# Linyou/Ced-NeRF

Measured on AMD Instinct MI355X. Metric: samples_per_sec (render_image_test, 800x800 D-NeRF lego-shaped synthetic), higher is better.
Workload: dtype f32 (MLP GEMMs: split-fp16 MFMA, 22-bit operands, fp32 accumulate)

## Files before the change

ced_nerf_amd/_lib.py:

```python
from __future__ import annotations

import ctypes as C
import os
import subprocess
from typing import List, Optional

_PKG = os.path.dirname(os.path.abspath(__file__))
_ROOT = os.path.dirname(_PKG)
LIB_PATH = os.environ.get("CED_NERF_LIB", os.path.join(_PKG, "libcednerf_hip.so"))
SOURCES = ["runtime.hip", "march.hip", "composite.hip", "field.hip", "field_half.hip", "field_mixed.hip", "frame.hip", "occgrid.hip",
           "raygen.hip", "wgrad.hip", "pixels.hip", "accel.hip", "linear.hip", "mlp.hip", "train_glue.hip", "losses.hip",
           "metrics.hip", "train_batch.hip", "importance.hip"]
MLP_F32, MLP_F16X2, MLP_F16, MLP_F32_HEAD16X2 = 0, 1, 2, 3
MLP_PRECISIONS = {"f32": MLP_F32, "f16x2": MLP_F16X2, "f16": MLP_F16, "f32+h16x2": MLP_F32_HEAD16X2}
HIPCC_FLAGS = ["--offload-arch=gfx950", "-O3", "-ffp-contract=off", "-fno-slp-vectorize", "-fPIC", "-shared", "-std=c++17"]
PER_SOURCE_FLAGS = {"field_half.hip": ["-mllvm", "-amdgpu-sched-strategy=max-memory-clause"]}
MAX_LEVELS = 16


class HashDesc(C.Structure):
    _fields_ = [
        ("n_levels", C.c_int32), ("table_dtype", C.c_int32), ("temporal", C.c_int32), ("reserved", C.c_int32),
        ("scale", C.c_float * MAX_LEVELS), ("res", C.c_uint32 * MAX_LEVELS), ("offset", C.c_uint32 * MAX_LEVELS),
        ("size", C.c_uint32 * MAX_LEVELS), ("hashed", C.c_uint32 * MAX_LEVELS),
# ... 20 lines not shown


EXCHANGE_FN = C.CFUNCTYPE(C.c_int, C.c_void_p, C.c_void_p, C.c_int32, C.c_int32, C.c_void_p)


class ShardExchange(C.Structure):
    _fields_ = [
        ("global_rays_per_frame", C.c_int64), ("local_rays", C.c_void_p), ("counts", C.c_void_p),
        ("reduce", EXCHANGE_FN), ("user", C.c_void_p),
    ]


_vp, _i64, _i32, _f = C.c_void_p, C.c_int64, C.c_int32, C.c_float

PROTOTYPES = {
    "ced_version": (C.c_int, []),
    "ced_last_error_string": (C.c_char_p, []),
    "ced_set_option": (C.c_int, [C.c_char_p, C.c_int]),
    "ced_packed_weight_floats": (_i64, [C.c_int, C.c_int]),
    "ced_pack_field_weights": (C.c_int, [C.c_int, C.c_int] + [_vp] * 10),
    "ced_packed_weight_words": (_i64, [C.c_int, C.c_int, C.c_int]),
    "ced_pack_field_weights_half": (C.c_int, [C.c_int, C.c_int, C.c_int] + [_vp] * 10),
    "ced_pack_field_weights_half_for": (C.c_int, [C.c_int] * 5 + [_vp] * 10),
    "ced_pack_field_weights_mixed": (C.c_int, [C.c_int, C.c_int] + [_vp] * 10),
    "ced_ray_aabb_intersect": (C.c_int, [_i64, _vp, _vp, _i32, _vp, _f, _f, _f, _vp, _vp, _vp, _vp]),
    "ced_sort_intersections": (C.c_int, [_i64, _i32, _vp, _vp, _vp, _vp, _vp]),
    "ced_traverse_grids": (C.c_int, [_i64, _vp, _vp, _vp, _i32, _i32, _vp, _vp, _vp, _f, _f, _i32, _vp, _vp, _vp, _vp,
                                     _i32, _vp, _vp, _vp, _vp, _vp, _vp, _vp, _vp]),
    "ced_host_skip_march": (_f, [_f, _f, _f, _f]),
    "ced_occupancy_accel_bytes": (_i64, [_i32, _i32]),
    "ced_build_occupancy_accel": (C.c_int, [_vp, _i32, _i32, _vp, _i64, _vp]),
    "ced_host_build_occupancy_accel": (C.c_int, [_vp, _i32, _i32, _vp]),
    "ced_host_count_steps": (_i32, [C.POINTER(C.c_float), _f, _f, _i32, C.POINTER(C.c_float)]),
    "ced_host_march_frame": (C.c_int, [_i64, _vp, _vp, _vp, _i32, _i32, _vp, _vp, _f, _f, _f, _i32, _vp, _vp, _vp, _vp, _i32, _i32,
                                       _i32, _vp, _vp, _vp, _vp]),
    "ced_hash_encode": (C.c_int, [C.POINTER(HashDesc), _i64, _vp, _vp, _vp, _vp]),
    "ced_hash_encode_backward": (C.c_int, [C.POINTER(HashDesc), _i64, _vp, _vp, _vp, _vp, _i32, _vp]),
    "ced_hash_encode_backward_temporal": (C.c_int, [C.POINTER(HashDesc), _i64, _vp, _vp, _vp, _vp, _vp]),
    "ced_field_forward": (C.c_int, [C.POINTER(FieldDesc), _i64, _vp, _vp, _vp, _vp, _vp, _vp, _vp]),
    "ced_field_forward_rays": (C.c_int, [C.POINTER(FieldDesc), _i64, _vp, _vp, _vp, _vp, _vp, _vp, _vp, _i32, _i32,
                                         _vp, _vp, _vp]),
    "ced_render_weights": (C.c_int, [_i64, _vp, _vp, _vp, _vp, _vp, _vp, _vp, _vp, _vp]),
    "ced_accumulate_along_rays": (C.c_int, [_i64, _vp, _vp, _vp, _i32, _vp, _vp]),
    "ced_reduce_along_rays": (C.c_int, [_i64, _vp, _vp, _i32, _vp, _i32, _i64, _i32, _vp, _vp, _vp]),
    "ced_visibility_mask": (C.c_int, [_i64, _vp, _vp, _vp, _vp, _f, _f, _vp, _vp]),
    "ced_composite_prefix": (C.c_int, [_i64, _vp, _vp, _vp, _vp, _vp, _vp, _vp, _vp, _vp]),
    "ced_composite_backward": (C.c_int, [_i64, _vp, _vp, _vp, _vp, _vp, _vp, _vp, _vp, _vp, _vp, _vp]),
    "ced_distortion_workspace_bytes": (_i64, [_i64, _i64, _i32]),
    "ced_distortion_loss": (C.c_int, [_i64, _i64] + [_vp] * 10),
    "ced_distortion_loss_density": (C.c_int, [_i64, _i64] + [_vp] * 10),
    "ced_ssim_workspace_bytes": (_i64, [_i64, _i64, _i64, _i64, _i32, _i32]),
    "ced_ssim": (C.c_int, [_i64, _i64, _i64, _i64, _vp, C.POINTER(_i64), _vp, C.POINTER(_i64), C.c_double, C.c_double,
                           C.c_double, _i32, C.POINTER(C.c_float), _i32, C.POINTER(C.c_float), _i32, _vp, _vp, _vp, _vp,
                           _vp, _vp]),
    "ced_frame_to_rgb8": (C.c_int, [_i32, _i32, _vp, _i32, _vp, _vp]),
    "ced_depth_to_u8": (C.c_int, [_i32, _i32, _vp, _i32, _vp, _vp, _vp]),
    "ced_scatter_pixels": (C.c_int, [_i64, _vp, _i32, _vp, _i32, _vp, _i32, _vp, _i64, _vp, _vp, _vp, _vp, _i32, _i32, _vp]),
    "ced_linear": (C.c_int, [_i64, _vp, _i32, _vp, _i32, _i32, _i32, _i32, _i32, _vp, _vp, _vp]),
    "ced_weight_grad_workspace_bytes": (_i64, [_i64, _i32, _i32]),
    "ced_weight_grad": (C.c_int, [_i64, _vp, _i32, _vp, _i32, _vp, _vp, _i64, _vp]),
    "ced_composite_step": (C.c_int, [_i64, _vp, _vp, _vp, _vp, _vp, _vp, _vp, _vp, _f, _i32, _vp, _vp, _vp]),
    "ced_composite_test": (C.c_int, [_i64, _vp, _vp, _vp, _vp, _vp, _vp, _f, _f, _vp, _vp, _vp, _vp]),
    "ced_finalize_pixels": (C.c_int, [_i64, _vp, _vp, _vp, _vp, _vp]),
    "ced_occ_cell_points": (C.c_int, [_i64, _vp, _vp, _i32, C.POINTER(C.c_float), _vp, _vp]),
    "ced_occ_ema_update": (C.c_int, [_i64, _vp, _vp, _f, _f, _vp, _vp]),
    "ced_generate_rays_pinhole": (C.c_int, [_i32, _i32, _f, _f, _f, _f, C.POINTER(C.c_float), _i32, _vp, _vp, _vp, _vp]),
    "ced_generate_rays_hypercam": (C.c_int, [_i32, _i32, C.POINTER(C.c_float), C.POINTER(C.c_float), _f, _f, _f, _f, _f,
                                             C.POINTER(C.c_float), C.POINTER(C.c_float), _vp, _vp, _vp]),
    "ced_sample_training_batch": (C.c_int, [_i32] * 5 + [_vp] * 3 + [_i64, C.c_uint64, _i64, _i32, _i32] + [_vp] * 7),
    "ced_importance_batch_workspace_bytes": (_i64, [_i64, _i64, _i64]),
    "ced_sample_importance_batch": (C.c_int, [_i32] * 5 + [_vp] * 4 + [_i32, _i64, _i64, C.c_uint64, _i64, _i32] + [_vp] * 8
                                    + [_i64, _vp]),
    "ced_temporal_median_u8": (C.c_int, [_i32] * 4 + [_vp] * 3),
    "ced_isg_weights": (C.c_int, [_i32] * 4 + [_vp, _vp, _f, _vp, _vp]),
    "ced_ist_weights": (C.c_int, [_i32] * 4 + [_vp, _f, _i32, _vp, _vp]),
    "ced_render_image_test_workspace_bytes": (_i64, [_i64, _i32, _i32, _f, _i32]),
    "ced_render_image_test": (C.c_int, [C.POINTER(FieldDesc), _i64, _vp, _vp, _vp, _i32, _i32, _vp, _vp, _f, _f, _f, _f, _f,
                                        _i32, _vp, _i32, _vp, _vp, _vp, _vp, _vp, _i64, _vp, C.POINTER(_i64),
                                        C.POINTER(FrameTrace), _vp, _vp]),
    "ced_render_frames_test_workspace_bytes": (_i64, [_i32, _i64, _i32, _i32, _f, _i32]),
    "ced_render_frames_test": (C.c_int, [C.POINTER(FieldDesc), _i32, _i64, _vp, _vp, _vp, _i32, _i32, _vp, _vp, _f, _f, _f, _f,
                                         _f, _i32, _vp, _vp, _vp, _vp, _vp, _vp, _i64, _vp, C.POINTER(_i64),
                                         C.POINTER(FrameTrace), _vp, _vp]),
    "ced_render_frames_test_sharded_workspace_bytes": (_i64, [_i32, _i64, _i64, _i32, _i32, _f, _i32]),
    "ced_render_frames_test_iterations": (_i32, [_f, _i32]),
    "ced_render_frames_test_host_bytes": (_i64, [_f, _i32]),
    "ced_render_frames_test_sharded": (C.c_int, [C.POINTER(FieldDesc), _i32, _i64, _vp, _vp, _vp, _i32, _i32, _vp, _vp, _f, _f, _f,
                                                 _f, _f, _i32, _vp, _vp, _vp, _vp, _vp, _vp, _i64, _vp, C.POINTER(_i64),
                                                 C.POINTER(FrameTrace), _vp, _vp, C.POINTER(ShardExchange)]),
    "ced_wall_clock_khz": (_i64, []),
    "ced_mlp_chain": (C.c_int, [_i64, _i32, _i32, _vp, C.POINTER(_i32), C.POINTER(_vp), C.POINTER(_vp), C.POINTER(_vp), _i32, _vp]),
    "ced_march_all": (C.c_int, [_i64, _vp, _vp, _vp, _i32, _i32, _vp, _vp, _vp, _f, _f, _f, _vp, _vp, _vp, _i32, _vp, _vp, _vp,
                                _vp, _i64, _vp, _vp]),
    "ced_render_image_workspace_bytes": (_i64, [_i64, _i64]),
    "ced_render_image": (C.c_int, [C.POINTER(FieldDesc), _i64, _vp, _vp, _i64, _vp, _vp, _vp, _f, _f, _vp, _i32, _vp, _vp, _vp,
                                   _vp, _vp, _vp, _i64, _vp, C.POINTER(_i64), _vp, _vp]),
    "ced_mlp_backward_dw_workspace_bytes": (_i64, [_i64, _i32, C.POINTER(_i32)]),
    "ced_mlp_backward_dw": (C.c_int, [_i64, _i32, _vp, C.POINTER(_i32), C.POINTER(_vp), C.POINTER(_vp), _vp, _vp, _vp, _i64, _vp]),
    "ced_train_inputs": (C.c_int, [_i64] + [_vp] * 13),
    "ced_train_warp": (C.c_int, [_i64, _vp, _vp, _i32, _i32, _f, C.POINTER(C.c_float), _vp, _vp, _vp, _vp]),
    "ced_train_warp_backward": (C.c_int, [_i64, _vp, _vp, _i32, _i32, _f, C.POINTER(C.c_float), _vp, _vp, _vp, _vp]),
    "ced_train_head_in": (C.c_int, [_i64] + [_vp] * 6),
    "ced_train_head_in_backward": (C.c_int, [_i64] + [_vp] * 6),
    "ced_render_image_gather": (C.c_int, [_i64, _i64, _i64, _vp, _i64, _vp, _i64, _vp, _vp, _vp, _vp, _vp, _vp, _vp, _vp, _vp]),
}


def _includes(path: str, seen=None) -> List[str]:
    import re
    seen = set() if seen is None else seen
    if path in seen or not os.path.exists(path):
        return []
    seen.add(path)
    out = [path]
    for inc in re.findall(r'^\s*#\s*include\s+"([^"]+)"', open(path).read(), flags=re.M):
        out += _includes(os.path.normpath(os.path.join(os.path.dirname(path), inc)), seen)
    return out


def build(force: bool = False, verbose: bool = False, extra_flags: Optional[List[str]] = None) -> str:
    from concurrent.futures import ThreadPoolExecutor
    srcs = [os.path.join(_PKG, "csrc", s) for s in SOURCES]
    hipcc = os.environ.get("HIPCC", "hipcc")
    flags = [f for f in HIPCC_FLAGS if f != "-shared"] + list(extra_flags or [])
    obj_dir = os.path.join(_ROOT, "build", "obj")
    os.makedirs(obj_dir, exist_ok=True)
    stamp = os.path.join(obj_dir, "flags.txt")
    flag_text = " ".join([hipcc] + flags + [f"{k}:{' '.join(v)}" for k, v in sorted(PER_SOURCE_FLAGS.items())])
    if not os.path.exists(stamp) or open(stamp).read() != flag_text:
        force = True
    jobs, objs = [], []
    for src in srcs:
        obj = os.path.join(obj_dir, os.path.basename(src) + ".o")
        objs.append(obj)
        deps = _includes(src)
        if force or not os.path.exists(obj) or any(os.path.getmtime(obj) < os.path.getmtime(d) for d in deps):
            jobs.append([hipcc] + flags + PER_SOURCE_FLAGS.get(os.path.basename(src), []) + ["-c", src, "-o", obj])
    if not jobs and os.path.exists(LIB_PATH) and all(os.path.getmtime(LIB_PATH) >= os.path.getmtime(o) for o in objs):
        return LIB_PATH

    def run(cmd):
        if verbose:
            print(" ".join(cmd), flush=True)
        subprocess.check_call(cmd)

    workers = max(1, min(len(jobs), int(os.environ.get("CED_BUILD_JOBS", str(min(os.cpu_count() or 1, 8))))))
    if jobs:
        with ThreadPoolExecutor(max_workers=workers) as pool:
            list(pool.map(run, jobs))
    run([hipcc, "--offload-arch=gfx950", "-shared", "-fPIC", "-o", LIB_PATH] + objs)
    from . import _k32_gate
    _, bad = _k32_gate.check(LIB_PATH)
    if bad:
        os.remove(LIB_PATH)
        raise RuntimeError("K = 32 residency gate failed (ced_nerf_amd/_k32_gate.py): "
                           + "; ".join(f"{k}: {v}" for k, v in sorted(bad.items())))
    with open(stamp, "w") as f:
        f.write(flag_text)
    return LIB_PATH


_lib: Optional[C.CDLL] = None


def lib() -> C.CDLL:
    global _lib
# ... 30 lines not shown
```

ced_nerf_amd/csrc/field_args.hpp:

```cpp
#pragma once
#include <hip/hip_runtime.h>
#include <atomic>
#include <cstdint>

#include "../../include/cednerf_hip.h"

namespace ced {

struct FieldArgs {
    int64_t n;
    const int64_t *n_dev;
    unsigned long long *stamp;
    const int64_t *base_dev;
    const float *pos, *t, *dir;
    const float *rays_o, *rays_d;
    const int64_t *ray_idx;
    const int32_t *ray_idx32;
    const float *t0, *t1, *timestamps;
    int rays_mode, t_per_ray, want_rgb;
    float *rgb, *sigma, *geo;
    float aabb[6];
    float moving_step;
    int use_div, time_mode;
    const void *weights;
    int table_dtype, temporal;
    int spread_tiles;
    int level_mode;
    int max_blocks;
    const void *table;
    float scale[CED_MAX_LEVELS];
    uint32_t res[CED_MAX_LEVELS], offset[CED_MAX_LEVELS], size[CED_MAX_LEVELS], hashed[CED_MAX_LEVELS];
};

extern std::atomic<int> g_march_two_pass;
extern std::atomic<int> g_field_spread_tiles;
constexpr int kFieldBlocksDefault = 256;

template <int NT, int THREADS, typename Kernel>
void launch_field_grid(Kernel kernel, const FieldArgs &A, void *stream)
{
    const int64_t n_tiles = (A.n + 16 * NT - 1) / (16 * NT);
    constexpr int waves = THREADS / 64;
    int64_t blocks = A.spread_tiles ? (n_tiles + 3) / 4 : (n_tiles + waves - 1) / waves;
    const int cap = A.max_blocks > 0 ? A.max_blocks : kFieldBlocksDefault;
    if (blocks > cap) blocks = cap;
    hipLaunchKernelGGL(kernel, dim3((unsigned)blocks), dim3(THREADS), 0, (hipStream_t)stream, A);
}

int launch_field(const ced_field_desc *d, FieldArgs &A, void *stream);
int launch_field_half(FieldArgs &A, int time_mode, int precision, void *stream);
int launch_field_mixed(FieldArgs &A, int time_mode, void *stream);

}
```

ced_nerf_amd/csrc/field_half.hip:

```cpp
#include <cstring>

#include "ced_common.hpp"
#include "field_args.hpp"
#include "field_device.hpp"
#include "field_half_device.hpp"

namespace ced {

template <bool TE> struct HalfBlob {
    static constexpr int KS_B0 = TE ? 2 : 1;
    static constexpr int M0 = 0;
    static constexpr int M1 = M0 + 4 * 1;
    static constexpr int M2 = M1 + 4 * 2;
    static constexpr int M3 = M2 + 4 * 2;
    static constexpr int B0 = M3 + 1 * 2;
    static constexpr int B1 = B0 + 4 * KS_B0;
    static constexpr int H0 = B1 + 1 * 2;
    static constexpr int H1 = H0 + 4 * 1;
    static constexpr int H2 = H1 + 4 * 2;
    static constexpr int FRAGS = H2 + 1 * 2;
};

constexpr bool half_kernel_k32(bool te, bool temporal, bool split, int threads)
{
// ... 10 lines not shown
    constexpr int WAVES = THREADS / kWave;
    constexpr bool K32 = half_kernel_k32(TE, TEMPORAL, SPLIT, THREADS);
    static_assert(!K32 || (WAVES & (WAVES - 1)) == 0, "field_tile_seq needs a power-of-two wave count");
    constexpr int TILE = 16 * NT;
    using BL = HalfBlob<TE>;
    constexpr int PLANE = BL::FRAGS * kFragHalves;
    constexpr int WHALVES = PLANE * (SPLIT ? 2 : 1);
    __shared__ __attribute__((aligned(16))) _Float16 lds[WHALVES + 16 * CED_MAX_LEVELS];
    __shared__ int next_elem;
    const int tid = threadIdx.x;
    const int lane = tid & 63;
    const int wave = __builtin_amdgcn_readfirstlane(tid >> 6);
    const int g = lane >> 4, c = lane & 15;

    int64_t n_eff = A.n;
    if (A.n_dev) {
        const int64_t nd = *A.n_dev;
        n_eff = nd < n_eff ? nd : n_eff;
    }
    const int64_t sbase = A.base_dev ? *A.base_dev : 0;
    const int64_t n_tiles = (n_eff + TILE - 1) / TILE;
    TileRange tiles;
    TileSeq seq;
    if constexpr (K32) {
        if (!field_tile_seq(A.spread_tiles, n_tiles, WAVES, seq)) return;
        tiles.first = field_tile_at(seq, wave);
        tiles.end = seq.end;
        tiles.stride = 0;
        if (tid == 0) next_elem = WAVES;
    } else {
        if (!field_tile_range(A.spread_tiles, n_tiles, WAVES, wave, tiles)) return;
    }
    if (A.stamp && tid == 0) atomicMin(A.stamp, (unsigned long long)wall_clock64());

    {
        const f4 *src = reinterpret_cast<const f4 *>(A.weights);
        f4 *dst = reinterpret_cast<f4 *>(lds);
        for (int i = tid; i < WHALVES / 8; i += THREADS) dst[i] = src[i];
        if (tid < CED_MAX_LEVELS) {
            uint32_t *lt = reinterpret_cast<uint32_t *>(lds + WHALVES);
            const LevelConst L = make_level(A.scale[tid], A.res[tid], A.offset[tid], A.size[tid], A.hashed[tid],
                                            EntryBytes<F16, TEMPORAL>::value);
            store_level(lt + tid * 8, L);
        }
    }
    __syncthreads();

    const float extent[3] = { A.aabb[3] - A.aabb[0], A.aabb[4] - A.aabb[1], A.aabb[5] - A.aabb[2] };

    auto next_tile = [&](int64_t tile) -> int64_t {
        if constexpr (K32) {
            int i = 0;
            if (lane == 0) i = atomicAdd(&next_elem, 1);
            return field_tile_at(seq, __builtin_amdgcn_readfirstlane(i));
        } else {
            return tile + tiles.stride;
        }
    };
    for (int64_t tile = tiles.first; tile < tiles.end; tile = next_tile(tile)) {
        int lds_off = 0;
        asm volatile("" : "+v"(lds_off));
        const _Float16 *const whi = lds + lds_off;
        const _Float16 *const wlo = whi + PLANE;
        const int64_t tile_base = tile * TILE;
        const int64_t left = n_eff - tile_base;
        const int in_tile = left < TILE ? (int)left : TILE;
        int sofs[NT];
        int64_t ridx[NT];
        float px[NT][3], tq[NT];
        bool any_used = !A.rays_mode;
#pragma unroll
        for (int j = 0; j < NT; ++j) {
            sofs[j] = 16 * j + c < in_tile ? 16 * j + c : in_tile - 1;
            const int64_t s = tile_base + sofs[j];
            if (A.rays_mode) {
                const int64_t r_in = A.ray_idx32 ? (int64_t)A.ray_idx32[sbase + s] : A.ray_idx[sbase + s];
                const bool used = r_in >= 0;
                const int64_t r = used ? r_in : 0;
                any_used = any_used || used;
                ridx[j] = r;
                const float tm2 = used ? A.t0[sbase + s] + A.t1[sbase + s] : 0.0f;
#pragma unroll
                for (int a = 0; a < 3; ++a) px[j][a] = A.rays_o[3 * r + a] + (A.rays_d[3 * r + a] * tm2) / 2.0f;
                tq[j] = A.t_per_ray ? A.timestamps[r] : A.timestamps[0];
            } else {
                ridx[j] = s;
#pragma unroll
                for (int a = 0; a < 3; ++a) px[j][a] = A.pos[3 * s + a];
                tq[j] = A.t[s];
            }
        }

        if (__ballot(any_used) == 0ull) continue;

        h8 Bh[NT][2], Bl[NT][2];
        f4 D[NT][4];

#pragma unroll
        for (int j = 0; j < NT; ++j) {
            float v = tq[j];
            v = (g == 0) ? px[j][0] : v;
            v = (g == 1) ? px[j][1] : v;
            v = (g == 2) ? px[j][2] : v;
            float f[8];
#pragma unroll
            for (int e = 0; e < 8; ++e) f[e] = det_sinpi_phase(v * (float)(1 << (e >> 1)), e & 1);
            to_half8<SPLIT>(f, Bh[j][0], Bl[j][0]);
        }
        mlp_layer_h<1, 4, NT, SPLIT>(whi + BL::M0 * kFragHalves, wlo + BL::M0 * kFragHalves, lane, Bh, Bl, D);
        to_operand_h<NT, SPLIT>(D, Bh, Bl);
        mlp_layer_h<2, 4, NT, SPLIT, K32>(whi + BL::M1 * kFragHalves, wlo + BL::M1 * kFragHalves, lane, Bh, Bl, D);
        to_operand_h<NT, SPLIT>(D, Bh, Bl);
        mlp_layer_h<2, 4, NT, SPLIT, K32>(whi + BL::M2 * kFragHalves, wlo + BL::M2 * kFragHalves, lane, Bh, Bl, D);
        to_operand_h<NT, SPLIT>(D, Bh, Bl);
        mlp_layer_h<2, 1, NT, SPLIT, K32>(whi + BL::M3 * kFragHalves, wlo + BL::M3 * kFragHalves, lane, Bh, Bl, D);

        float xn[NT][3], mnorm[NT];
        bool sel[NT];
#pragma unroll
        for (int j = 0; j < NT; ++j) {
            float mv[3];
            bool inside = true;
#pragma unroll
            for (int a = 0; a < 3; ++a) {
                const float off = __shfl(D[j][0][a], c, 64);
                float m = off * A.moving_step;
                if (A.use_div) {
                    constexpr int kFineReg[3] = { 3, 0, 1 };
                    const float fine = __shfl(D[j][0][kFineReg[a]], (a == 0) ? c : 16 + c, 64);
                    const float e = det_expf(2.0f * fine);
                    const float th = 1.0f - 2.0f / (e + 1.0f);
                    m = m + th * A.moving_step;
                }
                mv[a] = m;
                const float xm = px[j][a] + m;
                const float x = (xm - A.aabb[a]) / extent[a];
                inside = inside && (x > 0.0f && x < 1.0f);
                xn[j][a] = __builtin_fminf(__builtin_fmaxf(x, 0.0f), 1.0f);
            }
            sel[j] = inside;
            mnorm[j] = TE ? __builtin_sqrtf((mv[0] * mv[0] + mv[1] * mv[1]) + mv[2] * mv[2]) : 0.0f;
        }

        float R[NT][8];
        int k_lo[NT];
        float t_frac[NT];
#pragma unroll
        for (int j = 0; j < NT; ++j) {
            k_lo[j] = 0;
            t_frac[j] = 0.0f;
            if constexpr (TEMPORAL) temporal_keyframe(tq[j], k_lo[j], t_frac[j]);
        }
        const uint32_t *const ltab = reinterpret_cast<const uint32_t *>(whi + WHALVES);
#pragma unroll
        for (int i = 0; i < 4; ++i) {
            const LevelConst L = load_level(ltab + (4 * i + g) * 8);
            const int mode = (A.level_mode >> (2 * i)) & 3;
            if (mode == 1) {
#pragma unroll
                for (int j = 0; j < NT; ++j)
                    hash_level<F16, TEMPORAL, 1>(L, A.table, xn[j], k_lo[j], t_frac[j], R[j][2 * i], R[j][2 * i + 1]);
            } else if (mode == 2) {
#pragma unroll
                for (int j = 0; j < NT; ++j)
                    hash_level<F16, TEMPORAL, 2>(L, A.table, xn[j], k_lo[j], t_frac[j], R[j][2 * i], R[j][2 * i + 1]);
            } else if (mode == 3) {
#pragma unroll
                for (int j = 0; j < NT; ++j)
                    hash_level<F16, TEMPORAL, 3>(L, A.table, xn[j], k_lo[j], t_frac[j], R[j][2 * i], R[j][2 * i + 1]);
            } else {
#pragma unroll
                for (int j = 0; j < NT; ++j)
                    hash_level<F16, TEMPORAL, 0>(L, A.table, xn[j], k_lo[j], t_frac[j], R[j][2 * i], R[j][2 * i + 1]);
            }
        }
#pragma unroll
        for (int j = 0; j < NT; ++j) {
#pragma unroll
            for (int e = 0; e < 8; ++e) R[j][e] = __builtin_amdgcn_fmed3f(R[j][e], -kHalfMax, kHalfMax);
            to_half8<SPLIT>(R[j], Bh[j][0], Bl[j][0]);
            if constexpr (TE) {
                float tf[8];
#pragma unroll
                for (int e = 0; e < 8; ++e) tf[e] = (e < 3) ? time_feature(4 * e + g, A.time_mode, tq[j], mnorm[j]) : 0.0f;
                to_half8<SPLIT>(tf, Bh[j][1], Bl[j][1]);
            }
        }

        mlp_layer_h<BL::KS_B0, 4, NT, SPLIT>(whi + BL::B0 * kFragHalves, wlo + BL::B0 * kFragHalves, lane, Bh, Bl, D);
        to_operand_h<NT, SPLIT>(D, Bh, Bl);
        mlp_layer_h<2, 1, NT, SPLIT, K32>(whi + BL::B1 * kFragHalves, wlo + BL::B1 * kFragHalves, lane, Bh, Bl, D);

#pragma unroll
        for (int j = 0; j < NT; ++j) {
            const bool stored = 16 * j + c < in_tile;
            const int64_t s = tile_base + (16 * j + c);
            float sg = det_expf(D[j][0][3] - 1.0f);
            sg = sel[j] ? sg : 0.0f;
            if (g == 3 && stored) A.sigma[sbase + s] = sg;
            if (A.geo && stored) {
#pragma unroll
                for (int r = 0; r < 4; ++r)
                    if (4 * g + r < 15) A.geo[s * 15 + 4 * g + r] = D[j][0][r];
            }
        }

        if (A.want_rgb) {
#pragma unroll
            for (int j = 0; j < NT; ++j) {
                float dv[3];
#pragma unroll
                for (int a = 0; a < 3; ++a)
                    dv[a] = A.rays_mode ? A.rays_d[3 * ridx[j] + a] : A.dir[3 * (tile_base + sofs[j]) + a];
                const float nrm = __builtin_sqrtf((dv[0] * dv[0] + dv[1] * dv[1]) + dv[2] * dv[2]);
                const float comp = (g == 1) ? dv[1] : (g == 2) ? dv[2] : dv[0];
                const float u = (comp / nrm + 1.0f) / 2.0f;
                const float vv = u * 2.0f - 1.0f;
                const float coef = (g == 2) ? 0.48860251190291987f : -0.48860251190291987f;
                const float sh = (g == 0) ? 0.28209479177387814f : coef * vv;
                float hin[8];
                hin[0] = sh;
#pragma unroll
                for (int r = 0; r < 4; ++r) hin[1 + r] = __builtin_amdgcn_fmed3f(D[j][0][r], -kHalfMax, kHalfMax);
                hin[4] = (g == 3) ? 0.0f : hin[4];
                hin[5] = hin[6] = hin[7] = 0.0f;
                to_half8<SPLIT>(hin, Bh[j][0], Bl[j][0]);
            }
            mlp_layer_h<1, 4, NT, SPLIT>(whi + BL::H0 * kFragHalves, wlo + BL::H0 * kFragHalves, lane, Bh, Bl, D);
            to_operand_h<NT, SPLIT>(D, Bh, Bl);
            mlp_layer_h<2, 4, NT, SPLIT, K32>(whi + BL::H1 * kFragHalves, wlo + BL::H1 * kFragHalves, lane, Bh, Bl, D);
            to_operand_h<NT, SPLIT>(D, Bh, Bl);
            mlp_layer_h<2, 1, NT, SPLIT, K32>(whi + BL::H2 * kFragHalves, wlo + BL::H2 * kFragHalves, lane, Bh, Bl, D);
#pragma unroll
            for (int j = 0; j < NT; ++j) {
                const int64_t s = tile_base + (16 * j + c);
                const float o1 = 1.0f / (1.0f + det_expf(-D[j][0][0]));
                if (g < 3 && 16 * j + c < in_tile) A.rgb[3 * (sbase + s) + g] = o1;
            }
        }
    }
    if constexpr (K32) {
        __syncthreads();
        asm volatile("" ::: "v127");
    }
    if (A.stamp && lane == 0) atomicMax(A.stamp + 1, (unsigned long long)wall_clock64());
}

void pack_half_layer(const float *w, int n_out, int n_in, int nb, int ks, int frag, int row_map, int col_map,
                     _Float16 *hi, _Float16 *lo)
{
    for (int p = 0; p < nb * 16; ++p) {
        int neuron = p;
        if (row_map == HALF_ROW_HIDDEN) neuron = half_hidden_neuron(p);
        else if (row_map == HALF_ROW_HIDDEN_K32) neuron = half_hidden_neuron_k32(p);
        else if (row_map == HALF_ROW_BASE_OUT) neuron = half_base_out_neuron(p);
        else if (row_map == HALF_ROW_RGB) neuron = (p % 4 == 0) ? p / 4 : n_out;
        if (neuron >= n_out) continue;
        for (int k = 0; k < ks * 32; ++k) {
            const int g = (k % 32) / 8, e = k % 8;
            int in = k;
            if (col_map == HALF_COL_HASH) {
                if (k < 32) in = 2 * (4 * (e >> 1) + g) + (e & 1);
                else in = (e < 3 && 4 * e + g <= 8) ? 32 + 4 * e + g : -1;
            } else if (col_map == HALF_COL_K32) {
                in = half_hidden_neuron_k32(16 * (2 * (k / 32) + (e >> 2)) + 4 * g + (e & 3));
            } else if (col_map == HALF_COL_HEAD) {
                if (e == 0) in = g;
                else if (e <= 4 && 4 * g + e - 1 < 15) in = 4 + 4 * g + e - 1;
                else in = -1;
            }
            if (in < 0 || in >= n_in) continue;
            const float v = w[(int64_t)neuron * n_in + in];
            const _Float16 h = (_Float16)v;
            const int64_t idx = ((int64_t)(frag + (p / 16) * ks + k / 32) * 64 + 16 * g + (p % 16)) * 8 + e;
            hi[idx] = h;
            if (lo) lo[idx] = (_Float16)(v - (float)h);
        }
    }
}

int launch_field_half(FieldArgs &A, int time_mode, int precision, void *stream)
{
    const int sel = (time_mode ? 1 : 0) | (A.table_dtype ? 2 : 0) | (A.temporal ? 4 : 0);
    if (precision == CED_MLP_F16X2) {
        switch (sel) {
        case 0: launch_field_grid<2, 1024>(field_half_kernel<false, false, false, true, 2, 1024>, A, stream); break;
        case 1: launch_field_grid<2, 768>(field_half_kernel<true, false, false, true, 2, 768>, A, stream); break;
        case 2: launch_field_grid<2, 1024>(field_half_kernel<false, true, false, true, 2, 1024>, A, stream); break;
        case 3: launch_field_grid<2, 768>(field_half_kernel<true, true, false, true, 2, 768>, A, stream); break;
        case 4: launch_field_grid<2, 512>(field_half_kernel<false, false, true, true, 2, 512>, A, stream); break;
        case 5: launch_field_grid<2, 512>(field_half_kernel<true, false, true, true, 2, 512>, A, stream); break;
        case 6: launch_field_grid<2, 512>(field_half_kernel<false, true, true, true, 2, 512>, A, stream); break;
        default: launch_field_grid<2, 512>(field_half_kernel<true, true, true, true, 2, 512>, A, stream); break;
        }
    } else {
        switch (sel) {
        case 0: launch_field_grid<2, 768>(field_half_kernel<false, false, false, false, 2, 768>, A, stream); break;
        case 1: launch_field_grid<2, 768>(field_half_kernel<true, false, false, false, 2, 768>, A, stream); break;
        case 2: launch_field_grid<2, 768>(field_half_kernel<false, true, false, false, 2, 768>, A, stream); break;
        case 3: launch_field_grid<2, 768>(field_half_kernel<true, true, false, false, 2, 768>, A, stream); break;
// ... 78 lines not shown
```

ced_nerf_amd/csrc/field_kernel.hpp:

```cpp
#pragma once
#include "ced_common.hpp"
#include "field_args.hpp"
#include "field_device.hpp"
#include "field_half_device.hpp"

namespace ced {

struct LayerShape { int nb; int ks; };
__host__ __device__ constexpr int ks4_of(int ks) { return (ks + 3) / 4; }
__host__ __device__ constexpr int layer_floats(int nb, int ks) { return nb * ks4_of(ks) * 256; }

__host__ __device__ constexpr int base_out_neuron(int p)
{
    const int g = p >> 2, r = p & 3;
    return r > 0 ? (4 * r + g - 3) : (g < 3 ? 13 + g : 0);
}

template <bool TE> struct Blob {
    static constexpr int KS_B0 = TE ? 11 : 8;
    static constexpr int M0 = 0;
    static constexpr int M1 = M0 + layer_floats(4, 8);
    static constexpr int M2 = M1 + layer_floats(4, 16);
    static constexpr int M3 = M2 + layer_floats(4, 16);
    static constexpr int B0 = M3 + layer_floats(1, 16);
// ... 34 lines not shown
                    acc[j] = __builtin_amdgcn_mfma_f32_16x16x4f32(a[s], B[j][4 * q + s], acc[j], 0, 0, 0);
            }
        }
        if (q == KS4 - 1) {
#pragma unroll
            for (int j = 0; j < NT; ++j) D[j][nb] = acc[j];
        }
        a = a_next;
    }
}

template <int NB, bool RELU, int NT>
__device__ __forceinline__ void to_operand(const f4 (&D)[NT][4], float (&B)[NT][16])
{
#pragma unroll
    for (int j = 0; j < NT; ++j) {
#pragma unroll
        for (int nb = 0; nb < NB; ++nb) {
            float r[4];
#pragma unroll
            for (int q = 0; q < 4; ++q) {
                float v = D[j][nb][q];
                if constexpr (RELU) {
                    const int bits = __float_as_int(v);
                    v = __int_as_float(bits > 0 ? bits : 0);
                }
                r[q] = v;
            }
#pragma unroll
            for (int s = 0; s < 4; ++s) B[j][4 * nb + s] = r[s];
        }
    }
}

template <bool TE, bool F16, bool TEMPORAL, int NT, int THREADS, bool HEAD16 = false>
__global__ __launch_bounds__(THREADS) void field_kernel(FieldArgs A)
{
    constexpr int FIELD_THREADS = THREADS;
    constexpr int FIELD_WAVES = THREADS / kWave;
    constexpr int TILE = 16 * NT;
    using BL = Blob<TE>;
    __shared__ __attribute__((aligned(16))) float lds[BL::TOTAL + 8 * CED_MAX_LEVELS];
    const int tid = threadIdx.x;
    const int lane = tid & 63;
    const int g = lane >> 4, c = lane & 15;

    int64_t n_eff = A.n;
    if (A.n_dev) {
        const int64_t nd = *A.n_dev;
        n_eff = nd < n_eff ? nd : n_eff;
    }
    const int64_t sbase = A.base_dev ? *A.base_dev : 0;
    const int64_t n_tiles = (n_eff + TILE - 1) / TILE;
    TileRange tiles;
    if (!field_tile_range(A.spread_tiles, n_tiles, FIELD_WAVES, threadIdx.x >> 6, tiles)) return;
    if (A.stamp && tid == 0) atomicMin(A.stamp, (unsigned long long)wall_clock64());

    {
        const f4 *src = reinterpret_cast<const f4 *>(A.weights);
        f4 *dst = reinterpret_cast<f4 *>(lds);
        for (int i = tid; i < BL::TOTAL / 4; i += FIELD_THREADS) dst[i] = src[i];
        if (tid < CED_MAX_LEVELS) {
            uint32_t *lt = reinterpret_cast<uint32_t *>(lds + BL::TOTAL);
            const LevelConst L = make_level(A.scale[tid], A.res[tid], A.offset[tid], A.size[tid], A.hashed[tid],
                                            EntryBytes<F16, TEMPORAL>::value);
            store_level(lt + tid * 8, L);
        }
    }
    __syncthreads();

    const float extent[3] = { A.aabb[3] - A.aabb[0], A.aabb[4] - A.aabb[1], A.aabb[5] - A.aabb[2] };
    const bool shared_time = A.rays_mode && !A.t_per_ray;
    float t_feat[2] = { 0.0f, 0.0f };
    if (shared_time) {
        const float t_all = A.timestamps[0];
#pragma unroll
        for (int S = 6; S < 8; ++S) t_feat[S - 6] = det_sinpi_phase(t_all * (float)(1 << (2 * (S & 1) + (g >> 1))), g & 1);
    }

    for (int64_t tile = tiles.first; tile < tiles.end; tile += tiles.stride) {
        int lds_off = 0;
        asm volatile("" : "+v"(lds_off));
        const float *const lw = lds + lds_off;
        int64_t sidx[NT];
        int64_t ridx[NT];
        float px[NT][3], tq[NT];
        bool any_used = !A.rays_mode;
#pragma unroll
        for (int j = 0; j < NT; ++j) {
            int64_t s = tile * TILE + 16 * j + c;
            s = s < n_eff ? s : n_eff - 1;
            sidx[j] = s;
            if (A.rays_mode) {
                const int64_t r_in = A.ray_idx32 ? (int64_t)A.ray_idx32[sbase + s] : A.ray_idx[sbase + s];
                const bool used = r_in >= 0;
                const int64_t r = used ? r_in : 0;
                any_used = any_used || used;
                ridx[j] = r;
                const float tm2 = used ? A.t0[sbase + s] + A.t1[sbase + s] : 0.0f;
#pragma unroll
                for (int a = 0; a < 3; ++a) px[j][a] = A.rays_o[3 * r + a] + (A.rays_d[3 * r + a] * tm2) / 2.0f;
                tq[j] = A.t_per_ray ? A.timestamps[r] : A.timestamps[0];
            } else {
                ridx[j] = s;
#pragma unroll
                for (int a = 0; a < 3; ++a) px[j][a] = A.pos[3 * s + a];
                tq[j] = A.t[s];
            }
        }
        if (__ballot(any_used) == 0ull) continue;

        float B[NT][16];
        f4 D[NT][4];

#pragma unroll
        for (int j = 0; j < NT; ++j) {
            const bool odd = (g & 1) != 0;
            const float sc0 = (float)(1 << (g >> 1)), sc1 = 4.0f * sc0;
            const float vxy = odd ? px[j][1] : px[j][0];
            float p0, p1;
            det_sinpi_both(vxy * sc0, p0, p1);
            auto sw = __builtin_amdgcn_permlane16_swap(__float_as_uint(p0), __float_as_uint(p1), false, false);
            B[j][0] = __uint_as_float(sw[0]); B[j][2] = __uint_as_float(sw[1]);
            det_sinpi_both(vxy * sc1, p0, p1);
            sw = __builtin_amdgcn_permlane16_swap(__float_as_uint(p0), __float_as_uint(p1), false, false);
            B[j][1] = __uint_as_float(sw[0]); B[j][3] = __uint_as_float(sw[1]);
            const float scz = odd ? sc1 : sc0;
            det_sinpi_both(px[j][2] * scz, p0, p1);
            sw = __builtin_amdgcn_permlane16_swap(__float_as_uint(p0), __float_as_uint(p1), false, false);
            B[j][4] = __uint_as_float(sw[0]); B[j][5] = __uint_as_float(sw[1]);
            if (shared_time) {
                B[j][6] = t_feat[0];
                B[j][7] = t_feat[1];
            } else {
                det_sinpi_both(tq[j] * scz, p0, p1);
                sw = __builtin_amdgcn_permlane16_swap(__float_as_uint(p0), __float_as_uint(p1), false, false);
                B[j][6] = __uint_as_float(sw[0]); B[j][7] = __uint_as_float(sw[1]);
            }
        }
        mlp_layer<8, 4, NT>(lw + BL::M0, lane, B, D);
        to_operand<4, true, NT>(D, B);
        mlp_layer<16, 4, NT>(lw + BL::M1, lane, B, D);
        to_operand<4, true, NT>(D, B);
        mlp_layer<16, 4, NT>(lw + BL::M2, lane, B, D);
        to_operand<4, true, NT>(D, B);
        mlp_layer<16, 1, NT>(lw + BL::M3, lane, B, D);

        float xn[NT][3], mnorm[NT];
        bool sel[NT];
#pragma unroll
        for (int j = 0; j < NT; ++j) {
            float mv[3];
            bool inside = true;
#pragma unroll
            for (int a = 0; a < 3; ++a) {
                const float off = __shfl(D[j][0][a], c, 64);
                float m = off * A.moving_step;
                if (A.use_div) {
                    constexpr int kFineReg[3] = { 3, 0, 1 };
                    const float fine = __shfl(D[j][0][kFineReg[a]], (a == 0) ? c : 16 + c, 64);
                    const float e = det_expf(2.0f * fine);
                    const float th = 1.0f - 2.0f / (e + 1.0f);
                    m = m + th * A.moving_step;
                }
                mv[a] = m;
                const float xm = px[j][a] + m;
                const float x = (xm - A.aabb[a]) / extent[a];
                inside = inside && (x > 0.0f && x < 1.0f);
                xn[j][a] = __builtin_fminf(__builtin_fmaxf(x, 0.0f), 1.0f);
            }
            sel[j] = inside;
            mnorm[j] = TE ? __builtin_sqrtf((mv[0] * mv[0] + mv[1] * mv[1]) + mv[2] * mv[2]) : 0.0f;
        }

        float R[NT][8];
        int k_lo[NT];
        float t_frac[NT];
#pragma unroll
        for (int j = 0; j < NT; ++j) {
            k_lo[j] = 0;
            t_frac[j] = 0.0f;
            if constexpr (TEMPORAL) temporal_keyframe(tq[j], k_lo[j], t_frac[j]);
        }
        const uint32_t *const ltab = reinterpret_cast<const uint32_t *>(lw + BL::TOTAL);
#pragma unroll
        for (int i = 0; i < 4; ++i) {
            const LevelConst L = load_level(ltab + (4 * i + 2 * (g & 1) + (g >> 1)) * 8);
            const int mode = (A.level_mode >> (2 * i)) & 3;
            if (mode == 1) {
#pragma unroll
                for (int j = 0; j < NT; ++j)
                    hash_level<F16, TEMPORAL, 1>(L, A.table, xn[j], k_lo[j], t_frac[j], R[j][2 * i], R[j][2 * i + 1]);
            } else if (mode == 2) {
#pragma unroll
                for (int j = 0; j < NT; ++j)
                    hash_level<F16, TEMPORAL, 2>(L, A.table, xn[j], k_lo[j], t_frac[j], R[j][2 * i], R[j][2 * i + 1]);
            } else if (mode == 3) {
#pragma unroll
                for (int j = 0; j < NT; ++j)
                    hash_level<F16, TEMPORAL, 3>(L, A.table, xn[j], k_lo[j], t_frac[j], R[j][2 * i], R[j][2 * i + 1]);
            } else {
#pragma unroll
                for (int j = 0; j < NT; ++j)
                    hash_level<F16, TEMPORAL, 0>(L, A.table, xn[j], k_lo[j], t_frac[j], R[j][2 * i], R[j][2 * i + 1]);
            }
        }
#pragma unroll
        for (int j = 0; j < NT; ++j) {
#pragma unroll
            for (int i = 0; i < 4; ++i) {
                auto sw = __builtin_amdgcn_permlane16_swap(__float_as_uint(R[j][2 * i]), __float_as_uint(R[j][2 * i + 1]), false, false);
                B[j][2 * i] = __uint_as_float(sw[0]);
                B[j][2 * i + 1] = __uint_as_float(sw[1]);
            }
            if (TE) {
#pragma unroll
                for (int S = 8; S < 11; ++S) B[j][S] = time_feature(4 * (S - 8) + g, A.time_mode, tq[j], mnorm[j]);
            }
        }

        mlp_layer<BL::KS_B0, 4, NT>(lw + BL::B0, lane, B, D);
        to_operand<4, true, NT>(D, B);
        mlp_layer<16, 1, NT>(lw + BL::B1, lane, B, D);

#pragma unroll
        for (int j = 0; j < NT; ++j) {
            const int64_t s = tile * TILE + 16 * j + c;
            float sg = det_expf(D[j][0][HEAD16 ? 3 : 0] - 1.0f);
            sg = sel[j] ? sg : 0.0f;
            if (g == 3 && s < n_eff) A.sigma[sbase + s] = sg;
            if (A.geo && s < n_eff) {
#pragma unroll
                for (int r = 0; r < 4; ++r) {
                    const int nidx = HEAD16 ? half_base_out_neuron(4 * g + r) : base_out_neuron(4 * g + r);
                    if (nidx >= 1) A.geo[s * 15 + nidx - 1] = D[j][0][r];
                }
            }
        }

        if constexpr (HEAD16) {
            if (A.want_rgb) {
                const _Float16 *const hw = reinterpret_cast<const _Float16 *>(lw + BL::H0);
                const _Float16 *const hwl = hw + BL::HEAD_FRAGS * kFragHalves;
                h8 Bh[NT][2], Bl[NT][2];
#pragma unroll
                for (int j = 0; j < NT; ++j) {
                    float dv[3];
#pragma unroll
                    for (int a = 0; a < 3; ++a)
                        dv[a] = A.rays_mode ? A.rays_d[3 * ridx[j] + a] : A.dir[3 * sidx[j] + a];
                    const float nrm = __builtin_sqrtf((dv[0] * dv[0] + dv[1] * dv[1]) + dv[2] * dv[2]);
                    const float comp = (g == 1) ? dv[1] : (g == 2) ? dv[2] : dv[0];
                    const float u = (comp / nrm + 1.0f) / 2.0f;
                    const float vv = u * 2.0f - 1.0f;
                    const float coef = (g == 2) ? 0.48860251190291987f : -0.48860251190291987f;
                    float hin[8];
                    hin[0] = (g == 0) ? 0.28209479177387814f : coef * vv;
#pragma unroll
                    for (int r = 0; r < 4; ++r) hin[1 + r] = __builtin_amdgcn_fmed3f(D[j][0][r], -kHalfMax, kHalfMax);
                    hin[4] = (g == 3) ? 0.0f : hin[4];
                    hin[5] = hin[6] = hin[7] = 0.0f;
                    to_half8<true>(hin, Bh[j][0], Bl[j][0]);
                }
                mlp_layer_h<1, 4, NT, true>(hw + BL::HF_H0 * kFragHalves, hwl + BL::HF_H0 * kFragHalves, lane, Bh, Bl, D);
                to_operand_h<NT, true>(D, Bh, Bl);
                mlp_layer_h<2, 4, NT, true>(hw + BL::HF_H1 * kFragHalves, hwl + BL::HF_H1 * kFragHalves, lane, Bh, Bl, D);
                to_operand_h<NT, true>(D, Bh, Bl);
                mlp_layer_h<2, 1, NT, true>(hw + BL::HF_H2 * kFragHalves, hwl + BL::HF_H2 * kFragHalves, lane, Bh, Bl, D);
#pragma unroll
                for (int j = 0; j < NT; ++j) {
                    const float o1 = 1.0f / (1.0f + det_expf(-D[j][0][0]));
                    int lane_now = (int)threadIdx.x;
                    asm volatile("" : "+v"(lane_now));
                    const int g_now = (lane_now >> 4) & 3;
                    const int64_t s_now = tile * TILE + 16 * j + (lane_now & 15);
                    if (g_now < 3 && s_now < n_eff) A.rgb[3 * (sbase + s_now) + g_now] = o1;
                }
            }
            continue;
        }

        if (A.want_rgb) {
#pragma unroll
            for (int j = 0; j < NT; ++j) {
                const float geo_tail = (g == 3) ? 0.0f : D[j][0][0];
                float dv[3];
#pragma unroll
                for (int a = 0; a < 3; ++a)
                    dv[a] = A.rays_mode ? A.rays_d[3 * ridx[j] + a] : A.dir[3 * sidx[j] + a];
                const float nrm = __builtin_sqrtf((dv[0] * dv[0] + dv[1] * dv[1]) + dv[2] * dv[2]);
                const float comp = (g == 1) ? dv[1] : (g == 2) ? dv[2] : dv[0];
                const float u = (comp / nrm + 1.0f) / 2.0f;
                const float vv = u * 2.0f - 1.0f;
                const float coef = (g == 2) ? 0.48860251190291987f : -0.48860251190291987f;
                B[j][0] = (g == 0) ? 0.28209479177387814f : coef * vv;
                B[j][1] = D[j][0][1];
                B[j][2] = D[j][0][2];
                B[j][3] = D[j][0][3];
                B[j][4] = geo_tail;
            }
            mlp_layer<5, 4, NT>(lw + BL::H0, lane, B, D);
            to_operand<4, true, NT>(D, B);
            mlp_layer<16, 4, NT>(lw + BL::H1, lane, B, D);
            to_operand<4, true, NT>(D, B);
            mlp_layer<16, 1, NT>(lw + BL::H2, lane, B, D);
#pragma unroll
            for (int j = 0; j < NT; ++j) {
                const int64_t s = tile * TILE + 16 * j + c;
                const float o1 = 1.0f / (1.0f + det_expf(-D[j][0][0]));
                int lane_now = (int)threadIdx.x;
                asm volatile("" : "+v"(lane_now));
                const int g_now = (lane_now >> 4) & 3;
                const int64_t s_now = tile * TILE + 16 * j + (lane_now & 15);
                if (g_now < 3 && s_now < n_eff) A.rgb[3 * (sbase + s_now) + g_now] = o1;
            }
        }
    }
    if (A.stamp && lane == 0) atomicMax(A.stamp + 1, (unsigned long long)wall_clock64());
}

}
```

ced_nerf_amd/csrc/frame.hip:

```cpp
#include <atomic>
#include <cfloat>
#include <chrono>
#include <vector>

#include "ced_common.hpp"
#include "field_args.hpp"
#include "march_accel.hpp"

#ifdef CED_MARCH_DIAG
__device__ unsigned long long g_march_diag[8][3];
__device__ __forceinline__ unsigned long long (*ced_diag_acc())[8][3]
{
    __shared__ unsigned long long acc[16][8][3];
    return acc;
}
__device__ __forceinline__ unsigned long long *ced_diag_state()
{
    __shared__ unsigned long long st[16][2];
    return &st[0][0];
}
__device__ void ced_diag_tick(int phase)
{
    const unsigned long long m = __ballot(1);
    const int wave = threadIdx.x >> 6;
// ... 49 lines not shown
    int32_t gcount[kMaxFrames];
    int32_t limit[kMaxFrames];
    int32_t last[kMaxFrames];
    int32_t used[kMaxFrames];
    int32_t slot_base[kMaxFrames];
    int32_t samp_bound[kMaxFrames];
    int32_t total_slots;
    int32_t done;
    int32_t n_cand;
    int32_t cursor;
    int64_t sample_base;
    int64_t total_samples;
    unsigned long long next[kMaxFrames];
};

__device__ __forceinline__ int frame_of_slot(const IterPlan &P, int n_frames, int64_t s0)
{
    int lo = 0, hi = n_frames - 1;
    while (lo < hi) {
        const int mid = (lo + hi + 1) >> 1;
        if ((int64_t)P.slot_base[mid] <= s0) lo = mid; else hi = mid - 1;
    }
    return (P.count[lo] > 0 && s0 >= P.slot_base[lo] && s0 < (int64_t)P.slot_base[lo] + P.count[lo]) ? lo : -1;
}

template <int kWaves, class Reserve>
__device__ __forceinline__ int64_t workgroup_reserve(int n, Reserve reserve)
{
    __shared__ int wave_tot[kWaves];
    __shared__ long long block_base;
    const int lane = threadIdx.x & 63, wave = threadIdx.x >> 6;
    int incl = n;
#pragma unroll
    for (int off = 1; off < 64; off <<= 1) {
        const int v = __shfl_up(incl, off, 64);
        if (lane >= off) incl += v;
    }
    if (lane == 63) wave_tot[wave] = incl;
    __syncthreads();
    if (threadIdx.x == 0) {
        int run = 0;
        for (int w = 0; w < kWaves; ++w) { const int t = wave_tot[w]; wave_tot[w] = run; run += t; }
        block_base = run > 0 ? reserve(run) : 0;
    }
    __syncthreads();
    return (int64_t)block_base + wave_tot[wave] + (incl - n);
}

template <int kWaves, int kSums, class Reserve>
__device__ __forceinline__ int workgroup_append(bool take, const int *sums, Reserve reserve)
{
    __shared__ int wave_cnt[kWaves], wave_sum[kSums > 0 ? kSums : 1][kWaves];
    __shared__ int block_base;
    const int lane = threadIdx.x & 63, wave = threadIdx.x >> 6;
    const unsigned long long ballot = __ballot(take);
    int tot[kSums > 0 ? kSums : 1];
#pragma unroll
    for (int k = 0; k < kSums; ++k) tot[k] = sums[k];
#pragma unroll
    for (int off = 32; off >= 1; off >>= 1)
#pragma unroll
        for (int k = 0; k < kSums; ++k) tot[k] += __shfl_xor(tot[k], off, 64);
    if (lane == 0) {
        wave_cnt[wave] = __builtin_popcountll(ballot);
#pragma unroll
        for (int k = 0; k < kSums; ++k) wave_sum[k][wave] = tot[k];
    }
    __syncthreads();
    if (threadIdx.x == 0) {
        int run = 0;
#pragma unroll
        for (int k = 0; k < kSums; ++k) tot[k] = 0;
        for (int w = 0; w < kWaves; ++w) {
            const int t = wave_cnt[w]; wave_cnt[w] = run; run += t;
#pragma unroll
            for (int k = 0; k < kSums; ++k) tot[k] += wave_sum[k][w];
        }
        block_base = reserve(run, tot);
    }
    __syncthreads();
    return block_base + wave_cnt[wave] + __builtin_popcountll(ballot & ((1ull << lane) - 1ull));
}

__global__ __launch_bounds__(256) void frame_times_kernel(int64_t n_rays, int rays_per_frame,
                                                          const float *__restrict__ frame_times, float *__restrict__ ts_ray)
{
    const int64_t r = (int64_t)blockIdx.x * blockDim.x + threadIdx.x;
    if (r < n_rays) ts_ray[r] = frame_times[r / rays_per_frame];
}

__global__ __launch_bounds__(256) void frame_prep_kernel(int64_t n_rays, const float *__restrict__ rays_o,
                                                         const float *__restrict__ rays_d, int m,
                                                         const float *__restrict__ aabbs, float near_plane,
                                                         float *__restrict__ t_sorted, uint8_t *__restrict__ t_indices,
                                                         uint8_t *__restrict__ hits, float *__restrict__ near_planes,
                                                         float *__restrict__ rgb,
                                                         float *__restrict__ opacity, float *__restrict__ depth)
{
    int64_t r = (int64_t)blockIdx.x * blockDim.x + threadIdx.x;
    if (r >= n_rays) return;
    const float o[3] = { rays_o[3 * r], rays_o[3 * r + 1], rays_o[3 * r + 2] };
    const float inv_d[3] = { 1.0f / rays_d[3 * r], 1.0f / rays_d[3 * r + 1], 1.0f / rays_d[3 * r + 2] };
    float ev[2 * kMaxGrids];
    int id[2 * kMaxGrids];
    for (int a = 0; a < m; ++a) {
        float t0 = __builtin_inff(), t1 = __builtin_inff();
        bool hit = slab_test(o, inv_d, aabbs + 6 * a, t0, t1);
        if (!hit) { t0 = __builtin_inff(); t1 = __builtin_inff(); }
        hits[r * m + a] = hit ? 1 : 0;
        ev[a] = t0; id[a] = a;
        ev[m + a] = t1; id[m + a] = m + a;
    }
    if (m > 1) {
        for (int i = 1; i < 2 * m; ++i) {
            float v = ev[i];
            int k = id[i], j = i - 1;
            while (j >= 0 && ev[j] > v) { ev[j + 1] = ev[j]; id[j + 1] = id[j]; --j; }
            ev[j + 1] = v; id[j + 1] = k;
        }
    }
    for (int i = 0; i < 2 * m; ++i) {
        t_sorted[r * 2 * m + i] = ev[i];
        t_indices[r * 2 * m + i] = (uint8_t)id[i];
    }
    near_planes[r] = near_plane;
    rgb[3 * r] = 0.0f; rgb[3 * r + 1] = 0.0f; rgb[3 * r + 2] = 0.0f;
    opacity[r] = 0.0f;
    depth[r] = 0.0f;
}

__global__ __launch_bounds__(256) void frame_prep_single_kernel(int64_t n_rays, float near_plane, float *__restrict__ near_planes,
                                                                float *__restrict__ rgb, float *__restrict__ opacity,
                                                                float *__restrict__ depth)
{
    int64_t r = (int64_t)blockIdx.x * blockDim.x + threadIdx.x;
    if (r >= n_rays) return;
    near_planes[r] = near_plane;
    rgb[3 * r] = 0.0f; rgb[3 * r + 1] = 0.0f; rgb[3 * r + 2] = 0.0f;
    opacity[r] = 0.0f;
    depth[r] = 0.0f;
}

struct ScheduleArgs {
    IterPlan *plans;
    int it, n_frames, rays_per_frame, min_samples, max_samples;
    long long *host;
    long long seq;
    const int32_t *local_rays;
    const int64_t *xcounts;
    int64_t global_rays;
    long long *host_iter;
};

__device__ __forceinline__ void make_next_plan(const ScheduleArgs &S)
{
    const int f = threadIdx.x & 63;
    IterPlan &N = S.plans[S.it + 1];
    int local = 0, used = 0;
    long long global = 0;
    if (f < S.n_frames) {
        if (S.it < 0) {
            local = S.local_rays ? S.local_rays[f] : S.rays_per_frame;
            global = S.global_rays > 0 ? S.global_rays : local;
        } else {
            const IterPlan &P = S.plans[S.it];
            const unsigned long long nx = __hip_atomic_load(&P.next[f], __ATOMIC_RELAXED, __HIP_MEMORY_SCOPE_AGENT);
            const bool finished = P.last[f] || P.gcount[f] == 0;
            local = (finished || P.count[f] == 0) ? 0 : (int)(nx & 0xffffffffull);
            global = finished ? 0 : (S.xcounts ? S.xcounts[(int64_t)S.it * S.n_frames + f] : local);
            used = P.used[f];
        }
    }
    int count = 0, gcount = 0, limit = 0, last = 0;
    if (global > 0 && used < S.max_samples) {
        const long long n_total = S.global_rays > 0 ? S.global_rays : S.rays_per_frame;
        const long long q = n_total / global;
        limit = q < 64 ? (int)q : 64;
        if (limit < S.min_samples) limit = S.min_samples;
        used += limit;
        last = used >= S.max_samples ? 1 : 0;
        count = local;
        gcount = (int)(global < 0x7fffffffll ? global : 0x7fffffffll);
    }
    const int padded = (count + kSlotAlign - 1) & ~(kSlotAlign - 1);
    int incl = padded;
#pragma unroll
    for (int off = 1; off < 64; off <<= 1) {
        const int v = __shfl_up(incl, off, 64);
        if (f >= off) incl += v;
    }
    long long alive_here = count, alive_all = gcount;
#pragma unroll
    for (int off = 32; off >= 1; off >>= 1) {
        alive_here += __shfl_xor(alive_here, off, 64);
        alive_all += __shfl_xor(alive_all, off, 64);
    }
    const int total_slots = __shfl(incl, 63, 64);
    N.count[f] = count; N.gcount[f] = gcount; N.limit[f] = limit; N.last[f] = last; N.used[f] = used;
    N.slot_base[f] = incl - padded; N.samp_bound[f] = count * limit;
    N.next[f] = 0;
    if (f == 0) {
        N.total_slots = total_slots;
        N.sample_base = S.it < 0 ? 0 : S.plans[S.it].sample_base + S.plans[S.it].total_samples;
        N.total_samples = 0;
        N.n_cand = 0;
        N.cursor = 0;
        N.done = alive_all == 0 ? 1 : 0;
        S.host[0] = alive_here;
        S.host[1] = N.done;
        if (S.host_iter) {
            S.host_iter[3 * (S.it + 1)] = alive_here;
            S.host_iter[3 * (S.it + 1) + 1] = N.done;
        }
        __threadfence_system();
        __hip_atomic_store(&S.host[2], S.seq, __ATOMIC_RELEASE, __HIP_MEMORY_SCOPE_SYSTEM);
        if (S.host_iter) __hip_atomic_store(&S.host_iter[3 * (S.it + 1) + 2], S.seq, __ATOMIC_RELEASE, __HIP_MEMORY_SCOPE_SYSTEM);
    }
}

__global__ void frame_init_kernel(ScheduleArgs S, float *__restrict__ lattice_dev, unsigned long long *stamps = nullptr,
                                  int n_stamps = 0)
{
    for (int i = threadIdx.x; i < n_stamps; i += blockDim.x) {
// ... 140 lines not shown
            f = frame_of_slot(P, A.n_frames, s0);
            if (f < 0) continue;
            const int64_t idx = s0 + threadIdx.x - P.slot_base[f];
            active = idx < P.count[f];
            const int64_t first = (int64_t)f * A.rays_per_frame;
            r = active ? (A.alive ? (int64_t)A.alive[first + idx] : first + idx) : 0;
        }
        const int limit = P.limit[f];
        GridSpec grid = A.grid;
        grid.limit = limit;
        const int m = grid.n_grids;
        float o[3] = { 0.0f, 0.0f, 0.0f }, d[3] = { 0.0f, 0.0f, 1.0f };
        float near = 0.0f, t_term = 0.0f;
        const auto walk = [&](auto &&emit, float &t_out) {
            return traverse_ray_frame<kFrameLook, SINGLE, FIRST>(
                grid, A.accel, FIRST, o, d, near, A.far_plane,
                SINGLE ? nullptr : A.t_sorted + r * 2 * m, SINGLE ? (const uint8_t *)nullptr : A.t_indices + r * 2 * m,
                SINGLE ? nullptr : A.hits + r * m, emit, t_out);
        };
        SampleRuns runs;
        int n = 0;
        CED_DIAG_TICK(0);
        if (active) {
#pragma unroll
            for (int a = 0; a < 3; ++a) { o[a] = A.rays_o[3 * r + a]; d[a] = A.rays_d[3 * r + a]; }
            near = A.near_planes[r];
            n = walk([&](int i, float t0, float t1) { runs.record(i, t0, t1); }, t_term);
            A.near_planes[r] = t_term;
        }
        CED_DIAG_TICK(6);
        const int64_t start = workgroup_reserve<kWaves>(n, [&](int run) {
            return (long long)atomicAdd(reinterpret_cast<unsigned long long *>(&plan->total_samples), (unsigned long long)run);
        });
        if (active) {
            A.packed[2 * r] = (int32_t)start;
            A.packed[2 * r + 1] = n;
            float *const p0 = A.t_starts + start, *const p1 = A.t_ends + start;
            int32_t *const pr = A.ray_idx + start;
            const auto store = [&](int i, float t0, float t1) { p0[i] = t0; p1[i] = t1; pr[i] = (int32_t)r; };
            if (n > 0 && !runs.replayable(grid)) {
                float unused;
                (void)walk(store, unused);
            } else {
                runs.replay(grid, store);
            }
        }
        CED_DIAG_TICK(7);
        __syncthreads();
    }
#ifdef CED_MARCH_DIAG
    ced_diag_flush();
#endif
}

#ifdef CED_MARCH_DIAG
}
extern "C" int ced_diag_march_read(unsigned long long *out, int reset)
{
    if (hipDeviceSynchronize() != hipSuccess) return -1;
    if (out && hipMemcpyFromSymbol(out, HIP_SYMBOL(g_march_diag), sizeof(unsigned long long) * 24) != hipSuccess) return -1;
    if (reset) {
        unsigned long long z[24] = { 0 };
        if (hipMemcpyToSymbol(HIP_SYMBOL(g_march_diag), z, sizeof(z)) != hipSuccess) return -1;
    }
    return 0;
}
extern "C" int ced_diag_march_waves(unsigned int *out, int max_rows, int reset)
{
    if (hipDeviceSynchronize() != hipSuccess) return -1;
    unsigned int n = 0;
    if (hipMemcpyFromSymbol(&n, HIP_SYMBOL(g_march_wave_n), 4) != hipSuccess) return -1;
    if (n > (unsigned)kDiagWaves) n = kDiagWaves;
    if ((int)n > max_rows) n = max_rows;
    if (out && n && hipMemcpyFromSymbol(out, HIP_SYMBOL(g_march_wave_log), (size_t)n * 96) != hipSuccess) return -1;
    if (reset) {
        unsigned int z = 0;
        if (hipMemcpyToSymbol(HIP_SYMBOL(g_march_wave_n), &z, 4) != hipSuccess) return -1;
    }
    return (int)n;
}
namespace ced {
#endif

__global__ __launch_bounds__(kCompositeThreads) void frame_composite_kernel(
    IterPlan *plan, int n_frames, int rays_per_frame, const int32_t *__restrict__ alive_list,
    int32_t *__restrict__ next_list, const int32_t *__restrict__ packed, const float *__restrict__ t0,
    const float *__restrict__ t1, const float *__restrict__ sig, const float *__restrict__ rgbs, float *__restrict__ rgb,
    float *__restrict__ opacity, float *__restrict__ depth, float opc_thres)
{
    const IterPlan &P = *plan;
    const int64_t total = P.total_slots;
    for (int64_t s0 = (int64_t)blockIdx.x * kCompositeThreads; s0 < total; s0 += (int64_t)gridDim.x * kCompositeThreads) {
        const int f = frame_of_slot(P, n_frames, s0);
        if (f < 0) continue;
        const int limit = P.limit[f];
        const int64_t idx = s0 + threadIdx.x - P.slot_base[f];
        const bool active = idx < P.count[f];
        const int64_t first = (int64_t)f * rays_per_frame;
        const int64_t r = active ? (alive_list ? (int64_t)alive_list[first + idx] : first + idx) : 0;
        int cnt = 0;
        bool alive = false;
        if (active) {
            const int64_t sb = packed[2 * r];
            cnt = packed[2 * r + 1];
            float op = opacity[r];
            if (cnt > 0) {
                const float prefix = 1.0f - op;
                float c0 = rgb[3 * r], c1 = rgb[3 * r + 1], c2 = rgb[3 * r + 2], dp = depth[r];
                float acc = 0.0f;
                constexpr int kU = 4;
                int64_t i = sb;
                const int64_t end = sb + cnt;
                for (; i + kU <= end; i += kU) {
                    float ts[kU], te[kU], sg[kU], cr[kU], cg[kU], cb[kU];
#pragma unroll
                    for (int u = 0; u < kU; ++u) {
                        ts[u] = t0[i + u]; te[u] = t1[i + u]; sg[u] = sig[i + u];
                        cr[u] = rgbs[3 * (i + u)]; cg[u] = rgbs[3 * (i + u) + 1]; cb[u] = rgbs[3 * (i + u) + 2];
                    }
#pragma unroll
                    for (int u = 0; u < kU; ++u) {
                        float sd = sg[u] * (te[u] - ts[u]);
                        float a = 1.0f - det_expf(-sd);
                        float t = det_expf(-acc) * prefix;
                        float w = t * a;
                        c0 = c0 + w * cr[u];
                        c1 = c1 + w * cg[u];
                        c2 = c2 + w * cb[u];
                        op = op + w;
                        dp = dp + w * ((ts[u] + te[u]) / 2.0f);
                        acc = acc + sd;
                    }
                }
                for (; i < end; ++i) {
                    float ts = t0[i], te = t1[i];
                    float sd = sig[i] * (te - ts);
                    float a = 1.0f - det_expf(-sd);
                    float t = det_expf(-acc) * prefix;
                    float w = t * a;
                    c0 = c0 + w * rgbs[3 * i];
                    c1 = c1 + w * rgbs[3 * i + 1];
                    c2 = c2 + w * rgbs[3 * i + 2];
                    op = op + w;
                    dp = dp + w * ((ts + te) / 2.0f);
                    acc = acc + sd;
                }
                rgb[3 * r] = c0; rgb[3 * r + 1] = c1; rgb[3 * r + 2] = c2;
                opacity[r] = op;
                depth[r] = dp;
            }
            alive = !P.last[f] && (op <= opc_thres) && (cnt == limit);
        }
        const int slot = workgroup_append<kCompositeThreads / 64, 1>(alive, &cnt, [&](int run, const int *samples) {
            const unsigned long long add = (unsigned long long)run + ((unsigned long long)samples[0] << 32);
            return add != 0 ? (int)(atomicAdd(&plan->next[f], add) & 0xffffffffull) : 0;
        });
        if (alive) next_list[first + slot] = (int32_t)r;
        __syncthreads();
    }
}

__global__ __launch_bounds__(64) void frame_schedule_kernel(ScheduleArgs S)
{
    make_next_plan(S);
}

__global__ __launch_bounds__(64) void frame_pack_counts_kernel(const IterPlan *__restrict__ plan, int n_frames,
                                                               int64_t *__restrict__ row)
{
    const int f = threadIdx.x;
    if (f >= n_frames) return;
    const unsigned long long nx = __hip_atomic_load(&plan->next[f], __ATOMIC_RELAXED, __HIP_MEMORY_SCOPE_AGENT);
    const bool finished = plan->last[f] || plan->gcount[f] == 0 || plan->count[f] == 0;
    row[f] = finished ? 0 : (int64_t)(nx & 0xffffffffull);
}

__global__ __launch_bounds__(256) void frame_finalize_kernel(int64_t n_rays, const float *__restrict__ bkgd,
                                                             float *__restrict__ rgb, const float *__restrict__ opacity,
                                                             float *__restrict__ depth)
{
    int64_t r = (int64_t)blockIdx.x * blockDim.x + threadIdx.x;
    if (r >= n_rays) return;
    float op = opacity[r];
    if (bkgd) {
        float rem = 1.0f - op;
        rgb[3 * r] = rgb[3 * r] + bkgd[0] * rem;
        rgb[3 * r + 1] = rgb[3 * r + 1] + bkgd[1] * rem;
        rgb[3 * r + 2] = rgb[3 * r + 2] + bkgd[2] * rem;
    }
    depth[r] = depth[r] / __builtin_fmaxf(op, FLT_EPSILON);
}

struct ImageState {
    int32_t *cursor;
    float *acc_all;
    float *acc_kept;
    int32_t *kept;
};

__global__ __launch_bounds__(256) void image_prep_kernel(int64_t n_rays, ImageState st, float *__restrict__ rgb,
                                                         float *__restrict__ opacity, float *__restrict__ depth)
{
    int64_t r = (int64_t)blockIdx.x * blockDim.x + threadIdx.x;
    if (r >= n_rays) return;
    st.cursor[r] = 0; st.acc_all[r] = 0.0f; st.acc_kept[r] = 0.0f; st.kept[r] = 0;
    if (rgb) {
        rgb[3 * r] = 0.0f; rgb[3 * r + 1] = 0.0f; rgb[3 * r + 2] = 0.0f;
        opacity[r] = 0.0f;
        depth[r] = 0.0f;
    }
}

__device__ __forceinline__ int64_t ray_count(const int64_t *__restrict__ packed_all, int64_t r, int64_t n_all)
{
    const int64_t start = packed_all[2 * r], cnt = packed_all[2 * r + 1];
    return (start < 0 || cnt < 0 || start + cnt > n_all) ? 0 : cnt;
}

__global__ __launch_bounds__(kMarchThreads) void image_chunk_kernel(
    IterPlan *__restrict__ plan, int64_t n_all, const int32_t *__restrict__ alive, const int64_t *__restrict__ packed_all,
    const float *__restrict__ t0_all, const float *__restrict__ t1_all, const int32_t *__restrict__ cursor,
    float *__restrict__ t0s, float *__restrict__ t1s, int32_t *__restrict__ ridx, int32_t *__restrict__ packed)
{
    const IterPlan &P = *plan;
    const int64_t total = P.count[0];
    const int limit = P.limit[0];
    const int64_t base = P.sample_base;
    for (int64_t s0 = (int64_t)blockIdx.x * kMarchThreads; s0 < total; s0 += (int64_t)gridDim.x * kMarchThreads) {
        const int64_t idx = s0 + threadIdx.x;
        const bool active = idx < total;
        const int64_t r = active ? (alive ? (int64_t)alive[idx] : idx) : 0;
        int n = 0;
        int64_t src = 0;
        if (active) {
            const int cur = cursor[r];
            const int64_t left = ray_count(packed_all, r, n_all) - cur;
            n = (int)(left < limit ? left : limit);
            src = packed_all[2 * r] + cur;
        }
        const int64_t slot = workgroup_reserve<kMarchThreads / 64>(n, [&](int run) {
            return (long long)atomicAdd(reinterpret_cast<unsigned long long *>(&plan->total_samples), (unsigned long long)run);
        });
        if (active) {
            const int64_t start = base + slot;
            packed[2 * r] = (int32_t)start;
            packed[2 * r + 1] = n;
            for (int i = 0; i < n; ++i) {
                t0s[start + i] = t0_all[src + i];
                t1s[start + i] = t1_all[src + i];
                ridx[start + i] = (int32_t)r;
            }
        }
        __syncthreads();
    }
}

template <bool FULL>
__global__ __launch_bounds__(kCompositeThreads) void image_composite_kernel(
    IterPlan *plan, const int32_t *__restrict__ alive_list, int32_t *__restrict__ next_list,
    const int32_t *__restrict__ packed, const int64_t *__restrict__ packed_all, const float *__restrict__ t0,
    const float *__restrict__ t1, const float *__restrict__ sig, const float *__restrict__ rgbs, ImageState st,
    float *__restrict__ w_out, float *__restrict__ tr_out, float *__restrict__ al_out, int32_t *__restrict__ rank_out,
    float *__restrict__ rgb, float *__restrict__ opacity, float *__restrict__ depth, float eps, float alpha_thre,
    int64_t n_all)
{
    const IterPlan &P = *plan;
    const int64_t total = P.count[0];
    for (int64_t s0 = (int64_t)blockIdx.x * kCompositeThreads; s0 < total; s0 += (int64_t)gridDim.x * kCompositeThreads) {
        const int64_t idx = s0 + threadIdx.x;
        const bool active = idx < total;
        const int64_t r = active ? (alive_list ? (int64_t)alive_list[idx] : idx) : 0;
        int cnt = 0, kept_new = 0;
        bool alive = false;
        if (active) {
            const int64_t sb = packed[2 * r];
            cnt = packed[2 * r + 1];
            if (cnt > 0) {
                float c0 = 0.0f, c1 = 0.0f, c2 = 0.0f, op = 0.0f, dp = 0.0f;
                if constexpr (FULL) { c0 = rgb[3 * r]; c1 = rgb[3 * r + 1]; c2 = rgb[3 * r + 2]; op = opacity[r]; dp = depth[r]; }
                float acc = st.acc_all[r], acck = st.acc_kept[r];
                int kept = st.kept[r];
                const int kept_before = kept;
                bool open = true;
                constexpr int kU = 4;
                const int64_t end = sb + cnt;
                for (int64_t i = sb; i < end; i += kU) {
                    float ts[kU], te[kU], sg[kU], cr[kU], cg[kU], cb[kU];
#pragma unroll
// ... 105 lines not shown
#pragma unroll
    for (int a = 0; a < 3; ++a) { o[a] = A.rays_o[3 * r + a]; d[a] = A.rays_d[3 * r + a]; }
    const int m = A.grid.n_grids;
    const float *const ts_row = SINGLE ? nullptr : A.t_sorted + r * 2 * m;
    const int64_t *const ti_row = SINGLE ? nullptr : A.t_indices + r * 2 * m;
    const uint8_t *const hit_row = SINGLE ? nullptr : A.hits + r * m;
    float t_term;
    if constexpr (!FILL) {
        const int n = traverse_ray_frame<kFrameLook, SINGLE, false>(A.grid, A.accel, true, o, d, A.near_planes[r], A.far_plane, ts_row,
                                                             ti_row, hit_row, [](int, float, float) {}, t_term);
        A.packed[2 * r + 1] = n;
    } else {
        const int64_t start = A.packed[2 * r];
        if (A.packed[2 * r + 1] == 0) return;
        float *const p0 = A.t_starts + start, *const p1 = A.t_ends + start;
        int64_t *const pr = A.ray_indices ? A.ray_indices + start : nullptr;
        (void)traverse_ray_frame<kFrameLook, SINGLE, false>(A.grid, A.accel, true, o, d, A.near_planes[r], A.far_plane, ts_row, ti_row,
                                                     hit_row,
                                                     [&](int i, float t0, float t1) {
                                                         p0[i] = t0; p1[i] = t1;
                                                         if (pr) pr[i] = r;
                                                     },
                                                     t_term);
    }
}

template <bool SINGLE>
__global__ __launch_bounds__(kMarchThreads, SINGLE ? 4 : 3) void march_all_onepass_kernel(MarchAllArgs A, int64_t capacity,
                                                                                         unsigned long long *total)
{
    const int64_t r = (int64_t)blockIdx.x * kMarchThreads + threadIdx.x;
    const bool active = r < A.n_rays;
    const int m = A.grid.n_grids;
    float o[3] = { 0.0f, 0.0f, 0.0f }, d[3] = { 0.0f, 0.0f, 1.0f };
    float near = 0.0f, t_term = 0.0f;
    const float *const ts_row = (SINGLE || !active) ? nullptr : A.t_sorted + r * 2 * m;
    const int64_t *const ti_row = (SINGLE || !active) ? nullptr : A.t_indices + r * 2 * m;
    const uint8_t *const hit_row = (SINGLE || !active) ? nullptr : A.hits + r * m;
    const auto walk = [&](auto &&emit, float &t_out) {
        return traverse_ray_frame<kFrameLook, SINGLE, false>(A.grid, A.accel, true, o, d, near, A.far_plane, ts_row, ti_row,
                                                             hit_row, emit, t_out);
    };
    SampleRuns runs;
    int n = 0;
    if (active) {
#pragma unroll
        for (int a = 0; a < 3; ++a) { o[a] = A.rays_o[3 * r + a]; d[a] = A.rays_d[3 * r + a]; }
        near = A.near_planes[r];
        n = walk([&](int i, float t0, float t1) { runs.record(i, t0, t1); }, t_term);
    }
    const int64_t start = workgroup_reserve<kMarchThreads / 64>(n, [&](int run) {
        return (long long)atomicAdd(total, (unsigned long long)run);
    });
    if (!active) return;
    A.packed[2 * r] = start;
    A.packed[2 * r + 1] = n;
    if (n == 0 || start + n > capacity) return;
    float *const p0 = A.t_starts + start, *const p1 = A.t_ends + start;
    const auto store = [&](int i, float t0, float t1) { p0[i] = t0; p1[i] = t1; };
    if (!runs.replayable(A.grid)) {
        float unused;
        (void)walk(store, unused);
    } else {
        runs.replay(A.grid, store);
    }
}

struct Carver {
    char *base;
    size_t off = 0;
    template <class T> T *take(size_t count)
    {
        T *p = (T *)(base + off);
        off = (off + count * sizeof(T) + 255) & ~(size_t)255;
        return p;
    }
};

struct FrameWorkspace {
    float *t_sorted; uint8_t *t_indices; uint8_t *hits; float *near; int32_t *packed;
    int32_t *alive_a, *alive_b;
    IterPlan *plans;
    float *lattice;
    float *ts_ray;
    float *t0, *t1; int32_t *ridx; float *sigma, *rgbs;
    uint8_t *accel;
    size_t bytes;
};

static inline int min_samples_of(float cone_angle) { return cone_angle == 0.0f ? 1 : 4; }
static inline int max_iterations(int max_samples, int min_samples) { return (max_samples + min_samples - 1) / min_samples; }

static inline int64_t sample_capacity(int n_frames, int64_t rays_per_frame, int min_samples, int64_t global_rays)
{
    int64_t per = rays_per_frame * min_samples;
    if (global_rays > rays_per_frame) {
        const int64_t worst = rays_per_frame * 64 < global_rays ? rays_per_frame * 64 : global_rays;
        if (worst > per) per = worst;
    }
    return per * n_frames;
}

static FrameWorkspace carve(void *base, int64_t n, int m, int64_t cap, int max_iters, int res, bool per_ray_times = false)
{
    FrameWorkspace w{};
    Carver c{ (char *)base };
    w.t_sorted = c.take<float>((size_t)n * 2 * m);
    w.t_indices = c.take<uint8_t>((size_t)n * 2 * m);
    w.hits = c.take<uint8_t>((size_t)n * m);
    w.near = c.take<float>((size_t)n);
    w.packed = c.take<int32_t>((size_t)n * 2);
    w.alive_a = c.take<int32_t>((size_t)n);
    w.alive_b = c.take<int32_t>((size_t)n);
    w.plans = c.take<IterPlan>((size_t)max_iters + 2);
    w.lattice = c.take<float>(256);
    w.ts_ray = c.take<float>(per_ray_times ? (size_t)n : 0);
    w.t0 = c.take<float>((size_t)cap);
    w.t1 = c.take<float>((size_t)cap);
    w.ridx = c.take<int32_t>((size_t)cap);
    w.sigma = c.take<float>((size_t)cap);
    w.rgbs = c.take<float>((size_t)cap * 3);
    const int64_t nbk = (res + kBrick - 1) / kBrick;
    w.accel = c.take<uint8_t>((size_t)(2 * m * nbk * nbk * nbk));
    w.bytes = c.off;
    return w;
}

static std::atomic<long long> g_publish_seq{ 0 };

#if defined(__HIP_DEVICE_COMPILE__)
#define CED_CPU_PAUSE()
#else
#define CED_CPU_PAUSE() __builtin_ia32_pause()
#endif

static int wait_published(volatile long long *flag, long long seq, hipStream_t stream, const char *who)
{
    const auto t_start = std::chrono::steady_clock::now();
    long spins = 0;
    while (__atomic_load_n(flag, __ATOMIC_ACQUIRE) < seq) {
        if ((++spins & 0x3ff) == 0) {
            if (std::chrono::steady_clock::now() - t_start > std::chrono::milliseconds(200)) {
                if (hipStreamSynchronize(stream) != hipSuccess) return check_launch("render_image_test (sync)");
                if (__atomic_load_n(flag, __ATOMIC_ACQUIRE) < seq) {
                    set_error("%s: iteration %lld was not published although the stream has drained", who, seq);
                    return CED_E_LAUNCH;
                }
                break;
            }
        } else {
            CED_CPU_PAUSE();
        }
    }
    return CED_OK;
}

static int run_ahead(volatile long long *pub, volatile long long *host_iter, const std::vector<long long> &plan_seq, int it,
                     hipStream_t stream, const char *who, bool &stop, long long &alive_bound)
{
    const int need = it - kRunAhead;
    if (need < 0 && host_iter) return CED_OK;
    volatile long long *const rec = host_iter ? host_iter + 3 * need : pub;
    if (need >= 0) {
        const int rc = wait_published(rec + 2, plan_seq[need], stream, who);
        if (rc) return rc;
    }
    if (host_iter || __atomic_load_n(pub + 2, __ATOMIC_ACQUIRE) >= plan_seq[0]) {
        if (rec[1]) {
            stop = true;
            return CED_OK;
        }
        const long long a = rec[0];
        if (a >= 0 && a < alive_bound) alive_bound = a;
    }
    return CED_OK;
}

static int read_back_plans(const IterPlan *dev_plans, int enqueued, hipStream_t stream, const char *what, const char *who,
                           std::vector<IterPlan> &plans, int &n_iters)
{
    plans.resize((size_t)enqueued + 1);
    if (hipMemcpyAsync(plans.data(), dev_plans, plans.size() * sizeof(IterPlan), hipMemcpyDeviceToHost, stream) != hipSuccess ||
        hipStreamSynchronize(stream) != hipSuccess)
        return check_launch(what);
    n_iters = 0;
    while (n_iters < enqueued && !plans[n_iters].done && plans[n_iters].total_slots != 0) ++n_iters;
    if (n_iters == enqueued && !plans[enqueued].done) {
        set_error("%s: the loop stopped after %d iterations with rays still alive", who, enqueued);
        return CED_E_LAUNCH;
    }
    return CED_OK;
}

static int render_frames_impl(const ced_field_desc *field, int n_frames, int64_t rays_per_frame, const float *rays_o,
                              const float *rays_d, const uint8_t *binaries, int32_t n_grids, int32_t res,
                              const float *aabbs, const void *accel, float near_plane, float far_plane, float step_size,
                              float cone_angle, float early_stop_eps, int32_t max_samples, const float *timestamps,
                              int32_t t_per_ray, const float *frame_times, const float *bkgd, float *rgb, float *opacity,
                              float *depth, void *workspace, int64_t workspace_bytes, int64_t *host_stats,
                              int64_t *total_samples_out, ced_frame_trace *trace, void *field_stream_, void *stream_,
                              const char *who, const ced_shard_exchange *xch = nullptr)
{
    hipStream_t stream = (hipStream_t)stream_;
    hipStream_t fstream = field_stream_ ? (hipStream_t)field_stream_ : stream;
    const bool split = fstream != stream;
    constexpr int kMaxDevices = 64;
    static thread_local hipEvent_t ev_to_field[kMaxDevices] = {}, ev_from_field[kMaxDevices] = {};
    int dev = 0;
    if (split) {
        if (hipGetDevice(&dev) != hipSuccess || dev < 0 || dev >= kMaxDevices) return check_launch("render_image_test (device)");
        if (!ev_to_field[dev] &&
            (hipEventCreateWithFlags(&ev_to_field[dev], hipEventDisableTiming) != hipSuccess ||
             hipEventCreateWithFlags(&ev_from_field[dev], hipEventDisableTiming) != hipSuccess))
            return check_launch("render_image_test (event create)");
    }
    const int64_t n_rays = (int64_t)n_frames * rays_per_frame;
    CED_REQUIRE(field != nullptr, "%s: null field descriptor", who);
    CED_REQUIRE(n_frames >= 1 && n_frames <= kMaxFrames, "%s: n_frames must be 1..%d", who, kMaxFrames);
    CED_REQUIRE(rays_per_frame >= 0 && n_grids >= 1 && n_grids <= kMaxGrids && res >= 1 && res <= 1024, "%s: bad sizes", who);
    CED_REQUIRE(n_rays < (1ll << 31) / 4, "%s: too many rays for 32-bit sample indices", who);
    CED_REQUIRE(max_samples >= 0, "%s: max_samples < 0", who);
    if (total_samples_out)
        for (int f = 0; f < n_frames; ++f) total_samples_out[f] = 0;
    if (trace) trace->n_iters = 0;
    if (n_rays == 0) return CED_OK;
    CED_REQUIRE(rays_o && rays_d && binaries && aabbs && (timestamps || frame_times) && rgb && opacity && depth &&
                    workspace && host_stats,
                "%s: null pointer", who);
    const int min_samples = min_samples_of(cone_angle);
    const int64_t cap = sample_capacity(n_frames, rays_per_frame, min_samples, xch ? xch->global_rays_per_frame : 0);
    CED_REQUIRE(cap < (1ll << 31) - 64, "%s: too many samples per iteration for 32-bit sample indices", who);
    const int max_iters = max_iterations(max_samples, min_samples);
    FrameWorkspace W = carve(workspace, n_rays, n_grids, cap, max_iters, res, frame_times != nullptr);
    CED_REQUIRE((int64_t)W.bytes <= workspace_bytes, "%s: workspace too small (%lld < %lld bytes)", who,
                (long long)workspace_bytes, (long long)W.bytes);
    if (xch) {
        CED_REQUIRE(xch->reduce && xch->counts && xch->global_rays_per_frame >= rays_per_frame &&
                        xch->global_rays_per_frame < (1ll << 31),
                    "%s: bad ced_shard_exchange (reduce / counts NULL, or global_rays_per_frame < rays_per_frame)", who);
        CED_REQUIRE(!field_stream_ || field_stream_ == stream_, "%s: a sharded call takes no separate field stream", who);
    }
    long long *const host_iter = xch ? (long long *)host_stats + kHostIterWord : nullptr;
    const dim3 blk(256), grd((unsigned)((n_rays + 255) / 256));

    if (n_grids == 1)
        hipLaunchKernelGGL(frame_prep_single_kernel, grd, blk, 0, stream, n_rays, near_plane, W.near, rgb, opacity, depth);
    else
        hipLaunchKernelGGL(frame_prep_kernel, grd, blk, 0, stream, n_rays, rays_o, rays_d, (int)n_grids, aabbs, near_plane,
                           W.t_sorted, W.t_indices, W.hits, W.near, rgb, opacity, depth);
    if (frame_times)
        hipLaunchKernelGGL(frame_times_kernel, grd, blk, 0, stream, n_rays, (int)rays_per_frame, frame_times, W.ts_ray);
    const int nb = (res + kBrick - 1) / kBrick;
    AccelSpec acc;
    if (accel) {
        acc = accel_view(accel, n_grids, res, true);
    } else {
        int rc = build_brick_accel(binaries, n_grids, res, W.accel, W.accel + (size_t)n_grids * nb * nb * nb, stream);
        if (rc) return rc;
        acc = AccelSpec{ W.accel, nb, nullptr };
    }
    volatile long long *pub = (volatile long long *)host_stats;
    std::vector<long long> plan_seq((size_t)max_iters + 1);
    plan_seq[0] = ++g_publish_seq;
    const bool use_lattice = cone_angle == 0.0f && step_size > 0.0f && near_plane >= 0.0f;
    if (use_lattice) build_lattice(near_plane, step_size, reinterpret_cast<float *>(host_stats + kHostLatticeWord));
    hipLaunchKernelGGL(frame_init_kernel, dim3(1), dim3(64), 0, stream,
                       ScheduleArgs{ W.plans, -1, n_frames, (int)rays_per_frame, min_samples, (int)max_samples,
                                     (long long *)host_stats, plan_seq[0], xch ? xch->local_rays : nullptr, nullptr,
                                     xch ? xch->global_rays_per_frame : 0, host_iter },
                       use_lattice ? W.lattice : (float *)nullptr,
                       (unsigned long long *)(trace ? trace->field_stamps : nullptr),
                       (trace && trace->field_stamps) ? (int)trace->capacity : 0);
    int rc = check_launch("render_image_test (prep)");
    if (rc) return rc;

    const float opc_thres = (float)(1.0 - (double)early_stop_eps);
    long long alive_bound = n_rays;
    int it = 0;
    for (; it < max_iters; ++it) {
        bool stop = false;
        rc = run_ahead(pub, host_iter, plan_seq, it, stream, who, stop, alive_bound);
        if (rc) return rc;
        if (stop) break;
        IterPlan *plan = W.plans + it;
        const int32_t *cur_list = it == 0 ? nullptr : ((it & 1) ? W.alive_a : W.alive_b);
        int32_t *next_list = (it & 1) ? W.alive_b : W.alive_a;

        const int64_t slot_bound = alive_bound + (int64_t)n_frames * kSlotAlign;
        MarchArgs M{ rays_o, rays_d, GridSpec{ binaries, aabbs, n_grids, res, step_size, cone_angle, 0, use_lattice ? W.lattice : nullptr },
                     acc, W.near, far_plane, cur_list, n_frames,
                     (int)rays_per_frame, W.t_sorted, W.t_indices, W.hits, W.t0, W.t1, W.ridx, W.packed, W.alive_b };
        int64_t mgrid = (slot_bound + kMarchThreads - 1) / kMarchThreads;
        if (mgrid > 8192) mgrid = 8192;
        const dim3 mblk(kMarchThreads);
        const int two_pass_opt = g_march_two_pass;
        const bool two_pass = two_pass_opt < 0 ? n_grids > 1 : two_pass_opt != 0;
        if (it == 0 && acc.bdist && two_pass) {
            int64_t kgrid = (slot_bound + kCullThreads - 1) / kCullThreads;
            if (kgrid > 8192) kgrid = 8192;
            if (mgrid > 4096) mgrid = 4096;
            if (n_grids == 1) {
                hipLaunchKernelGGL(march_cull_kernel<true>, dim3((unsigned)kgrid), dim3(kCullThreads), 0, stream, M, plan);
                hipLaunchKernelGGL((march_frame_kernel<true, true, true>), dim3((unsigned)mgrid), mblk, 0, stream, M, plan);
            } else {
                hipLaunchKernelGGL(march_cull_kernel<false>, dim3((unsigned)kgrid), dim3(kCullThreads), 0, stream, M, plan);
                hipLaunchKernelGGL((march_frame_kernel<false, true, true>), dim3((unsigned)mgrid), mblk, 0, stream, M, plan);
            }
        } else if (it == 0) {
            if (n_grids == 1) hipLaunchKernelGGL((march_frame_kernel<true, false, true>), dim3((unsigned)mgrid), mblk, 0, stream, M, plan);
            else hipLaunchKernelGGL((march_frame_kernel<false, false, true>), dim3((unsigned)mgrid), mblk, 0, stream, M, plan);
        } else {
            if (n_grids == 1) hipLaunchKernelGGL((march_frame_kernel<true, false, false>), dim3((unsigned)mgrid), mblk, 0, stream, M, plan);
            else hipLaunchKernelGGL((march_frame_kernel<false, false, false>), dim3((unsigned)mgrid), mblk, 0, stream, M, plan);
        }
        rc = check_launch("render_image_test (march)");
        if (rc) return rc;

        FieldArgs F{};
        F.n = cap;
        F.n_dev = &plan->total_samples;
        F.rays_o = rays_o; F.rays_d = rays_d; F.ray_idx32 = W.ridx;
        F.t0 = W.t0; F.t1 = W.t1;
        F.timestamps = frame_times ? W.ts_ray : timestamps;
        F.rays_mode = 1; F.t_per_ray = (frame_times || t_per_ray) ? 1 : 0; F.want_rgb = 1;
        F.rgb = W.rgbs; F.sigma = W.sigma; F.geo = nullptr;
        if (trace && trace->field_stamps && it < trace->capacity)
            F.stamp = reinterpret_cast<unsigned long long *>(trace->field_stamps) + 2 * it;
        if (split) {
            (void)hipEventRecord(ev_to_field[dev], stream);
            (void)hipStreamWaitEvent(fstream, ev_to_field[dev], 0);
        }
        if (trace && it < trace->capacity && trace->field_begin)
            (void)hipEventRecord((hipEvent_t)trace->field_begin[it], fstream);
        rc = launch_field(field, F, (void *)fstream);
        if (rc) return rc;
        if (trace && it < trace->capacity && trace->field_end)
            (void)hipEventRecord((hipEvent_t)trace->field_end[it], fstream);
        if (split) {
            (void)hipEventRecord(ev_from_field[dev], fstream);
            (void)hipStreamWaitEvent(stream, ev_from_field[dev], 0);
        }

        int64_t cgrid = (slot_bound + kCompositeThreads - 1) / kCompositeThreads;
        if (cgrid > 4096) cgrid = 4096;
        plan_seq[it + 1] = ++g_publish_seq;
        hipLaunchKernelGGL(frame_composite_kernel, dim3((unsigned)cgrid), dim3(kCompositeThreads), 0, stream,
                           plan, n_frames, (int)rays_per_frame, cur_list, next_list, W.packed, W.t0, W.t1, W.sigma, W.rgbs,
                           rgb, opacity, depth, opc_thres);
        int64_t *xrow = nullptr;
        if (xch) {
            xrow = xch->counts + (int64_t)it * n_frames;
            hipLaunchKernelGGL(frame_pack_counts_kernel, dim3(1), dim3(64), 0, stream, plan, n_frames, xrow);
            rc = check_launch("render_image_test (pack counts)");
            if (rc) return rc;
            const int xrc = xch->reduce(xch->user, xrow, n_frames, it, (void *)stream);
            if (xrc != 0) {
                set_error("%s: the exchange step of iteration %d failed (code %d)", who, it, xrc);
                (void)hipStreamSynchronize(stream);
                return CED_E_LAUNCH;
            }
        }
        hipLaunchKernelGGL(frame_schedule_kernel, dim3(1), dim3(64), 0, stream,
                           ScheduleArgs{ W.plans, it, n_frames, (int)rays_per_frame, min_samples, (int)max_samples,
                                         (long long *)host_stats, plan_seq[it + 1], xch ? xch->local_rays : nullptr,
                                         xch ? xch->counts : nullptr, xch ? xch->global_rays_per_frame : 0, host_iter });
        rc = check_launch("render_image_test (composite / schedule)");
        if (rc) return rc;
    }
    const int enqueued = it;
    hipLaunchKernelGGL(frame_finalize_kernel, grd, blk, 0, stream, n_rays, bkgd, rgb, opacity, depth);
    rc = check_launch("render_image_test (finalize)");
    if (rc) return rc;
    std::vector<IterPlan> plans;
    int n_iters = 0;
    rc = read_back_plans(W.plans, enqueued, stream, "render_image_test (read-back)", who, plans, n_iters);
    if (rc) return rc;
    int64_t total[kMaxFrames] = { 0 };
    for (int k = 0; k < n_iters; ++k) {
        const IterPlan &P = plans[k];
        int64_t alive_total = 0, samples_it = 0;
        int max_limit = 0;
        for (int f = 0; f < n_frames; ++f) {
            alive_total += P.count[f];
            samples_it += (int64_t)(P.next[f] >> 32);
            total[f] += (int64_t)(P.next[f] >> 32);
            if (P.count[f] > 0 && P.limit[f] > max_limit) max_limit = P.limit[f];
        }
        if (trace && k < trace->capacity) {
            if (trace->iter_alive) trace->iter_alive[k] = alive_total;
            if (trace->iter_n_samples) trace->iter_n_samples[k] = max_limit;
            if (trace->iter_samples) trace->iter_samples[k] = samples_it;
        }
    }
    if (trace) trace->n_iters = n_iters;
    if (total_samples_out)
        for (int f = 0; f < n_frames; ++f) total_samples_out[f] = total[f];
    return CED_OK;
}

struct ImageWorkspace {
    ImageState st;
    int32_t *packed, *alive_a, *alive_b;
    IterPlan *plans;
    float *t0, *t1; int32_t *ridx; float *sigma, *rgbs, *w, *tr, *al; int32_t *rank;
    size_t bytes;
};

constexpr int kImageMaxIters = 1024;

static ImageWorkspace carve_image(void *base, int64_t n, int64_t cap)
{
    ImageWorkspace w{};
    Carver c{ (char *)base };
    w.st.cursor = c.take<int32_t>((size_t)n);
    w.st.acc_all = c.take<float>((size_t)n);
    w.st.acc_kept = c.take<float>((size_t)n);
    w.packed = c.take<int32_t>((size_t)n * 2);
    w.alive_a = c.take<int32_t>((size_t)n);
    w.alive_b = c.take<int32_t>((size_t)n);
    w.plans = c.take<IterPlan>((size_t)kImageMaxIters + 2);
    w.t0 = c.take<float>((size_t)cap);
    w.t1 = c.take<float>((size_t)cap);
    w.ridx = c.take<int32_t>((size_t)cap);
    w.sigma = c.take<float>((size_t)cap);
    w.rgbs = c.take<float>((size_t)cap * 3);
    w.w = c.take<float>((size_t)cap);
    w.tr = c.take<float>((size_t)cap);
    w.al = c.take<float>((size_t)cap);
    w.rank = c.take<int32_t>((size_t)cap);
    w.bytes = c.off;
    return w;
}

static inline int64_t image_capacity(int64_t n_rays, int64_t n_all) { return n_all + 64; }

static int render_image_impl(const ced_field_desc *field, int64_t n_rays, const float *rays_o, const float *rays_d,
                             int64_t n_all, const int64_t *packed_all, const float *t0_all, const float *t1_all,
                             float early_stop_eps, float alpha_thre, const float *timestamps, int32_t t_per_ray,
                             const float *bkgd, float *rgb, float *opacity, float *depth, int32_t *kept, void *workspace,
                             int64_t workspace_bytes, int64_t *host_stats, int64_t *stats_out, void *field_stream_,
                             void *stream_)
{
    const char *who = "render_image";
    hipStream_t stream = (hipStream_t)stream_;
    hipStream_t fstream = field_stream_ ? (hipStream_t)field_stream_ : stream;
    CED_REQUIRE(fstream == stream, "%s: a separate field stream is not supported", who);
    CED_REQUIRE(field != nullptr, "%s: null field descriptor", who);
    CED_REQUIRE(n_rays >= 0 && n_all >= 0, "%s: bad sizes", who);
    CED_REQUIRE(n_rays < (1ll << 31) / 4 && n_all < (1ll << 31) - 128, "%s: too many rays / samples for 32-bit indices", who);
    if (stats_out) { stats_out[0] = 0; stats_out[1] = 0; stats_out[2] = 0; }
    if (n_rays == 0) return CED_OK;
    const bool full = rgb != nullptr;
    CED_REQUIRE(rays_o && rays_d && packed_all && (n_all == 0 || (t0_all && t1_all)) && timestamps && kept && workspace &&
                    host_stats && (!full || (opacity && depth)),
                "%s: null pointer", who);
    const int64_t cap = image_capacity(n_rays, n_all);
    ImageWorkspace W = carve_image(workspace, n_rays, cap);
    W.st.kept = kept;
    CED_REQUIRE((int64_t)W.bytes <= workspace_bytes, "%s: workspace too small (%lld < %lld bytes)", who,
                (long long)workspace_bytes, (long long)W.bytes);
    const dim3 blk(256), grd((unsigned)((n_rays + 255) / 256));
    hipLaunchKernelGGL(image_prep_kernel, grd, blk, 0, stream, n_rays, W.st, rgb, opacity, depth);
    volatile long long *pub = (volatile long long *)host_stats;
    std::vector<long long> plan_seq((size_t)kImageMaxIters + 1);
    plan_seq[0] = ++g_publish_seq;
    const int big = 1 << 30;
    const int min_chunk = full ? 4 : 8;
    hipLaunchKernelGGL(frame_init_kernel, dim3(1), dim3(64), 0, stream,
                       ScheduleArgs{ W.plans, -1, 1, (int)n_rays, min_chunk, big, (long long *)host_stats, plan_seq[0] }, (float *)nullptr,
                       (unsigned long long *)nullptr, 0);
    int rc = check_launch("render_image (prep)");
    if (rc) return rc;
    long long alive_bound = n_rays;
    int it = 0;
    for (; it < kImageMaxIters; ++it) {
        bool stop = false;
        rc = run_ahead(pub, nullptr, plan_seq, it, stream, who, stop, alive_bound);
        if (rc) return rc;
        if (stop) break;
        IterPlan *plan = W.plans + it;
        const int32_t *cur_list = it == 0 ? nullptr : ((it & 1) ? W.alive_a : W.alive_b);
        int32_t *next_list = (it & 1) ? W.alive_b : W.alive_a;
        int64_t mgrid = (alive_bound + kMarchThreads - 1) / kMarchThreads;
        if (mgrid > 8192) mgrid = 8192;
        if (mgrid < 1) mgrid = 1;
        hipLaunchKernelGGL(image_chunk_kernel, dim3((unsigned)mgrid), dim3(kMarchThreads), 0, stream, plan, n_all, cur_list,
                           packed_all, t0_all, t1_all, W.st.cursor, W.t0, W.t1, W.ridx, W.packed);
        FieldArgs F{};
        F.n = n_rays * (int64_t)min_chunk;
        F.n_dev = &plan->total_samples;
        F.base_dev = &plan->sample_base;
        F.rays_o = rays_o; F.rays_d = rays_d; F.ray_idx32 = W.ridx;
        F.t0 = W.t0; F.t1 = W.t1;
        F.timestamps = timestamps;
        F.rays_mode = 1; F.t_per_ray = t_per_ray ? 1 : 0; F.want_rgb = full ? 1 : 0;
        F.rgb = full ? W.rgbs : nullptr; F.sigma = W.sigma; F.geo = nullptr;
        rc = launch_field(field, F, (void *)stream);
        if (rc) return rc;
        int64_t cgrid = (alive_bound + kCompositeThreads - 1) / kCompositeThreads;
        if (cgrid > 4096) cgrid = 4096;
        if (cgrid < 1) cgrid = 1;
        plan_seq[it + 1] = ++g_publish_seq;
        if (full)
            hipLaunchKernelGGL(image_composite_kernel<true>, dim3((unsigned)cgrid), dim3(kCompositeThreads), 0, stream, plan,
                               cur_list, next_list, W.packed, packed_all, W.t0, W.t1, W.sigma, W.rgbs, W.st, W.w, W.tr, W.al,
                               W.rank, rgb, opacity, depth, early_stop_eps, alpha_thre, n_all);
        else
            hipLaunchKernelGGL(image_composite_kernel<false>, dim3((unsigned)cgrid), dim3(kCompositeThreads), 0, stream, plan,
                               cur_list, next_list, W.packed, packed_all, W.t0, W.t1, W.sigma, (const float *)nullptr, W.st,
                               (float *)nullptr, (float *)nullptr, (float *)nullptr, W.rank, (float *)nullptr,
                               (float *)nullptr, (float *)nullptr, early_stop_eps, alpha_thre, n_all);
        hipLaunchKernelGGL(frame_schedule_kernel, dim3(1), dim3(64), 0, stream,
                           ScheduleArgs{ W.plans, it, 1, (int)n_rays, min_chunk, big, (long long *)host_stats, plan_seq[it + 1] });
        rc = check_launch("render_image (iteration)");
        if (rc) return rc;
    }
    const int enqueued = it;
    if (full) hipLaunchKernelGGL(frame_finalize_kernel, grd, blk, 0, stream, n_rays, bkgd, rgb, opacity, depth);
    rc = check_launch("render_image (finalize)");
    if (rc) return rc;
    std::vector<IterPlan> plans;
    int n_iters = 0;
    rc = read_back_plans(W.plans, enqueued, stream, "render_image (read-back)", who, plans, n_iters);
    if (rc) return rc;
    int64_t processed = 0, kept_total = 0;
    for (int k = 0; k < n_iters; ++k) {
        processed = plans[k].sample_base + plans[k].total_samples;
        kept_total += (int64_t)plans[k].next[1];
    }
    CED_REQUIRE(processed <= cap, "%s: internal: %lld samples processed, capacity %lld", who, (long long)processed, (long long)cap);
    if (stats_out) { stats_out[0] = processed; stats_out[1] = n_iters; stats_out[2] = kept_total; }
    return CED_OK;
}

}

extern "C" int64_t ced_render_image_test_workspace_bytes(int64_t n_rays, int32_t n_grids, int32_t res,
                                                         float cone_angle, int32_t max_samples)
{
    if (n_rays < 0 || n_grids < 1 || n_grids > ced::kMaxGrids || res < 1 || res > 1024 || max_samples < 0) return -1;
    const int ms = ced::min_samples_of(cone_angle);
    return (int64_t)ced::carve(nullptr, n_rays, n_grids, n_rays * ms, ced::max_iterations(max_samples, ms), res).bytes;
}

extern "C" int ced_render_image_test(const ced_field_desc *field, int64_t n_rays, const float *rays_o,
                                     const float *rays_d, const uint8_t *binaries, int32_t n_grids, int32_t res,
                                     const float *aabbs, const void *accel, float near_plane, float far_plane,
                                     float step_size, float cone_angle, float early_stop_eps, int32_t max_samples,
                                     const float *timestamps, int32_t t_per_ray, const float *bkgd, float *rgb,
                                     float *opacity, float *depth, void *workspace, int64_t workspace_bytes,
                                     int64_t *host_stats, int64_t *total_samples_out, ced_frame_trace *trace,
                                     void *field_stream_, void *stream_)
{
    return ced::render_frames_impl(field, 1, n_rays, rays_o, rays_d, binaries, n_grids, res, aabbs, accel, near_plane,
                                   far_plane, step_size, cone_angle, early_stop_eps, max_samples, timestamps, t_per_ray,
                                   nullptr, bkgd, rgb, opacity, depth, workspace, workspace_bytes, host_stats,
                                   total_samples_out, trace, field_stream_, stream_, "render_image_test");
}

extern "C" int64_t ced_render_frames_test_workspace_bytes(int32_t n_frames, int64_t rays_per_frame, int32_t n_grids,
                                                          int32_t res, float cone_angle, int32_t max_samples)
{
    if (n_frames < 1 || n_frames > ced::kMaxFrames || rays_per_frame < 0 || n_grids < 1 || n_grids > ced::kMaxGrids ||
        res < 1 || res > 1024 || max_samples < 0)
        return -1;
    const int64_t n_rays = (int64_t)n_frames * rays_per_frame;
    const int ms = ced::min_samples_of(cone_angle);
    return (int64_t)ced::carve(nullptr, n_rays, n_grids, n_rays * ms, ced::max_iterations(max_samples, ms), res, true).bytes;
}

extern "C" int ced_render_frames_test(const ced_field_desc *field, int32_t n_frames, int64_t rays_per_frame,
                                      const float *rays_o, const float *rays_d, const uint8_t *binaries, int32_t n_grids,
                                      int32_t res, const float *aabbs, const void *accel, float near_plane,
                                      float far_plane, float step_size, float cone_angle, float early_stop_eps,
                                      int32_t max_samples, const float *frame_times, const float *bkgd, float *rgb,
                                      float *opacity, float *depth, void *workspace, int64_t workspace_bytes,
                                      int64_t *host_stats, int64_t *total_samples_out, ced_frame_trace *trace,
                                      void *field_stream_, void *stream_)
{
    CED_REQUIRE(frame_times != nullptr, "render_frames_test: null frame_times");
    return ced::render_frames_impl(field, n_frames, rays_per_frame, rays_o, rays_d, binaries, n_grids, res, aabbs, accel,
                                   near_plane, far_plane, step_size, cone_angle, early_stop_eps, max_samples, nullptr, 0,
                                   frame_times, bkgd, rgb, opacity, depth, workspace, workspace_bytes, host_stats,
                                   total_samples_out, trace, field_stream_, stream_, "render_frames_test");
}


extern "C" int64_t ced_render_frames_test_sharded_workspace_bytes(int32_t n_frames, int64_t rays_per_frame,
                                                                  int64_t global_rays_per_frame, int32_t n_grids,
                                                                  int32_t res, float cone_angle, int32_t max_samples)
{
    if (n_frames < 1 || n_frames > ced::kMaxFrames || rays_per_frame < 0 || global_rays_per_frame < rays_per_frame ||
        n_grids < 1 || n_grids > ced::kMaxGrids || res < 1 || res > 1024 || max_samples < 0)
        return -1;
    const int64_t n_rays = (int64_t)n_frames * rays_per_frame;
    const int ms = ced::min_samples_of(cone_angle);
    return (int64_t)ced::carve(nullptr, n_rays, n_grids, ced::sample_capacity(n_frames, rays_per_frame, ms, global_rays_per_frame),
                               ced::max_iterations(max_samples, ms), res, true).bytes;
}

extern "C" int32_t ced_render_frames_test_iterations(float cone_angle, int32_t max_samples)
{
    if (max_samples < 0) return -1;
    return ced::max_iterations(max_samples, ced::min_samples_of(cone_angle));
}

extern "C" int64_t ced_render_frames_test_host_bytes(float cone_angle, int32_t max_samples)
{
    if (max_samples < 0) return -1;
    const int64_t iters = ced::max_iterations(max_samples, ced::min_samples_of(cone_angle));
    return (ced::kHostIterWord + 3 * (iters + 2)) * (int64_t)sizeof(int64_t);
}

extern "C" int ced_render_frames_test_sharded(const ced_field_desc *field, int32_t n_frames, int64_t rays_per_frame,
                                              const float *rays_o, const float *rays_d, const uint8_t *binaries,
                                              int32_t n_grids, int32_t res, const float *aabbs, const void *accel,
                                              float near_plane, float far_plane, float step_size, float cone_angle,
                                              float early_stop_eps, int32_t max_samples, const float *frame_times,
                                              const float *bkgd, float *rgb, float *opacity, float *depth, void *workspace,
                                              int64_t workspace_bytes, int64_t *host_stats, int64_t *total_samples_out,
                                              ced_frame_trace *trace, void *field_stream_, void *stream_,
                                              const ced_shard_exchange *exchange)
{
    CED_REQUIRE(frame_times != nullptr, "render_frames_test_sharded: null frame_times");
    return ced::render_frames_impl(field, n_frames, rays_per_frame, rays_o, rays_d, binaries, n_grids, res, aabbs, accel,
                                   near_plane, far_plane, step_size, cone_angle, early_stop_eps, max_samples, nullptr, 0,
                                   frame_times, bkgd, rgb, opacity, depth, workspace, workspace_bytes, host_stats,
                                   total_samples_out, trace, field_stream_, stream_, "render_frames_test_sharded", exchange);
}

extern "C" int64_t ced_render_image_workspace_bytes(int64_t n_rays, int64_t n_all)
{
    if (n_rays < 0 || n_all < 0) return -1;
    return (int64_t)ced::carve_image(nullptr, n_rays, ced::image_capacity(n_rays, n_all)).bytes;
}

extern "C" int ced_render_image(const ced_field_desc *field, int64_t n_rays, const float *rays_o, const float *rays_d,
                                int64_t n_all, const int64_t *packed_info, const float *t_starts, const float *t_ends,
                                float early_stop_eps, float alpha_thre, const float *timestamps, int32_t t_per_ray,
                                const float *bkgd, float *rgb, float *opacity, float *depth, int32_t *kept,
                                void *workspace, int64_t workspace_bytes, int64_t *host_stats, int64_t *stats_out,
                                void *field_stream, void *stream)
{
    return ced::render_image_impl(field, n_rays, rays_o, rays_d, n_all, packed_info, t_starts, t_ends, early_stop_eps,
                                  alpha_thre, timestamps, t_per_ray, bkgd, rgb, opacity, depth, kept, workspace,
                                  workspace_bytes, host_stats, stats_out, field_stream, stream);
}

extern "C" int ced_render_image_gather(int64_t n_rays, int64_t n_all, int64_t processed, const void *workspace,
                                       int64_t workspace_bytes, const int64_t *ray_offsets, int64_t chunk_rays,
                                       int64_t *ray_indices, float *t_starts, float *t_ends, float *sigmas, float *rgbs,
                                       float *weights, float *trans, float *alphas, void *stream)
{
    CED_REQUIRE(n_rays >= 0 && n_all >= 0 && processed >= 0, "render_image_gather: bad sizes");
    if (processed == 0) return CED_OK;
    CED_REQUIRE(workspace && ray_offsets && ray_indices && t_starts && t_ends, "render_image_gather: null pointer");
    CED_REQUIRE((rgbs && weights && trans && alphas) || (!rgbs && !weights && !trans && !alphas),
                "render_image_gather: rgbs / weights / trans / alphas go together");
    const ced::ImageWorkspace W = ced::carve_image(const_cast<void *>(workspace), n_rays, ced::image_capacity(n_rays, n_all));
    CED_REQUIRE((int64_t)W.bytes <= workspace_bytes && processed <= ced::image_capacity(n_rays, n_all),
                "render_image_gather: workspace does not match");
    int64_t grid = (processed + 255) / 256;
    if (grid > 16384) grid = 16384;
    hipLaunchKernelGGL(ced::image_gather_kernel, dim3((unsigned)grid), dim3(256), 0, (hipStream_t)stream, processed, W.rank,
                       W.ridx, W.t0, W.t1, W.sigma, W.rgbs, W.w, W.tr, W.al, ray_offsets, chunk_rays,
                       ced::ImageOut{ ray_indices, t_starts, t_ends, sigmas, rgbs, weights, trans, alphas });
    return ced::check_launch("render_image_gather");
}


extern "C" int ced_march_all(int64_t n_rays, const float *rays_o, const float *rays_d, const uint8_t *binaries,
                             int32_t n_grids, int32_t res, const float *aabbs, const void *accel, const float *near_planes,
                             float far_plane, float step_size, float cone_angle, const float *t_sorted,
                             const int64_t *t_indices, const uint8_t *hits, int32_t fill, int64_t *packed_info,
                             float *t_starts, float *t_ends, int64_t *ray_indices, int64_t capacity, int64_t *total,
                             void *stream)
{
    CED_REQUIRE(n_rays >= 0 && res >= 1 && res <= 1024 && n_grids >= 1 && n_grids <= ced::kMaxGrids, "march_all: bad sizes");
    if (n_rays == 0) return CED_OK;
    CED_REQUIRE(rays_o && rays_d && binaries && aabbs && accel && near_planes && packed_info, "march_all: null pointer");
    CED_REQUIRE(n_grids == 1 || (t_sorted && t_indices && hits), "march_all: %d grid levels need the sorted intersections", n_grids);
// ... 27 lines not shown
```

ced_nerf_amd/dist.py:

```python
from __future__ import annotations

from typing import Callable, Dict, Optional

import numpy as np
import torch
import torch.distributed as dist

TILE = 8


_assignment_cache: Dict = {}


def tile_cyclic_assignment(n_frames: int, height: int, width: int, world: int, tile: int = TILE):
    key = (n_frames, height, width, world, tile)
    if key not in _assignment_cache:
        if len(_assignment_cache) > 16:
            _assignment_cache.clear()
        _assignment_cache[key] = _tile_cyclic_assignment(n_frames, height, width, world, tile)
    return _assignment_cache[key]


def _tile_cyclic_assignment(n_frames: int, height: int, width: int, world: int, tile: int):
    ty = (np.arange(height) // tile)[:, None]
    tx = (np.arange(width) // tile)[None, :]
    tiles_x = (width + tile - 1) // tile
    tiles_y = (height + tile - 1) // tile
    tile_id = ty * tiles_x + tx
    ids = (np.arange(n_frames)[:, None, None] * (tiles_x * tiles_y) + tile_id[None]).reshape(-1)
    owner = (ids % world).astype(np.int32)
    order = np.argsort(ids, kind="stable")
    shards = [order[owner[order] == r] for r in range(world)]
    return owner, shards


class ShardedRenderer:

    def __init__(self, field, estimator, world: int, rank: int, device, max_samples: int = 1024,
                 render_kwargs: Optional[Dict] = None, render_fn: Optional[Callable] = None,
                 force_collective: bool = False, tile_order: bool = False, units: int = 1, schedule_group=None):
        self.field, self.estimator = field, estimator
        self.world, self.rank, self.device = world, rank, device
        self.max_samples = max_samples
        self.render_kwargs = dict(render_kwargs or {})
        self.render_fn = render_fn or self._hip_render
        self.shape = None
        self.tracer = None
        self.field_max_workgroups = 0
        self.field_stream = None
        self.force_collective = force_collective
        self.tile_order = tile_order
        self.unpermute = None
        self.units = int(units)
        assert 1 <= self.units <= 64, "units must be 1..64"
        self.schedule_group = schedule_group
        self.exchange = None
        self.exchange_issuer = None
        self.sharded = False

    def _hip_render(self, rays_o, rays_d, timestamps):
        from .utils import Rays, render_frames_test, render_image_test
        if self.sharded:
            F = self.shape[0]
            ts = timestamps.reshape(-1).float()
            ts = ts.expand(F).contiguous() if ts.numel() == 1 else ts
            if self.exchange is None:
                from . import ops
                H, W = self.shape[1], self.shape[2]
                self.exchange = ops.ScheduleExchange(F, H * W, self.local_real, rays_o.device, self.max_samples,
                                                     float(self.render_kwargs.get("cone_angle", 0.0)),
                                                     group=self.schedule_group)
            self.exchange.issuer = self.exchange_issuer
            rgb, op, dp, totals = render_frames_test(
                self.max_samples, self.field, self.estimator, Rays(rays_o.view(F, -1, 3), rays_d.view(F, -1, 3)), timestamps=ts,
                tracer=self.tracer, field_max_workgroups=self.field_max_workgroups, exchange=self.exchange,
                **self.render_kwargs)
            return rgb.view(-1, 3), op.view(-1, 1), dp.view(-1, 1), sum(totals)
        if self.units == 1:
            return render_image_test(self.max_samples, self.field, self.estimator, Rays(rays_o, rays_d),
                                     timestamps=timestamps, tracer=self.tracer, field_stream=self.field_stream,
                                     field_max_workgroups=self.field_max_workgroups, **self.render_kwargs)
        u = self.units
        ts = timestamps.reshape(-1).float()
        ts = ts.expand(u).contiguous() if ts.numel() == 1 else ts
        rgb, op, dp, totals = render_frames_test(
            self.max_samples, self.field, self.estimator, Rays(rays_o.view(u, -1, 3), rays_d.view(u, -1, 3)), timestamps=ts,
            tracer=self.tracer, field_stream=self.field_stream, field_max_workgroups=self.field_max_workgroups,
            **self.render_kwargs)
        return rgb.view(-1, 3), op.view(-1, 1), dp.view(-1, 1), sum(totals)

    def set_rays(self, origins: torch.Tensor, viewdirs: torch.Tensor) -> None:
        assert origins.ndim == 4 and origins.shape == viewdirs.shape, "rays must be [F,H,W,3]"
        F, H, W, _ = origins.shape
        o = origins.reshape(-1, 3); d = viewdirs.reshape(-1, 3)
        if self.shape == (F, H, W) and getattr(self, "_ray_index", None) is not None and self._ray_index.device == o.device:
            self.local_o, self.local_d = o[self._ray_index].contiguous(), d[self._ray_index].contiguous()
            return
        self.shape = (F, H, W)
        self._ray_index = None
        self.exchange = None
        self.sharded = self.world > 1 or self.force_collective
        if not self.sharded:
            if self.units > 1 and F % self.units:
                raise ValueError(f"{F} frames do not split into {self.units} equal groups")
            self.n_local = self.n_pad = o.shape[0]
            self.gather_index = None
            if self.tile_order:
                _, shards = tile_cyclic_assignment(F, H, W, 1)
                order = torch.from_numpy(shards[0].astype(np.int64)).to(o.device)
                self.local_o, self.local_d = o[order].contiguous(), d[order].contiguous()
                inv = torch.empty_like(order)
                inv[order] = torch.arange(order.numel(), device=o.device)
                self.unpermute = inv
                self._ray_index = order
            else:
                self.local_o, self.local_d = o.contiguous(), d.contiguous()
                self.unpermute = None
            return
        if F > 64:
            raise ValueError("at most 64 frames per sharded call")
        _, shards = tile_cyclic_assignment(F, H, W, self.world)
        n_img = H * W
        per = [[s[(s >= f * n_img) & (s < (f + 1) * n_img)] for f in range(F)] for s in shards]
        self.n_unit = max(1, max(len(x) for row in per for x in row))
        mine = per[self.rank]
        self.local_real = [len(x) for x in mine]
        self.n_local = int(sum(self.local_real))
        self.n_pad = F * self.n_unit
        self.global_rays = n_img

        def padded(x):
            fill = x[-1:] if len(x) else np.zeros((1,), np.int64)
            return np.concatenate([x, np.repeat(fill, self.n_unit - len(x))])
        idx = np.concatenate([padded(x) for x in mine])
        idx_t = torch.from_numpy(idx.astype(np.int64)).to(o.device)
        self._ray_index = idx_t
        self.local_o = o[idx_t].contiguous()
        self.local_d = d[idx_t].contiguous()
        n_rays = F * n_img
        dest = np.full((self.world, F, self.n_unit), n_rays, np.int64)
        for r in range(self.world):
            for f in range(F):
                dest[r, f, :len(per[r][f])] = per[r][f]
        dest = np.concatenate([dest.reshape(self.world, -1), np.full((self.world, 1), n_rays, np.int64)], axis=1)
        self.gather_index = torch.from_numpy(dest.reshape(-1)).to(o.device)

    @torch.no_grad()
    def render_local(self, timestamps: torch.Tensor):
        rgb, op, dp, n_samples = self.render_fn(self.local_o, self.local_d, timestamps)
        return rgb, op, dp, int(n_samples)

    @torch.no_grad()
    def gather(self, local, sync_total: bool = True) -> Dict:
        F, H, W = self.shape
        rgb, op, dp, n_samples = local
        if self.gather_index is None:
            if self.unpermute is not None:
                if rgb.is_cuda:
                    from . import ops
                    rgb, op, dp, _ = ops.scatter_pixels(self._ray_index, F * H * W, rgb.reshape(-1, 3), op.reshape(-1, 1),
                                                        dp.reshape(-1, 1))
                else:
                    rgb, op, dp = rgb[self.unpermute], op[self.unpermute], dp[self.unpermute]
            return dict(rgb=rgb.view(F, H, W, 3), opacity=op.view(F, H, W, 1), depth=dp.view(F, H, W, 1),
                        local_samples=n_samples, total_samples=n_samples)
        payload = torch.empty((self.n_pad + 1, 5), device=rgb.device, dtype=torch.float32)
        payload[:-1, 0:3] = rgb.reshape(-1, 3)
        payload[:-1, 3:4] = op.reshape(-1, 1)
        payload[:-1, 4:5] = dp.reshape(-1, 1)
        payload[-1].zero_()
        payload[-1, 0] = float(n_samples >> 16)
        payload[-1, 1] = float(n_samples & 0xFFFF)
        gathered = torch.empty((self.world, self.n_pad + 1, 5), device=rgb.device, dtype=torch.float32)
        if payload.is_cuda and dist.get_backend(self.schedule_group) == "gloo":
            parts = [torch.empty((self.n_pad + 1, 5), dtype=torch.float32) for _ in range(self.world)]
            dist.all_gather(parts, payload.cpu(), group=self.schedule_group)
            gathered.copy_(torch.stack(parts))
        else:
            dist.all_gather_into_tensor(gathered.view(-1, 5), payload, group=self.schedule_group)
        tail = gathered[:, -1, :2].to(torch.float64)
        total_t = (tail[:, 0] * 65536.0 + tail[:, 1]).sum()
        total = int(total_t.item()) if sync_total else None
        n_rays = F * H * W
        rows = gathered.view(-1, 5)
        if rows.is_cuda:
            from . import ops
            o_rgb, o_op, o_dp, _ = ops.scatter_pixels(self.gather_index, n_rays, rows[:, 0:3], rows[:, 3:4], rows[:, 4:5])
        else:
            image = torch.empty((n_rays + 1, 5), dtype=torch.float32)
            image[self.gather_index] = rows
            o_rgb, o_op, o_dp = image[:n_rays, 0:3], image[:n_rays, 3:4], image[:n_rays, 4:5]
        return dict(rgb=o_rgb.reshape(F, H, W, 3), opacity=o_op.reshape(F, H, W, 1), depth=o_dp.reshape(F, H, W, 1),
                    local_samples=n_samples, total_samples=total, total_samples_tensor=total_t)

    @torch.no_grad()
    def render(self, timestamps: torch.Tensor) -> Dict:
        return self.gather(self.render_local(timestamps))


def _all_reduce_on(row: torch.Tensor, stream: int, group) -> None:
    if not row.is_cuda:
        dist.all_reduce(row, op=dist.ReduceOp.SUM, group=group)
        return
    ext = torch.cuda.ExternalStream(stream, device=row.device) if stream else torch.cuda.current_stream(row.device)
    with torch.cuda.stream(ext):
        dist.all_reduce(row, op=dist.ReduceOp.SUM, group=group)


class ExchangeTimeout(RuntimeError):
    """A lane or the collecting thread of a PipelinedRenderer waited longer than `comm_timeout_s` for its counterpart."""


class PipelinedRenderer:

    def __init__(self, lanes, share_field_stream: bool = False, async_gather: bool = False,
                 field_max_blocks: Optional[int] = 128, comm_timeout_s: Optional[float] = None):
        import os
        from concurrent.futures import ThreadPoolExecutor
        self.lanes = list(lanes)
        self.field_max_blocks = field_max_blocks if len(self.lanes) > 1 else None
        if self.field_max_blocks is not None:
            for lane in self.lanes:
                lane.field_max_workgroups = int(self.field_max_blocks)
        self.async_gather = bool(async_gather)
        self.comm_timeout_s = float(comm_timeout_s if comm_timeout_s is not None else os.environ.get("CED_COMM_TIMEOUT_S", "120"))
        self.comm_stream = None
        self.streams = [torch.cuda.Stream(device=l.device) if torch.cuda.is_available() and str(l.device) != "cpu"
                        else None for l in self.lanes]
        self.pool = ThreadPoolExecutor(max_workers=len(self.lanes)) if len(self.lanes) > 1 else None
        collective = [l for l in self.lanes if getattr(l, "world", 1) > 1 or getattr(l, "force_collective", False)]
        if self.pool is not None and collective:
            groups = {id(getattr(l, "schedule_group", None)) for l in self.lanes}
            if len(groups) != 1:
                raise ValueError("PipelinedRenderer: the lanes use different process groups; every lane's collectives are "
                                 "issued by ONE thread on ONE communicator (pass the same schedule_group, or None, to all)")
            for i, lane in enumerate(self.lanes):
                lane.exchange_issuer = self._issuer_of_lane(i)
                if getattr(lane, "exchange", None) is not None:
                    lane.exchange.issuer = lane.exchange_issuer
        self._msgq = None
        self._abort = None
        self._where = None
        if share_field_stream and self.pool is not None and self.streams[0] is not None:
            self.field_stream = torch.cuda.Stream(device=self.lanes[0].device)
            for lane in self.lanes:
                lane.field_stream = self.field_stream

    def _issuer_of_lane(self, i):
        import threading

        def issue(exchange, row, stream, iteration):
            if self._abort is not None:
                raise self._abort
            q = self._msgq
            if q is None:
                _all_reduce_on(row, stream, exchange.group)
                return
            ack, box = threading.Event(), {}
            q[i].put(("reduce", iteration, row, stream, exchange.group, ack, box))
            waited = 0.0
            while not ack.wait(0.05):
                waited += 0.05
                if self._abort is not None:
                    raise self._abort
                if waited >= self.comm_timeout_s:
                    raise ExchangeTimeout(f"lane {i}: the survivor-count all-reduce of iteration {iteration} was not issued within "
                                          f"{self.comm_timeout_s:.0f} s; the collecting thread is waiting for (lane, step) {self._where}")
            if "error" in box:
                raise box["error"]
        return issue

    def _lane(self, i, timestamps):
        lane, stream = self.lanes[i], self.streams[i]
        if stream is None:
            return lane.render_local(timestamps)
        with torch.cuda.stream(stream):
            return lane.render_local(timestamps)

    @torch.no_grad()
    def render(self, timestamps: torch.Tensor):
# ... 113 lines not shown
```

ced_nerf_amd/ops.py:

```python
from __future__ import annotations

import ctypes as C
from typing import Dict, Optional, Tuple

import numpy as np
import torch

from . import _lib, profiling
from .hashgrid import level_tables


def _stream() -> C.c_void_p:
    return C.c_void_p(torch.cuda.current_stream().cuda_stream)


def _chk(t: Optional[torch.Tensor], dtype: torch.dtype, name: str, allow_none: bool = False):
    if t is None:
        if allow_none:
            return None
        raise ValueError(f"{name} is required")
    if not t.is_cuda:
        raise NotImplementedError(f"Only support cuda inputs ({name} is on {t.device}).")
    _check_current_device(t.device.index, name)
    if t.dtype != dtype:
# ... 790 lines not shown
                            _p(timestamps), int(bool(t_per_ray)), _p(bkgd), *(map(_p, pixels) if full else (None,) * 3),
                            _p(kept), _p(ws[0]), ws[0].numel(), C.c_void_p(ws[1].data_ptr()), stats, None, _stream())
    mode = "" if full else " (sampling)"
    _lib.check(rc, "render_image" + mode)
    processed = int(stats[0])
    offsets = torch.zeros((n + 1,), device=dev, dtype=torch.int64)
    torch.cumsum(kept, 0, out=offsets[1:])
    total = int(stats[2])
    extras = {"ray_indices": torch.empty((total,), device=dev, dtype=torch.int64), "t_starts": f(total), "t_ends": f(total)}
    if full:
        extras.update(sigmas=f(total), rgbs=f(total, 3), weights=f(total), trans=f(total), alphas=f(total))
    if total > 0:
        names = ("ray_indices", "t_starts", "t_ends", "sigmas", "rgbs", "weights", "trans", "alphas")
        rc = L.ced_render_image_gather(n, n_all, processed, _p(ws[0]), ws[0].numel(), _p(offsets), int(chunk_rays),
                                       *(_p(extras.get(k)) for k in names), _stream())
        _lib.check(rc, "render_image_gather" + mode)
    return pixels, extras, offsets, (processed, int(stats[1]))


def render_image_eval_native(desc: _lib.FieldDesc, rays_o, rays_d, packed_info, t_starts, t_ends, early_stop_eps,
                             alpha_thre, timestamps, t_per_ray, bkgd, chunk_rays: int = 0, max_workgroups: int = 0):
    _chk(bkgd, torch.float32, "render_bkgd", allow_none=True)
    assert rays_o.ndim == 2 and rays_o.shape[1] == 3 and rays_o.shape == rays_d.shape
    (rgb, opacity, depth), extras, offsets, stats = _render_image(
        desc, rays_o, rays_d, packed_info, t_starts, t_ends, early_stop_eps, alpha_thre, timestamps, t_per_ray, bkgd,
        True, chunk_rays, max_workgroups)
    return rgb, opacity, depth, extras, offsets, stats


def sampling_native(desc: _lib.FieldDesc, rays_o, rays_d, packed_info, t_starts, t_ends, early_stop_eps, alpha_thre,
                    timestamps, t_per_ray, max_workgroups: int = 0):
    _, extras, _, _ = _render_image(desc, rays_o, rays_d, packed_info, t_starts, t_ends, early_stop_eps, alpha_thre,
                                    timestamps, t_per_ray, None, False, 0, max_workgroups)
    return extras["ray_indices"], extras["t_starts"], extras["t_ends"]


class ScheduleExchange:

    def __init__(self, n_frames: int, global_rays: int, local_rays, device, max_samples: int, cone_angle: float,
                 group=None, reduce_fn=None):
        import torch.distributed as dist
        L = _lib.lib()
        self.n_frames = int(n_frames)
        self.iterations = int(L.ced_render_frames_test_iterations(float(cone_angle), int(max_samples)))
        self.host_words = (int(L.ced_render_frames_test_host_bytes(float(cone_angle), int(max_samples))) + 7) // 8
        self.counts = torch.zeros((self.iterations + 1, self.n_frames), device=device, dtype=torch.int64)
        self.local_rays = torch.as_tensor(local_rays, dtype=torch.int32).reshape(-1).to(device).contiguous()
        assert self.local_rays.numel() == self.n_frames
        self.group, self.error, self.calls = group, None, 0
        self._reduce_fn = reduce_fn
        self.issuer = None

        def _cb(user, counts_ptr, n_counts, iteration, stream):
            try:
                row = self.counts[iteration]
                assert row.data_ptr() == counts_ptr and n_counts == self.n_frames
                if self.issuer is not None and self._reduce_fn is None:
                    self.issuer(self, row, stream or 0, iteration)
                    self.calls += 1
                    return 0
                cur = torch.cuda.current_stream(row.device)
                if cur.cuda_stream != (stream or 0):
                    cur = torch.cuda.ExternalStream(stream, device=row.device)
                with torch.cuda.stream(cur):
                    if self._reduce_fn is not None:
                        self._reduce_fn(row)
                    else:
                        dist.all_reduce(row, op=dist.ReduceOp.SUM, group=self.group)
                self.calls += 1
                return 0
            except BaseException as e:
                self.error = e
                return 1

        self._cb = _lib.EXCHANGE_FN(_cb)
        self.struct = _lib.ShardExchange(int(global_rays), C.c_void_p(self.local_rays.data_ptr()),
                                         C.c_void_p(self.counts.data_ptr()), self._cb, None)


def render_frames_test_native(desc: _lib.FieldDesc, n_frames: int, rays_o, rays_d, binaries, aabbs, near_plane, far_plane,
                              render_step_size, cone_angle, early_stop_eps, max_samples, frame_times, bkgd,
                              tracer: Optional[FrameTracer] = None, field_stream: Optional[torch.cuda.Stream] = None,
                              accel: Optional[torch.Tensor] = None, max_workgroups: int = 0,
                              exchange: Optional[ScheduleExchange] = None):
    _chk(rays_o, torch.float32, "rays_o"); _chk(rays_d, torch.float32, "rays_d")
    _chk(aabbs, torch.float32, "aabbs"); _chk(frame_times, torch.float32, "frame_times")
    _chk(bkgd, torch.float32, "render_bkgd", allow_none=True)
    assert rays_o.ndim == 2 and rays_o.shape[1] == 3 and rays_o.shape == rays_d.shape
    assert binaries.is_cuda and binaries.is_contiguous() and binaries.ndim == 4
    n = rays_o.shape[0]
    assert n_frames >= 1 and n % n_frames == 0, "rays must hold n_frames equal frames"
    assert frame_times.numel() == n_frames, "one time per frame"
    m, res = binaries.shape[0], binaries.shape[1]
    assert aabbs.shape == (m, 6)
    dev = rays_o.device
    L = _lib.lib()
    if exchange is None:
        need = int(L.ced_render_frames_test_workspace_bytes(n_frames, n // n_frames, m, res, float(cone_angle), int(max_samples)))
    else:
        need = int(L.ced_render_frames_test_sharded_workspace_bytes(n_frames, n // n_frames, int(exchange.struct.global_rays_per_frame),
                                                                    m, res, float(cone_angle), int(max_samples)))
    if need < 0:
        raise ValueError("render_frames_test: unsupported sizes (1..64 frames)")
    host_words = 512 if exchange is None else max(512, exchange.host_words)
    ws = _cached_workspace(_frame_ws, dev, torch.cuda.current_stream().cuda_stream, need, host_words)
    rgb = torch.empty((n, 3), device=dev, dtype=torch.float32)
    opacity = torch.empty((n, 1), device=dev, dtype=torch.float32)
    depth = torch.empty((n, 1), device=dev, dtype=torch.float32)
    totals = (C.c_int64 * n_frames)()
    args = (C.byref(_with_workgroups(desc, max_workgroups)), n_frames, n // n_frames, _p(rays_o),
            _p(rays_d), _p(_as_u8(binaries)), m, res, _p(aabbs), _p(accel), float(near_plane), float(far_plane), float(render_step_size),
            float(cone_angle), float(early_stop_eps), int(max_samples), _p(frame_times), _p(bkgd),
            _p(rgb), _p(opacity), _p(depth), _p(ws[0]), ws[0].numel(), C.c_void_p(ws[1].data_ptr()),
            totals, C.byref(tracer.struct) if tracer is not None else None,
            C.c_void_p(field_stream.cuda_stream) if field_stream is not None else None, _stream())
    if exchange is None:
        rc = L.ced_render_frames_test(*args)
    else:
        assert exchange.n_frames == n_frames and exchange.counts.device == dev
        exchange.error = None
        rc = L.ced_render_frames_test_sharded(*args, C.byref(exchange.struct))
        if exchange.error is not None:
            raise exchange.error
    _lib.check(rc, "render_frames_test")
    return rgb, opacity, depth, [int(v) for v in totals]


def occ_cell_points(cell_indices: torch.Tensor, noise: torch.Tensor, res: int, aabb) -> torch.Tensor:
    _chk(cell_indices, torch.int64, "cell_indices"); _chk(noise, torch.float32, "noise")
    n = cell_indices.shape[0]
    assert noise.shape == (n, 3)
    pos = torch.empty((n, 3), device=cell_indices.device, dtype=torch.float32)
    ab = (C.c_float * 6)(*[float(v) for v in aabb])
    rc = _lib.lib().ced_occ_cell_points(n, _p(cell_indices), _p(noise), int(res), ab, _p(pos), _stream())
    _lib.check(rc, "occ_cell_points")
    return pos


def occ_ema_update_(occs: torch.Tensor, cell_ids: torch.Tensor, density: torch.Tensor, step_size: float,
                    ema_decay: float) -> None:
    _chk(occs, torch.float32, "occs"); _chk(cell_ids, torch.int64, "cell_ids"); _chk(density, torch.float32, "density")
    assert density.shape == cell_ids.shape
    rc = _lib.lib().ced_occ_ema_update(cell_ids.shape[0], _p(cell_ids), _p(density), float(step_size), float(ema_decay),
                                       _p(occs), _stream())
    _lib.check(rc, "occ_ema_update")
```

ced_nerf_amd/utils.py:

```python
from __future__ import annotations

import collections
import random
from typing import Optional

import numpy as np
import torch

from . import ops
from .nerfacc_api import OccGridEstimator, march_packed, ray_aabb_intersect, sort_intersections
from .render import rendering

Rays = collections.namedtuple("Rays", ("origins", "viewdirs"))


def namedtuple_map(fn, tup):
    return type(tup)(*(None if x is None else fn(x) for x in tup))


def set_random_seed(seed):
    random.seed(seed)
    np.random.seed(seed)
    torch.manual_seed(seed)

# ... 109 lines not shown

        def rgb_sigma_fn(t_starts, t_ends, ray_indices):
            return radiance_field.query_rays(chunk_rays.origins, chunk_rays.viewdirs, ray_indices, t_starts, t_ends,
                                             ts, want_rgb=True)

        ray_indices, t_starts, t_ends = estimator.sampling(
            chunk_rays.origins, chunk_rays.viewdirs, sigma_fn=sigma_fn, near_plane=near_plane, far_plane=far_plane,
            render_step_size=render_step_size, stratified=training, cone_angle=cone_angle, alpha_thre=alpha_thre,
            sigma_field=(radiance_field, ts, training) if two_pass else None)
        rgb, opacity, depth, extras = rendering(t_starts, t_ends, ray_indices, n_rays=n_pass,
                                                rgb_sigma_fn=rgb_sigma_fn, render_bkgd=render_bkgd)
        extras["ray_indices"] = ray_indices
        extras["t_starts"] = t_starts
        extras["t_ends"] = t_ends
        if training or n_pass <= test_chunk_size:
            results.append([rgb, opacity, depth, len(t_starts)])
            extra_info.append(extras)
            continue
        starts = list(range(0, n_pass, test_chunk_size)) + [n_pass]
        bounds = torch.searchsorted(ray_indices, torch.tensor(starts, device=rgb.device)).tolist()
        sizes = [bounds[c + 1] - bounds[c] for c in range(len(starts) - 1)]
        extras["ray_indices"] = ray_indices % test_chunk_size
        cut = {k: v.split(sizes) for k, v in extras.items()}
        results.append([rgb, opacity, depth, len(t_starts)])
        extra_info.extend([{k: cut[k][c] for k in cut} for c in range(len(sizes))])
    colors, opacities, depths, n_rendering_samples = [
        torch.cat(r, dim=0) if isinstance(r[0], torch.Tensor) else r for r in zip(*results)
    ]
    return (colors.view((*rays_shape[:-1], -1)), opacities.view((*rays_shape[:-1], -1)),
            depths.view((*rays_shape[:-1], -1)), sum(n_rendering_samples), extra_info)


@torch.no_grad()
def render_image_test(
    max_samples: int,
    radiance_field: torch.nn.Module,
    estimator: OccGridEstimator,
    rays: Rays,
    near_plane: float = 0.0,
    far_plane: float = 1e10,
    render_step_size: float = 1e-3,
    render_bkgd: Optional[torch.Tensor] = None,
    cone_angle: float = 0.0,
    alpha_thre: float = 0.0,
    early_stop_eps: float = 1e-4,
    timestamps: Optional[torch.Tensor] = None,
    tracer=None,
    field_stream=None,
    field_max_workgroups: int = 0,
):
    if timestamps is None:
        raise NotImplementedError("DNGPradianceField needs timestamps (dnerf path of cednerf/utils.py:186-194)")
    rays, rays_shape, N_rays = _flatten_rays(rays)
    rays_o = rays.origins.contiguous().float()
    rays_d = rays.viewdirs.contiguous().float()
    bk = None if render_bkgd is None else render_bkgd.to(rays_o.device, torch.float32).reshape(-1).contiguous()
    ts = timestamps.reshape(-1).float().contiguous()
    rgb, opacity, depth, total = ops.render_image_test_native(
        radiance_field._descriptor(), rays_o, rays_d, estimator.binaries, estimator.aabbs.contiguous(), near_plane,
        far_plane, render_step_size, cone_angle, early_stop_eps, max_samples, ts, bool(radiance_field.training), bk,
        tracer=tracer, field_stream=field_stream, accel=estimator.occupancy_accel(), max_workgroups=field_max_workgroups)
    return (rgb.view((*rays_shape[:-1], -1)), opacity.view((*rays_shape[:-1], -1)),
            depth.view((*rays_shape[:-1], -1)), total)


@torch.no_grad()
def render_frames_test(
    max_samples: int,
    radiance_field: torch.nn.Module,
    estimator: OccGridEstimator,
    rays: Rays,
    near_plane: float = 0.0,
    far_plane: float = 1e10,
    render_step_size: float = 1e-3,
    render_bkgd: Optional[torch.Tensor] = None,
    cone_angle: float = 0.0,
    alpha_thre: float = 0.0,
    early_stop_eps: float = 1e-4,
    timestamps: Optional[torch.Tensor] = None,
    tracer=None,
    field_stream=None,
    field_max_workgroups: int = 0,
    exchange=None,
):
    if timestamps is None:
        raise NotImplementedError("DNGPradianceField needs timestamps (dnerf path of cednerf/utils.py:186-194)")
    if radiance_field.training:
        raise NotImplementedError("render_frames_test renders eval frames (one time per frame)")
    shape = tuple(rays.origins.shape)
    assert len(shape) >= 3 and shape[-1] == 3 and tuple(rays.viewdirs.shape) == shape, "rays must be [F, ..., 3]"
    n_frames = shape[0]
    rays_o = rays.origins.reshape(-1, 3).contiguous().float()
    rays_d = rays.viewdirs.reshape(-1, 3).contiguous().float()
    bk = None if render_bkgd is None else render_bkgd.to(rays_o.device, torch.float32).reshape(-1).contiguous()
    ts = timestamps.reshape(-1).float().contiguous()
    assert ts.numel() == n_frames, "one timestamp per frame"
    rgb, opacity, depth, totals = ops.render_frames_test_native(
        radiance_field._descriptor(), n_frames, rays_o, rays_d, estimator.binaries, estimator.aabbs.contiguous(),
        near_plane, far_plane, render_step_size, cone_angle, early_stop_eps, max_samples, ts, bk,
        tracer=tracer, field_stream=field_stream, accel=estimator.occupancy_accel(), max_workgroups=field_max_workgroups,
        exchange=exchange)
    return rgb.view((*shape[:-1], 3)), opacity.view((*shape[:-1], 1)), depth.view((*shape[:-1], 1)), totals


@torch.no_grad()
def render_image_test_staged(
    max_samples: int,
    radiance_field: torch.nn.Module,
    estimator: OccGridEstimator,
    rays: Rays,
    near_plane: float = 0.0,
    far_plane: float = 1e10,
    render_step_size: float = 1e-3,
    render_bkgd: Optional[torch.Tensor] = None,
    cone_angle: float = 0.0,
    alpha_thre: float = 0.0,
    early_stop_eps: float = 1e-4,
    timestamps: Optional[torch.Tensor] = None,
):
    if timestamps is None:
        raise NotImplementedError("DNGPradianceField needs timestamps (dnerf path of cednerf/utils.py:186-194)")
    rays, rays_shape, N_rays = _flatten_rays(rays)
    rays_o = rays.origins.contiguous().float()
    rays_d = rays.viewdirs.contiguous().float()
    device = rays_o.device
    opacity = torch.zeros(N_rays, 1, device=device)
    depth = torch.zeros(N_rays, 1, device=device)
    rgb = torch.zeros(N_rays, 3, device=device)
    ray_mask = torch.ones(N_rays, device=device).bool()
    min_samples = 1 if cone_angle == 0 else 4
    iter_samples = total_samples = 0
    near_planes = torch.full_like(rays_o[..., 0], fill_value=near_plane)
    far_planes = torch.full_like(rays_o[..., 0], fill_value=far_plane)
    aabbs = estimator.aabbs.contiguous()
    t_mins, t_maxs, hits = ray_aabb_intersect(rays_o, rays_d, aabbs)
    t_sorted, t_indices = sort_intersections(t_mins, t_maxs)
    opc_thres = 1 - early_stop_eps
    op_flat, dp_flat = opacity.view(-1), depth.view(-1)
    binaries = estimator.binaries
    stats = torch.zeros((max(int(max_samples), 1) + 1, 2), device=device, dtype=torch.int64)
    host_stats = torch.zeros((2,), dtype=torch.int64).pin_memory()
    stream = torch.cuda.current_stream()
    N_alive = N_rays
    it = 0
    while iter_samples < max_samples:
        if N_alive == 0:
            break
        N_samples = max(min(N_rays // N_alive, 64), min_samples)
        iter_samples += N_samples
        bound = N_alive * N_samples
        counts = torch.empty((N_rays,), device=device, dtype=torch.int64)
        march = (rays_o, rays_d, binaries, aabbs, near_planes, far_planes, render_step_size, cone_angle, N_samples,
                 ray_mask, t_sorted, t_indices, hits)
        ops.traverse_grids_raw(*march, 0, counts=counts)
        incl = torch.cumsum(counts, 0)
        t_starts = torch.empty((bound,), device=device, dtype=torch.float32)
        t_ends = torch.empty((bound,), device=device, dtype=torch.float32)
        ray_indices = torch.empty((bound,), device=device, dtype=torch.int64)
        packed_info = torch.empty((N_rays, 2), device=device, dtype=torch.int64)
        ops.traverse_grids_raw(*march, 3, base=incl, counts=counts, t_starts=t_starts, t_ends=t_ends,
                               ray_indices=ray_indices, termination_planes=near_planes, packed_info_out=packed_info)
        rgbs, sigmas = radiance_field.query_rays(rays_o, rays_d, ray_indices, t_starts, t_ends, timestamps,
                                                 want_rgb=True, n_dev=incl[-1:])
        ops.composite_step_(packed_info, t_starts, t_ends, sigmas, rgbs, rgb, op_flat, dp_flat, opc_thres, N_samples,
                            ray_mask, stats[it])
        host_stats.copy_(stats[it], non_blocking=True)
        stream.synchronize()
        N_alive = int(host_stats[0])
        total_samples += int(host_stats[1])
        it += 1

    bk = None if render_bkgd is None else render_bkgd.to(device, torch.float32).reshape(-1).contiguous()
    ops.finalize_pixels_(bk, rgb, op_flat, dp_flat)
    return (rgb.view((*rays_shape[:-1], -1)), opacity.view((*rays_shape[:-1], -1)),
            depth.view((*rays_shape[:-1], -1)), total_samples)


render_image_with_occgrid = render_image
```

include/cednerf_hip.h:

```cpp
#ifndef CEDNERF_HIP_H
#define CEDNERF_HIP_H

#include <stddef.h>
#include <stdint.h>

#ifdef __cplusplus
extern "C" {
#endif

#define CED_MAX_LEVELS 16

#define CED_OK 0
#define CED_E_INVALID (-1)
#define CED_E_LAUNCH (-2)
#define CED_E_UNSUPPORTED (-3)

typedef struct ced_hash_desc {
    int32_t n_levels;
    int32_t table_dtype;
    int32_t temporal;
    int32_t reserved;
    float scale[CED_MAX_LEVELS];
    uint32_t res[CED_MAX_LEVELS];
    uint32_t offset[CED_MAX_LEVELS];
// ... 169 lines not shown
                        float *depth, void *stream);


int ced_occ_cell_points(int64_t n, const int64_t *cell_indices, const float *noise, int32_t res,
                        const float *aabb_host, float *positions, void *stream);

int ced_occ_ema_update(int64_t n, const int64_t *cell_ids, const float *density, float step_size,
                       float ema_decay, float *occs, void *stream);


int ced_generate_rays_pinhole(int32_t width, int32_t height, float fx, float fy, float cx, float cy,
                              const float *c2w_host, int32_t opengl, float *origins, float *viewdirs,
                              float *directions, void *stream);

int ced_generate_rays_hypercam(int32_t width, int32_t height, const float *orientation_host,
                               const float *position_host, float focal_length, float principal_x, float principal_y,
                               float skew, float pixel_aspect_ratio, const float *radial3_host,
                               const float *tangential2_host, float *origins, float *viewdirs, void *stream);

#define CED_CAMERA_PINHOLE 0
#define CED_CAMERA_HYPERCAM 1
#define CED_PINHOLE_FLOATS 17
#define CED_HYPERCAM_FLOATS 22
#define CED_VIEW_PER_RAY 0
#define CED_VIEW_PER_STEP 1
#define CED_BKGD_WHITE 0
#define CED_BKGD_BLACK 1
#define CED_BKGD_RANDOM 2
int ced_sample_training_batch(int32_t camera_model, int32_t n_views, int32_t width, int32_t height, int32_t channels,
                              const uint8_t *images, const float *cameras, const float *view_timestamps,
                              int64_t num_rays, uint64_t seed, int64_t step, int32_t view_mode, int32_t bkgd_mode,
                              float *origins, float *viewdirs, float *pixels, float *timestamps, float *color_bkgd,
                              int32_t *indices, void *stream);

int64_t ced_importance_batch_workspace_bytes(int64_t n_cells, int64_t pool_size, int64_t num_cells);
int ced_sample_importance_batch(int32_t camera_model, int32_t n_views, int32_t width, int32_t height, int32_t channels,
                                const uint8_t *images, const float *cameras, const float *view_timestamps,
                                const float *weights, int32_t weights_subsampled, int64_t pool_size, int64_t num_cells,
                                uint64_t seed, int64_t step, int32_t bkgd_mode, float *origins, float *viewdirs,
                                float *pixels, float *timestamps, float *color_bkgd, int32_t *indices, uint32_t *min_key,
                                void *workspace, int64_t workspace_bytes, void *stream);

int ced_temporal_median_u8(int32_t n_cameras, int32_t n_frames, int32_t height, int32_t width, const uint8_t *images,
                           uint8_t *median, void *stream);
int ced_isg_weights(int32_t n_cameras, int32_t n_frames, int32_t height, int32_t width, const uint8_t *images,
                    const uint8_t *median, float gamma, float *weights, void *stream);
int ced_ist_weights(int32_t n_cameras, int32_t n_frames, int32_t height, int32_t width, const uint8_t *images,
                    float alpha, int32_t frame_shift, float *weights, void *stream);

typedef struct ced_frame_trace {
    int32_t capacity;
    int32_t n_iters;
    void **field_begin;
    void **field_end;
    int64_t *iter_alive;
    int64_t *iter_n_samples;
    int64_t *iter_samples;
    uint64_t *field_stamps;
} ced_frame_trace;

int64_t ced_wall_clock_khz(void);

int64_t ced_render_image_test_workspace_bytes(int64_t n_rays, int32_t n_grids, int32_t res, float cone_angle,
                                              int32_t max_samples);

int ced_render_image_test(const ced_field_desc *field, int64_t n_rays, const float *rays_o, const float *rays_d,
                          const uint8_t *binaries, int32_t n_grids, int32_t res, const float *aabbs, const void *accel,
                          float near_plane, float far_plane, float render_step_size, float cone_angle,
                          float early_stop_eps, int32_t max_samples,
                          const float *timestamps, int32_t t_per_ray, const float *bkgd,
                          float *rgb, float *opacity, float *depth,
                          void *workspace, int64_t workspace_bytes, int64_t *host_stats,
                          int64_t *total_samples_out, ced_frame_trace *trace, void *field_stream, void *stream);

int64_t ced_render_frames_test_workspace_bytes(int32_t n_frames, int64_t rays_per_frame, int32_t n_grids, int32_t res,
                                               float cone_angle, int32_t max_samples);
int ced_render_frames_test(const ced_field_desc *field, int32_t n_frames, int64_t rays_per_frame,
                           const float *rays_o, const float *rays_d, const uint8_t *binaries, int32_t n_grids,
                           int32_t res, const float *aabbs, const void *accel, float near_plane, float far_plane,
                           float render_step_size, float cone_angle, float early_stop_eps, int32_t max_samples,
                           const float *frame_times, const float *bkgd, float *rgb, float *opacity, float *depth,
                           void *workspace, int64_t workspace_bytes, int64_t *host_stats,
                           int64_t *total_samples_out, ced_frame_trace *trace, void *field_stream, void *stream);

typedef int (*ced_exchange_fn)(void *user, int64_t *counts, int32_t n_counts, int32_t iteration, void *stream);
typedef struct ced_shard_exchange {
    int64_t global_rays_per_frame;
    const int32_t *local_rays;
    int64_t *counts;
    ced_exchange_fn reduce;
    void *user;
} ced_shard_exchange;
int64_t ced_render_frames_test_sharded_workspace_bytes(int32_t n_frames, int64_t rays_per_frame,
                                                       int64_t global_rays_per_frame, int32_t n_grids, int32_t res,
                                                       float cone_angle, int32_t max_samples);
int32_t ced_render_frames_test_iterations(float cone_angle, int32_t max_samples);
int64_t ced_render_frames_test_host_bytes(float cone_angle, int32_t max_samples);
int ced_render_frames_test_sharded(const ced_field_desc *field, int32_t n_frames, int64_t rays_per_frame,
                                   const float *rays_o, const float *rays_d, const uint8_t *binaries, int32_t n_grids,
                                   int32_t res, const float *aabbs, const void *accel, float near_plane, float far_plane,
                                   float render_step_size, float cone_angle, float early_stop_eps, int32_t max_samples,
                                   const float *frame_times, const float *bkgd, float *rgb, float *opacity, float *depth,
                                   void *workspace, int64_t workspace_bytes, int64_t *host_stats,
                                   int64_t *total_samples_out, ced_frame_trace *trace, void *field_stream, void *stream,
                                   const ced_shard_exchange *exchange);

int64_t ced_render_image_workspace_bytes(int64_t n_rays, int64_t n_all);
int ced_render_image(const ced_field_desc *field, int64_t n_rays, const float *rays_o, const float *rays_d,
                     int64_t n_all, const int64_t *packed_info, const float *t_starts, const float *t_ends,
                     float early_stop_eps, float alpha_thre, const float *timestamps, int32_t t_per_ray,
                     const float *bkgd, float *rgb, float *opacity, float *depth, int32_t *kept, void *workspace,
                     int64_t workspace_bytes, int64_t *host_stats, int64_t *stats_out, void *field_stream, void *stream);
int ced_render_image_gather(int64_t n_rays, int64_t n_all, int64_t processed, const void *workspace,
                            int64_t workspace_bytes, const int64_t *ray_offsets, int64_t chunk_rays,
                            int64_t *ray_indices, float *t_starts, float *t_ends, float *sigmas, float *rgbs,
                            float *weights, float *trans, float *alphas, void *stream);

int ced_march_all(int64_t n_rays, const float *rays_o, const float *rays_d, const uint8_t *binaries, int32_t n_grids,
                  int32_t res, const float *aabbs, const void *accel, const float *near_planes, float far_plane,
                  float render_step_size, float cone_angle, const float *t_sorted, const int64_t *t_indices,
                  const uint8_t *hits, int32_t fill, int64_t *packed_info, float *t_starts, float *t_ends,
                  int64_t *ray_indices, int64_t capacity, int64_t *total, void *stream);

int ced_mlp_chain(int64_t n, int32_t n_layers, int32_t backward, const float *x, const int32_t *widths,
                  const float *const *weights, float *const *outs, const float *const *masks, int32_t relu_last,
                  void *stream);

int64_t ced_mlp_backward_dw_workspace_bytes(int64_t n, int32_t n_layers, const int32_t *widths);
int ced_mlp_backward_dw(int64_t n, int32_t n_layers, const float *dy, const int32_t *widths,
                        const float *const *weights, const float *const *acts, float *g0, float *dws, void *workspace,
                        int64_t workspace_bytes, void *stream);

int ced_train_inputs(int64_t n, const float *rays_o, const float *rays_d, const int64_t *ray_indices,
                     const float *t_starts, const float *t_ends, const float *timestamps, const float *positions,
                     const float *directions, float *pos_out, float *enc_out, float *sh_out, float *t_out, void *stream);
int ced_train_warp(int64_t n, const float *pos, const float *mo, int32_t mo_width, int32_t use_div_offsets,
                   float moving_step, const float *aabb_host, float *xn, float *move, float *selector, void *stream);
int ced_train_warp_backward(int64_t n, const float *pos, const float *mo, int32_t mo_width, int32_t use_div_offsets,
                            float moving_step, const float *aabb_host, const float *d_xn, const float *d_move,
                            float *d_mo, void *stream);
int ced_train_head_in(int64_t n, const float *bout, const float *sh, const float *selector, float *head_in,
                      float *sigma, void *stream);
int ced_train_head_in_backward(int64_t n, const float *bout, const float *selector, const float *d_head_in,
                               const float *d_sigma, float *d_bout, void *stream);

#ifdef __cplusplus
}
#endif
#endif
```

Before: 4.517 billion.

## Precompute per-ray SH direction, fuse unpermute into finalize, derive frame index by magic division

The frame prep kernels now compute the normalized SH direction components once per ray and store them, so field kernels load them instead of recomputing the norm and division per sample. Per-ray timestamps are replaced by a frame index computed with multiply-high division, which removes the frame_times kernel and buffer. The finalize kernel scatters results straight to raster positions through a pixel index, skipping a separate unpermute pass. The first composite iteration skips reading zeroed accumulators, at the cost of an extra per-ray SH buffer and more code paths.

After: 4.504 billion. No clear change (-0.3%).

```diff
diff --git a/ced_nerf_amd/_lib.py b/ced_nerf_amd/_lib.py
--- a/ced_nerf_amd/_lib.py
+++ b/ced_nerf_amd/_lib.py
@@ -126,6 +126,10 @@
     "ced_render_frames_test": (C.c_int, [C.POINTER(FieldDesc), _i32, _i64, _vp, _vp, _vp, _i32, _i32, _vp, _vp, _f, _f, _f, _f,
                                          _f, _i32, _vp, _vp, _vp, _vp, _vp, _vp, _i64, _vp, C.POINTER(_i64),
                                          C.POINTER(FrameTrace), _vp, _vp]),
+    "ced_render_frames_test_raster": (C.c_int, [C.POINTER(FieldDesc), _i32, _i64, _vp, _vp, _vp, _i32, _i32, _vp, _vp, _f, _f, _f,
+                                                _f, _f, _i32, _vp, _vp, _vp, _vp, _vp, _vp, _i64, _vp, C.POINTER(_i64),
+                                                C.POINTER(FrameTrace), _vp, _vp, _vp]),
+    "ced_host_frames_of_rays": (C.c_int, [_i64, _vp, _i64, _vp]),
     "ced_render_frames_test_sharded_workspace_bytes": (_i64, [_i32, _i64, _i64, _i32, _i32, _f, _i32]),
     "ced_render_frames_test_iterations": (_i32, [_f, _i32]),
     "ced_render_frames_test_host_bytes": (_i64, [_f, _i32]),
diff --git a/ced_nerf_amd/csrc/field_args.hpp b/ced_nerf_amd/csrc/field_args.hpp
--- a/ced_nerf_amd/csrc/field_args.hpp
+++ b/ced_nerf_amd/csrc/field_args.hpp
@@ -12,12 +12,18 @@
     const int64_t *n_dev;
     unsigned long long *stamp;
     const int64_t *base_dev;
-    const float *pos, *t, *dir;
+    const float *pos, *t;
+    union {
+        const float *dir;
+        const float *ray_sh;
+    };
     const float *rays_o, *rays_d;
     const int64_t *ray_idx;
     const int32_t *ray_idx32;
     const float *t0, *t1, *timestamps;
     int rays_mode, t_per_ray, want_rgb;
+    uint32_t frame_mul;
+    int frame_shift;
     float *rgb, *sigma, *geo;
     float aabb[6];
     float moving_step;
@@ -31,6 +37,50 @@
     float scale[CED_MAX_LEVELS];
     uint32_t res[CED_MAX_LEVELS], offset[CED_MAX_LEVELS], size[CED_MAX_LEVELS], hashed[CED_MAX_LEVELS];
 };
+
+struct FrameDiv {
+    uint32_t mul;
+    int shift;
+};
+
+__host__ __device__ __forceinline__ uint32_t frame_of_ray(uint32_t r, uint32_t mul, int shift)
+{
+#if defined(__HIP_DEVICE_COMPILE__)
+    return __umulhi(r, mul) >> shift;
+#else
+    return (uint32_t)(((uint64_t)r * mul) >> 32) >> shift;
+#endif
+}
+
+inline bool make_frame_div(int64_t d, FrameDiv &out)
+{
+    if (d < 2 || d >= (1ll << 31)) return false;
+    int l = 1;
+    while ((1ll << l) < d) ++l;
+    const uint64_t pow = 1ull << (31 + l);
+    const uint64_t mul = (pow + (uint64_t)d - 1) / (uint64_t)d;
+    if (mul >= (1ull << 32)) return false;
+    const uint64_t md = mul * (uint64_t)d;
+    if (md < pow || md > pow + (1ull << l)) return false;
+    out.mul = (uint32_t)mul;
+    out.shift = l - 1;
+    const uint64_t top = (1ull << 31) - 1;
+    const uint64_t edge = top / (uint64_t)d * (uint64_t)d;
+    const uint64_t probe[5] = { 0, (uint64_t)d - 1, (uint64_t)d, edge - 1, top };
+    for (uint64_t r : probe)
+        if (frame_of_ray((uint32_t)r, out.mul, out.shift) != (uint32_t)(r / (uint64_t)d)) return false;
+    return frame_of_ray((uint32_t)edge, out.mul, out.shift) == (uint32_t)(edge / (uint64_t)d);
+}
+
+__device__ __forceinline__ float dir_norm(const float dv[3])
+{
+    return __builtin_sqrtf((dv[0] * dv[0] + dv[1] * dv[1]) + dv[2] * dv[2]);
+}
+__device__ __forceinline__ float sh_dir_component(float comp, float nrm)
+{
+    const float u = (comp / nrm + 1.0f) / 2.0f;
+    return u * 2.0f - 1.0f;
+}
 
 extern std::atomic<int> g_march_two_pass;
 extern std::atomic<int> g_field_spread_tiles;
diff --git a/ced_nerf_amd/csrc/field_half.hip b/ced_nerf_amd/csrc/field_half.hip
--- a/ced_nerf_amd/csrc/field_half.hip
+++ b/ced_nerf_amd/csrc/field_half.hip
@@ -116,7 +116,8 @@
                 const float tm2 = used ? A.t0[sbase + s] + A.t1[sbase + s] : 0.0f;
 #pragma unroll
                 for (int a = 0; a < 3; ++a) px[j][a] = A.rays_o[3 * r + a] + (A.rays_d[3 * r + a] * tm2) / 2.0f;
-                tq[j] = A.t_per_ray ? A.timestamps[r] : A.timestamps[0];
+                tq[j] = A.t_per_ray ? A.timestamps[A.t_per_ray == 2 ? (int64_t)frame_of_ray((uint32_t)r, A.frame_mul, A.frame_shift) : r]
+                                    : A.timestamps[0];
             } else {
                 ridx[j] = s;
 #pragma unroll
@@ -242,14 +243,18 @@
         if (A.want_rgb) {
 #pragma unroll
             for (int j = 0; j < NT; ++j) {
-                float dv[3];
-#pragma unroll
-                for (int a = 0; a < 3; ++a)
-                    dv[a] = A.rays_mode ? A.rays_d[3 * ridx[j] + a] : A.dir[3 * (tile_base + sofs[j]) + a];
-                const float nrm = __builtin_sqrtf((dv[0] * dv[0] + dv[1] * dv[1]) + dv[2] * dv[2]);
-                const float comp = (g == 1) ? dv[1] : (g == 2) ? dv[2] : dv[0];
-                const float u = (comp / nrm + 1.0f) / 2.0f;
-                const float vv = u * 2.0f - 1.0f;
+                const int ca = (g == 1) ? 1 : (g == 2) ? 2 : 0;
+                float vv;
+                if (A.rays_mode && A.ray_sh) {
+                    vv = A.ray_sh[3 * ridx[j] + ca];
+                } else {
+                    float dv[3];
+#pragma unroll
+                    for (int a = 0; a < 3; ++a)
+                        dv[a] = A.rays_mode ? A.rays_d[3 * ridx[j] + a] : A.dir[3 * (tile_base + sofs[j]) + a];
+                    const float comp = (g == 1) ? dv[1] : (g == 2) ? dv[2] : dv[0];
+                    vv = sh_dir_component(comp, dir_norm(dv));
+                }
                 const float coef = (g == 2) ? 0.48860251190291987f : -0.48860251190291987f;
                 const float sh = (g == 0) ? 0.28209479177387814f : coef * vv;
                 float hin[8];
diff --git a/ced_nerf_amd/csrc/field_kernel.hpp b/ced_nerf_amd/csrc/field_kernel.hpp
--- a/ced_nerf_amd/csrc/field_kernel.hpp
+++ b/ced_nerf_amd/csrc/field_kernel.hpp
@@ -140,7 +140,6 @@
         int lds_off = 0;
         asm volatile("" : "+v"(lds_off));
         const float *const lw = lds + lds_off;
-        int64_t sidx[NT];
         int64_t ridx[NT];
         float px[NT][3], tq[NT];
         bool any_used = !A.rays_mode;
@@ -148,7 +147,6 @@
         for (int j = 0; j < NT; ++j) {
             int64_t s = tile * TILE + 16 * j + c;
             s = s < n_eff ? s : n_eff - 1;
-            sidx[j] = s;
             if (A.rays_mode) {
                 const int64_t r_in = A.ray_idx32 ? (int64_t)A.ray_idx32[sbase + s] : A.ray_idx[sbase + s];
                 const bool used = r_in >= 0;
@@ -158,7 +156,8 @@
                 const float tm2 = used ? A.t0[sbase + s] + A.t1[sbase + s] : 0.0f;
 #pragma unroll
                 for (int a = 0; a < 3; ++a) px[j][a] = A.rays_o[3 * r + a] + (A.rays_d[3 * r + a] * tm2) / 2.0f;
-                tq[j] = A.t_per_ray ? A.timestamps[r] : A.timestamps[0];
+                tq[j] = A.t_per_ray ? A.timestamps[A.t_per_ray == 2 ? (int64_t)frame_of_ray((uint32_t)r, A.frame_mul, A.frame_shift) : r]
+                                    : A.timestamps[0];
             } else {
                 ridx[j] = s;
 #pragma unroll
@@ -301,16 +300,15 @@
                 const _Float16 *const hw = reinterpret_cast<const _Float16 *>(lw + BL::H0);
                 const _Float16 *const hwl = hw + BL::HEAD_FRAGS * kFragHalves;
                 h8 Bh[NT][2], Bl[NT][2];
+                const bool sh_ready = A.rays_mode && A.ray_sh;
+                const float *const dsrc = A.rays_mode ? (sh_ready ? A.ray_sh : A.rays_d) : A.dir;
 #pragma unroll
                 for (int j = 0; j < NT; ++j) {
                     float dv[3];
 #pragma unroll
-                    for (int a = 0; a < 3; ++a)
-                        dv[a] = A.rays_mode ? A.rays_d[3 * ridx[j] + a] : A.dir[3 * sidx[j] + a];
-                    const float nrm = __builtin_sqrtf((dv[0] * dv[0] + dv[1] * dv[1]) + dv[2] * dv[2]);
-                    const float comp = (g == 1) ? dv[1] : (g == 2) ? dv[2] : dv[0];
-                    const float u = (comp / nrm + 1.0f) / 2.0f;
-                    const float vv = u * 2.0f - 1.0f;
+                    for (int a = 0; a < 3; ++a) dv[a] = dsrc[3 * ridx[j] + a];
+                    float vv = (g == 1) ? dv[1] : (g == 2) ? dv[2] : dv[0];
+                    if (!sh_ready) vv = sh_dir_component(vv, dir_norm(dv));
                     const float coef = (g == 2) ? 0.48860251190291987f : -0.48860251190291987f;
                     float hin[8];
                     hin[0] = (g == 0) ? 0.28209479177387814f : coef * vv;
@@ -339,17 +337,25 @@
         }
 
         if (A.want_rgb) {
+            constexpr bool kRaySh = !(TE && TEMPORAL && !F16);
+            const bool sh_ready = kRaySh && A.rays_mode && A.ray_sh;
+            const float *const dsrc = !kRaySh ? nullptr : A.rays_mode ? (sh_ready ? A.ray_sh : A.rays_d) : A.dir;
 #pragma unroll
             for (int j = 0; j < NT; ++j) {
                 const float geo_tail = (g == 3) ? 0.0f : D[j][0][0];
-                float dv[3];
-#pragma unroll
-                for (int a = 0; a < 3; ++a)
-                    dv[a] = A.rays_mode ? A.rays_d[3 * ridx[j] + a] : A.dir[3 * sidx[j] + a];
-                const float nrm = __builtin_sqrtf((dv[0] * dv[0] + dv[1] * dv[1]) + dv[2] * dv[2]);
-                const float comp = (g == 1) ? dv[1] : (g == 2) ? dv[2] : dv[0];
-                const float u = (comp / nrm + 1.0f) / 2.0f;
-                const float vv = u * 2.0f - 1.0f;
+                float dv[3], vv;
+                if constexpr (kRaySh) {
+#pragma unroll
+                    for (int a = 0; a < 3; ++a) dv[a] = dsrc[3 * ridx[j] + a];
+                    vv = (g == 1) ? dv[1] : (g == 2) ? dv[2] : dv[0];
+                    if (__builtin_expect(!sh_ready, 0)) vv = sh_dir_component(vv, dir_norm(dv));
+                } else {
+                    const int64_t s = tile * TILE + 16 * j + c;
+#pragma unroll
+                    for (int a = 0; a < 3; ++a)
+                        dv[a] = A.rays_mode ? A.rays_d[3 * ridx[j] + a] : A.dir[3 * (s < n_eff ? s : n_eff - 1) + a];
+                    vv = sh_dir_component((g == 1) ? dv[1] : (g == 2) ? dv[2] : dv[0], dir_norm(dv));
+                }
                 const float coef = (g == 2) ? 0.48860251190291987f : -0.48860251190291987f;
                 B[j][0] = (g == 0) ? 0.28209479177387814f : coef * vv;
                 B[j][1] = D[j][0][1];
diff --git a/ced_nerf_amd/csrc/frame.hip b/ced_nerf_amd/csrc/frame.hip
--- a/ced_nerf_amd/csrc/frame.hip
+++ b/ced_nerf_amd/csrc/frame.hip
@@ -155,11 +155,12 @@
     return block_base + wave_cnt[wave] + __builtin_popcountll(ballot & ((1ull << lane) - 1ull));
 }
 
-__global__ __launch_bounds__(256) void frame_times_kernel(int64_t n_rays, int rays_per_frame,
-                                                          const float *__restrict__ frame_times, float *__restrict__ ts_ray)
-{
-    const int64_t r = (int64_t)blockIdx.x * blockDim.x + threadIdx.x;
-    if (r < n_rays) ts_ray[r] = frame_times[r / rays_per_frame];
+__device__ __forceinline__ void store_ray_sh(int64_t r, const float *__restrict__ rays_d, float *__restrict__ ray_sh)
+{
+    const float dv[3] = { rays_d[3 * r], rays_d[3 * r + 1], rays_d[3 * r + 2] };
+    const float nrm = dir_norm(dv);
+#pragma unroll
+    for (int a = 0; a < 3; ++a) ray_sh[3 * r + a] = sh_dir_component(dv[a], nrm);
 }
 
 __global__ __launch_bounds__(256) void frame_prep_kernel(int64_t n_rays, const float *__restrict__ rays_o,
@@ -167,7 +168,7 @@
                                                          const float *__restrict__ aabbs, float near_plane,
                                                          float *__restrict__ t_sorted, uint8_t *__restrict__ t_indices,
                                                          uint8_t *__restrict__ hits, float *__restrict__ near_planes,
-                                                         float *__restrict__ rgb,
+                                                         float *__restrict__ ray_sh, float *__restrict__ rgb,
                                                          float *__restrict__ opacity, float *__restrict__ depth)
 {
     int64_t r = (int64_t)blockIdx.x * blockDim.x + threadIdx.x;
@@ -197,21 +198,28 @@
         t_indices[r * 2 * m + i] = (uint8_t)id[i];
     }
     near_planes[r] = near_plane;
-    rgb[3 * r] = 0.0f; rgb[3 * r + 1] = 0.0f; rgb[3 * r + 2] = 0.0f;
-    opacity[r] = 0.0f;
-    depth[r] = 0.0f;
+    store_ray_sh(r, rays_d, ray_sh);
+    if (rgb) {
+        rgb[3 * r] = 0.0f; rgb[3 * r + 1] = 0.0f; rgb[3 * r + 2] = 0.0f;
+        opacity[r] = 0.0f;
+        depth[r] = 0.0f;
+    }
 }
 
 __global__ __launch_bounds__(256) void frame_prep_single_kernel(int64_t n_rays, float near_plane, float *__restrict__ near_planes,
+                                                                const float *__restrict__ rays_d, float *__restrict__ ray_sh,
                                                                 float *__restrict__ rgb, float *__restrict__ opacity,
                                                                 float *__restrict__ depth)
 {
     int64_t r = (int64_t)blockIdx.x * blockDim.x + threadIdx.x;
     if (r >= n_rays) return;
     near_planes[r] = near_plane;
-    rgb[3 * r] = 0.0f; rgb[3 * r + 1] = 0.0f; rgb[3 * r + 2] = 0.0f;
-    opacity[r] = 0.0f;
-    depth[r] = 0.0f;
+    store_ray_sh(r, rays_d, ray_sh);
+    if (rgb) {
+        rgb[3 * r] = 0.0f; rgb[3 * r + 1] = 0.0f; rgb[3 * r + 2] = 0.0f;
+        opacity[r] = 0.0f;
+        depth[r] = 0.0f;
+    }
 }
 
 struct ScheduleArgs {
@@ -518,6 +526,7 @@
 namespace ced {
 #endif
 
+template <bool FIRST>
 __global__ __launch_bounds__(kCompositeThreads) void frame_composite_kernel(
     IterPlan *plan, int n_frames, int rays_per_frame, const int32_t *__restrict__ alive_list,
     int32_t *__restrict__ next_list, const int32_t *__restrict__ packed, const float *__restrict__ t0,
@@ -539,10 +548,11 @@
         if (active) {
             const int64_t sb = packed[2 * r];
             cnt = packed[2 * r + 1];
-            float op = opacity[r];
+            float op = FIRST ? 0.0f : opacity[r];
+            float c0 = 0.0f, c1 = 0.0f, c2 = 0.0f, dp = 0.0f;
             if (cnt > 0) {
                 const float prefix = 1.0f - op;
-                float c0 = rgb[3 * r], c1 = rgb[3 * r + 1], c2 = rgb[3 * r + 2], dp = depth[r];
+                if constexpr (!FIRST) { c0 = rgb[3 * r]; c1 = rgb[3 * r + 1]; c2 = rgb[3 * r + 2]; dp = depth[r]; }
                 float acc = 0.0f;
                 constexpr int kU = 4;
                 int64_t i = sb;
@@ -581,6 +591,8 @@
                     dp = dp + w * ((ts + te) / 2.0f);
                     acc = acc + sd;
                 }
+            }
+            if (FIRST || cnt > 0) {
                 rgb[3 * r] = c0; rgb[3 * r + 1] = c1; rgb[3 * r + 2] = c2;
                 opacity[r] = op;
                 depth[r] = dp;
@@ -612,19 +624,25 @@
 }
 
 __global__ __launch_bounds__(256) void frame_finalize_kernel(int64_t n_rays, const float *__restrict__ bkgd,
-                                                             float *__restrict__ rgb, const float *__restrict__ opacity,
-                                                             float *__restrict__ depth)
+                                                             const float *acc_rgb, const float *acc_opacity,
+                                                             const float *acc_depth, const int64_t *__restrict__ dest,
+                                                             float *rgb, float *opacity, float *depth)
 {
     int64_t r = (int64_t)blockIdx.x * blockDim.x + threadIdx.x;
     if (r >= n_rays) return;
-    float op = opacity[r];
+    const int64_t p = dest ? dest[r] : r;
+    if (p < 0 || p >= n_rays) return;
+    float op = acc_opacity[r];
+    float c0 = acc_rgb[3 * r], c1 = acc_rgb[3 * r + 1], c2 = acc_rgb[3 * r + 2];
     if (bkgd) {
         float rem = 1.0f - op;
-        rgb[3 * r] = rgb[3 * r] + bkgd[0] * rem;
-        rgb[3 * r + 1] = rgb[3 * r + 1] + bkgd[1] * rem;
-        rgb[3 * r + 2] = rgb[3 * r + 2] + bkgd[2] * rem;
-    }
-    depth[r] = depth[r] / __builtin_fmaxf(op, FLT_EPSILON);
+        c0 = c0 + bkgd[0] * rem;
+        c1 = c1 + bkgd[1] * rem;
+        c2 = c2 + bkgd[2] * rem;
+    }
+    if (bkgd || acc_rgb != rgb) { rgb[3 * p] = c0; rgb[3 * p + 1] = c1; rgb[3 * p + 2] = c2; }
+    if (acc_opacity != opacity) opacity[p] = op;
+    depth[p] = acc_depth[r] / __builtin_fmaxf(op, FLT_EPSILON);
 }
 
 struct ImageState {
@@ -634,12 +652,14 @@
     int32_t *kept;
 };
 
-__global__ __launch_bounds__(256) void image_prep_kernel(int64_t n_rays, ImageState st, float *__restrict__ rgb,
+__global__ __launch_bounds__(256) void image_prep_kernel(int64_t n_rays, ImageState st, const float *__restrict__ rays_d,
+                                                         float *__restrict__ ray_sh, float *__restrict__ rgb,
                                                          float *__restrict__ opacity, float *__restrict__ depth)
 {
     int64_t r = (int64_t)blockIdx.x * blockDim.x + threadIdx.x;
     if (r >= n_rays) return;
     st.cursor[r] = 0; st.acc_all[r] = 0.0f; st.acc_kept[r] = 0.0f; st.kept[r] = 0;
+    if (ray_sh) store_ray_sh(r, rays_d, ray_sh);
     if (rgb) {
         rgb[3 * r] = 0.0f; rgb[3 * r + 1] = 0.0f; rgb[3 * r + 2] = 0.0f;
         opacity[r] = 0.0f;
@@ -911,9 +931,10 @@
     int32_t *alive_a, *alive_b;
     IterPlan *plans;
     float *lattice;
-    float *ts_ray;
+    float *ray_sh;
     float *t0, *t1; int32_t *ridx; float *sigma, *rgbs;
     uint8_t *accel;
+    float *acc_rgb, *acc_opacity, *acc_depth;
     size_t bytes;
 };
 
@@ -930,7 +951,7 @@
     return per * n_frames;
 }
 
-static FrameWorkspace carve(void *base, int64_t n, int m, int64_t cap, int max_iters, int res, bool per_ray_times = false)
+static FrameWorkspace carve(void *base, int64_t n, int m, int64_t cap, int max_iters, int res, bool own_sums = false)
 {
     FrameWorkspace w{};
     Carver c{ (char *)base };
@@ -943,7 +964,7 @@
     w.alive_b = c.take<int32_t>((size_t)n);
     w.plans = c.take<IterPlan>((size_t)max_iters + 2);
     w.lattice = c.take<float>(256);
-    w.ts_ray = c.take<float>(per_ray_times ? (size_t)n : 0);
+    w.ray_sh = c.take<float>((size_t)n * 3);
     w.t0 = c.take<float>((size_t)cap);
     w.t1 = c.take<float>((size_t)cap);
     w.ridx = c.take<int32_t>((size_t)cap);
@@ -951,6 +972,9 @@
     w.rgbs = c.take<float>((size_t)cap * 3);
     const int64_t nbk = (res + kBrick - 1) / kBrick;
     w.accel = c.take<uint8_t>((size_t)(2 * m * nbk * nbk * nbk));
+    w.acc_rgb = c.take<float>(own_sums ? (size_t)n * 3 : 0);
+    w.acc_opacity = c.take<float>(own_sums ? (size_t)n : 0);
+    w.acc_depth = c.take<float>(own_sums ? (size_t)n : 0);
     w.bytes = c.off;
     return w;
 }
@@ -1028,7 +1052,8 @@
                               int32_t t_per_ray, const float *frame_times, const float *bkgd, float *rgb, float *opacity,
                               float *depth, void *workspace, int64_t workspace_bytes, int64_t *host_stats,
                               int64_t *total_samples_out, ced_frame_trace *trace, void *field_stream_, void *stream_,
-                              const char *who, const ced_shard_exchange *xch = nullptr)
+                              const char *who, const ced_shard_exchange *xch = nullptr,
+                              const int64_t *pixel_index = nullptr)
 {
     hipStream_t stream = (hipStream_t)stream_;
     hipStream_t fstream = field_stream_ ? (hipStream_t)field_stream_ : stream;
@@ -1060,9 +1085,24 @@
     const int64_t cap = sample_capacity(n_frames, rays_per_frame, min_samples, xch ? xch->global_rays_per_frame : 0);
     CED_REQUIRE(cap < (1ll << 31) - 64, "%s: too many samples per iteration for 32-bit sample indices", who);
     const int max_iters = max_iterations(max_samples, min_samples);
-    FrameWorkspace W = carve(workspace, n_rays, n_grids, cap, max_iters, res, frame_times != nullptr);
+    FrameWorkspace W = carve(workspace, n_rays, n_grids, cap, max_iters, res, pixel_index != nullptr);
     CED_REQUIRE((int64_t)W.bytes <= workspace_bytes, "%s: workspace too small (%lld < %lld bytes)", who,
                 (long long)workspace_bytes, (long long)W.bytes);
+    FrameDiv fdiv{ 0, 0 };
+    const float *per_frame_times = nullptr;
+    if (frame_times) {
+        if (n_frames == 1) { timestamps = frame_times; t_per_ray = 0; }
+        else if (rays_per_frame == 1) { timestamps = frame_times; t_per_ray = 1; }
+        else {
+            per_frame_times = frame_times;
+            CED_REQUIRE(make_frame_div(rays_per_frame, fdiv), "%s: no exact multiply-high divider for %lld rays per frame", who,
+                        (long long)rays_per_frame);
+        }
+    }
+    float *const sum_rgb = pixel_index ? W.acc_rgb : rgb, *const sum_op = pixel_index ? W.acc_opacity : opacity,
+                *const sum_dp = pixel_index ? W.acc_depth : depth;
+    const bool zero_in_first = !(xch && xch->local_rays) && max_iters > 0 && max_samples > 0;
+    float *const z_rgb = zero_in_first ? nullptr : sum_rgb;
     if (xch) {
         CED_REQUIRE(xch->reduce && xch->counts && xch->global_rays_per_frame >= rays_per_frame &&
                         xch->global_rays_per_frame < (1ll << 31),
@@ -1073,12 +1113,11 @@
     const dim3 blk(256), grd((unsigned)((n_rays + 255) / 256));
 
     if (n_grids == 1)
-        hipLaunchKernelGGL(frame_prep_single_kernel, grd, blk, 0, stream, n_rays, near_plane, W.near, rgb, opacity, depth);
+        hipLaunchKernelGGL(frame_prep_single_kernel, grd, blk, 0, stream, n_rays, near_plane, W.near, rays_d, W.ray_sh, z_rgb,
+                           sum_op, sum_dp);
     else
         hipLaunchKernelGGL(frame_prep_kernel, grd, blk, 0, stream, n_rays, rays_o, rays_d, (int)n_grids, aabbs, near_plane,
-                           W.t_sorted, W.t_indices, W.hits, W.near, rgb, opacity, depth);
-    if (frame_times)
-        hipLaunchKernelGGL(frame_times_kernel, grd, blk, 0, stream, n_rays, (int)rays_per_frame, frame_times, W.ts_ray);
+                           W.t_sorted, W.t_indices, W.hits, W.near, W.ray_sh, z_rgb, sum_op, sum_dp);
     const int nb = (res + kBrick - 1) / kBrick;
     AccelSpec acc;
     if (accel) {
@@ -1150,8 +1189,10 @@
         F.n_dev = &plan->total_samples;
         F.rays_o = rays_o; F.rays_d = rays_d; F.ray_idx32 = W.ridx;
         F.t0 = W.t0; F.t1 = W.t1;
-        F.timestamps = frame_times ? W.ts_ray : timestamps;
-        F.rays_mode = 1; F.t_per_ray = (frame_times || t_per_ray) ? 1 : 0; F.want_rgb = 1;
+        F.timestamps = per_frame_times ? per_frame_times : timestamps;
+        F.frame_mul = fdiv.mul; F.frame_shift = fdiv.shift;
+        F.ray_sh = W.ray_sh;
+        F.rays_mode = 1; F.t_per_ray = per_frame_times ? 2 : (t_per_ray ? 1 : 0); F.want_rgb = 1;
         F.rgb = W.rgbs; F.sigma = W.sigma; F.geo = nullptr;
         if (trace && trace->field_stamps && it < trace->capacity)
             F.stamp = reinterpret_cast<unsigned long long *>(trace->field_stamps) + 2 * it;
@@ -1173,9 +1214,14 @@
         int64_t cgrid = (slot_bound + kCompositeThreads - 1) / kCompositeThreads;
         if (cgrid > 4096) cgrid = 4096;
         plan_seq[it + 1] = ++g_publish_seq;
-        hipLaunchKernelGGL(frame_composite_kernel, dim3((unsigned)cgrid), dim3(kCompositeThreads), 0, stream,
-                           plan, n_frames, (int)rays_per_frame, cur_list, next_list, W.packed, W.t0, W.t1, W.sigma, W.rgbs,
-                           rgb, opacity, depth, opc_thres);
+        if (it == 0 && zero_in_first)
+            hipLaunchKernelGGL(frame_composite_kernel<true>, dim3((unsigned)cgrid), dim3(kCompositeThreads), 0, stream,
+                               plan, n_frames, (int)rays_per_frame, cur_list, next_list, W.packed, W.t0, W.t1, W.sigma, W.rgbs,
+                               sum_rgb, sum_op, sum_dp, opc_thres);
+        else
+            hipLaunchKernelGGL(frame_composite_kernel<false>, dim3((unsigned)cgrid), dim3(kCompositeThreads), 0, stream,
+                               plan, n_frames, (int)rays_per_frame, cur_list, next_list, W.packed, W.t0, W.t1, W.sigma, W.rgbs,
+                               sum_rgb, sum_op, sum_dp, opc_thres);
         int64_t *xrow = nullptr;
         if (xch) {
             xrow = xch->counts + (int64_t)it * n_frames;
@@ -1197,7 +1243,8 @@
         if (rc) return rc;
     }
     const int enqueued = it;
-    hipLaunchKernelGGL(frame_finalize_kernel, grd, blk, 0, stream, n_rays, bkgd, rgb, opacity, depth);
+    hipLaunchKernelGGL(frame_finalize_kernel, grd, blk, 0, stream, n_rays, bkgd, (const float *)sum_rgb, (const float *)sum_op,
+                       (const float *)sum_dp, pixel_index, rgb, opacity, depth);
     rc = check_launch("render_image_test (finalize)");
     if (rc) return rc;
     std::vector<IterPlan> plans;
@@ -1232,6 +1279,7 @@
     int32_t *packed, *alive_a, *alive_b;
     IterPlan *plans;
     float *t0, *t1; int32_t *ridx; float *sigma, *rgbs, *w, *tr, *al; int32_t *rank;
+    float *ray_sh;
     size_t bytes;
 };
 
@@ -1257,6 +1305,7 @@
     w.tr = c.take<float>((size_t)cap);
     w.al = c.take<float>((size_t)cap);
     w.rank = c.take<int32_t>((size_t)cap);
+    w.ray_sh = c.take<float>((size_t)n * 3);
     w.bytes = c.off;
     return w;
 }
@@ -1289,7 +1338,8 @@
     CED_REQUIRE((int64_t)W.bytes <= workspace_bytes, "%s: workspace too small (%lld < %lld bytes)", who,
                 (long long)workspace_bytes, (long long)W.bytes);
     const dim3 blk(256), grd((unsigned)((n_rays + 255) / 256));
-    hipLaunchKernelGGL(image_prep_kernel, grd, blk, 0, stream, n_rays, W.st, rgb, opacity, depth);
+    hipLaunchKernelGGL(image_prep_kernel, grd, blk, 0, stream, n_rays, W.st, rays_d, full ? W.ray_sh : (float *)nullptr, rgb,
+                       opacity, depth);
     volatile long long *pub = (volatile long long *)host_stats;
     std::vector<long long> plan_seq((size_t)kImageMaxIters + 1);
     plan_seq[0] = ++g_publish_seq;
@@ -1322,6 +1372,7 @@
         F.rays_o = rays_o; F.rays_d = rays_d; F.ray_idx32 = W.ridx;
         F.t0 = W.t0; F.t1 = W.t1;
         F.timestamps = timestamps;
+        F.ray_sh = full ? W.ray_sh : nullptr;
         F.rays_mode = 1; F.t_per_ray = t_per_ray ? 1 : 0; F.want_rgb = full ? 1 : 0;
         F.rgb = full ? W.rgbs : nullptr; F.sigma = W.sigma; F.geo = nullptr;
         rc = launch_field(field, F, (void *)stream);
@@ -1345,7 +1396,9 @@
         if (rc) return rc;
     }
     const int enqueued = it;
-    if (full) hipLaunchKernelGGL(frame_finalize_kernel, grd, blk, 0, stream, n_rays, bkgd, rgb, opacity, depth);
+    if (full)
+        hipLaunchKernelGGL(frame_finalize_kernel, grd, blk, 0, stream, n_rays, bkgd, (const float *)rgb, (const float *)opacity,
+                           (const float *)depth, (const int64_t *)nullptr, rgb, opacity, depth);
     rc = check_launch("render_image (finalize)");
     if (rc) return rc;
     std::vector<IterPlan> plans;
@@ -1398,6 +1451,38 @@
     return (int64_t)ced::carve(nullptr, n_rays, n_grids, n_rays * ms, ced::max_iterations(max_samples, ms), res, true).bytes;
 }
 
+extern "C" int ced_render_frames_test_raster(const ced_field_desc *field, int32_t n_frames, int64_t rays_per_frame,
+                                             const float *rays_o, const float *rays_d, const uint8_t *binaries,
+                                             int32_t n_grids, int32_t res, const float *aabbs, const void *accel,
+                                             float near_plane, float far_plane, float step_size, float cone_angle,
+                                             float early_stop_eps, int32_t max_samples, const float *frame_times,
+                                             const float *bkgd, float *rgb, float *opacity, float *depth, void *workspace,
+                                             int64_t workspace_bytes, int64_t *host_stats, int64_t *total_samples_out,
+                                             ced_frame_trace *trace, void *field_stream_, void *stream_,
+                                             const int64_t *pixel_index)
+{
+    CED_REQUIRE(frame_times != nullptr, "render_frames_test_raster: null frame_times");
+    return ced::render_frames_impl(field, n_frames, rays_per_frame, rays_o, rays_d, binaries, n_grids, res, aabbs, accel,
+                                   near_plane, far_plane, step_size, cone_angle, early_stop_eps, max_samples, nullptr, 0,
+                                   frame_times, bkgd, rgb, opacity, depth, workspace, workspace_bytes, host_stats,
+                                   total_samples_out, trace, field_stream_, stream_, "render_frames_test_raster", nullptr,
+                                   pixel_index);
+}
+
+extern "C" int ced_host_frames_of_rays(int64_t n, const int64_t *rays, int64_t rays_per_frame, int64_t *frames)
+{
+    CED_REQUIRE(n >= 0 && rays_per_frame >= 1 && rays_per_frame < (1ll << 31), "host_frames_of_rays: bad sizes");
+    if (n == 0) return CED_OK;
+    CED_REQUIRE(rays && frames, "host_frames_of_rays: null pointer");
+    ced::FrameDiv fd{ 0, 0 };
+    CED_REQUIRE(rays_per_frame == 1 || ced::make_frame_div(rays_per_frame, fd), "host_frames_of_rays: no exact divider");
+    for (int64_t i = 0; i < n; ++i) {
+        CED_REQUIRE(rays[i] >= 0 && rays[i] < (1ll << 31), "host_frames_of_rays: ray index outside [0, 2^31)");
+        frames[i] = rays_per_frame == 1 ? rays[i] : (int64_t)ced::frame_of_ray((uint32_t)rays[i], fd.mul, fd.shift);
+    }
+    return CED_OK;
+}
+
 extern "C" int ced_render_frames_test(const ced_field_desc *field, int32_t n_frames, int64_t rays_per_frame,
                                       const float *rays_o, const float *rays_d, const uint8_t *binaries, int32_t n_grids,
                                       int32_t res, const float *aabbs, const void *accel, float near_plane,
@@ -1425,7 +1510,7 @@
     const int64_t n_rays = (int64_t)n_frames * rays_per_frame;
     const int ms = ced::min_samples_of(cone_angle);
     return (int64_t)ced::carve(nullptr, n_rays, n_grids, ced::sample_capacity(n_frames, rays_per_frame, ms, global_rays_per_frame),
-                               ced::max_iterations(max_samples, ms), res, true).bytes;
+                               ced::max_iterations(max_samples, ms), res).bytes;
 }
 
 extern "C" int32_t ced_render_frames_test_iterations(float cone_angle, int32_t max_samples)
diff --git a/ced_nerf_amd/dist.py b/ced_nerf_amd/dist.py
--- a/ced_nerf_amd/dist.py
+++ b/ced_nerf_amd/dist.py
@@ -51,6 +51,7 @@
         self.force_collective = force_collective
         self.tile_order = tile_order
         self.unpermute = None
+        self._native_unpermute = render_fn is None
         self.units = int(units)
         assert 1 <= self.units <= 64, "units must be 1..64"
         self.schedule_group = schedule_group
@@ -76,6 +77,13 @@
                 tracer=self.tracer, field_max_workgroups=self.field_max_workgroups, exchange=self.exchange,
                 **self.render_kwargs)
             return rgb.view(-1, 3), op.view(-1, 1), dp.view(-1, 1), sum(totals)
+        index = self._ray_index if (self.unpermute is not None and self._native_unpermute) else None
+        if self.units == 1 and index is not None and timestamps.numel() == 1 and not self.field.training:
+            rgb, op, dp, totals = render_frames_test(
+                self.max_samples, self.field, self.estimator, Rays(rays_o.view(1, -1, 3), rays_d.view(1, -1, 3)),
+                timestamps=timestamps.reshape(1).float(), tracer=self.tracer, field_stream=self.field_stream,
+                field_max_workgroups=self.field_max_workgroups, pixel_index=index, **self.render_kwargs)
+            return _raster_rows(rgb.view(-1, 3)), op.view(-1, 1), dp.view(-1, 1), sum(totals)
         if self.units == 1:
             return render_image_test(self.max_samples, self.field, self.estimator, Rays(rays_o, rays_d),
                                      timestamps=timestamps, tracer=self.tracer, field_stream=self.field_stream,
@@ -86,8 +94,9 @@
         rgb, op, dp, totals = render_frames_test(
             self.max_samples, self.field, self.estimator, Rays(rays_o.view(u, -1, 3), rays_d.view(u, -1, 3)), timestamps=ts,
             tracer=self.tracer, field_stream=self.field_stream, field_max_workgroups=self.field_max_workgroups,
-            **self.render_kwargs)
-        return rgb.view(-1, 3), op.view(-1, 1), dp.view(-1, 1), sum(totals)
+            pixel_index=index, **self.render_kwargs)
+        rgb = rgb.view(-1, 3)
+        return (_raster_rows(rgb) if index is not None else rgb), op.view(-1, 1), dp.view(-1, 1), sum(totals)
 
     def set_rays(self, origins: torch.Tensor, viewdirs: torch.Tensor) -> None:
         assert origins.ndim == 4 and origins.shape == viewdirs.shape, "rays must be [F,H,W,3]"
@@ -155,7 +164,7 @@
         F, H, W = self.shape
         rgb, op, dp, n_samples = local
         if self.gather_index is None:
-            if self.unpermute is not None:
+            if self.unpermute is not None and not getattr(rgb, "rows_in_raster", False):
                 if rgb.is_cuda:
                     from . import ops
                     rgb, op, dp, _ = ops.scatter_pixels(self._ray_index, F * H * W, rgb.reshape(-1, 3), op.reshape(-1, 1),
@@ -196,6 +205,11 @@
     @torch.no_grad()
     def render(self, timestamps: torch.Tensor) -> Dict:
         return self.gather(self.render_local(timestamps))
+
+
+def _raster_rows(rgb: torch.Tensor) -> torch.Tensor:
+    rgb.rows_in_raster = True
+    return rgb
 
 
 def _all_reduce_on(row: torch.Tensor, stream: int, group) -> None:
diff --git a/ced_nerf_amd/ops.py b/ced_nerf_amd/ops.py
--- a/ced_nerf_amd/ops.py
+++ b/ced_nerf_amd/ops.py
@@ -896,9 +896,11 @@
                               render_step_size, cone_angle, early_stop_eps, max_samples, frame_times, bkgd,
                               tracer: Optional[FrameTracer] = None, field_stream: Optional[torch.cuda.Stream] = None,
                               accel: Optional[torch.Tensor] = None, max_workgroups: int = 0,
-                              exchange: Optional[ScheduleExchange] = None):
+                              exchange: Optional[ScheduleExchange] = None, pixel_index: Optional[torch.Tensor] = None):
     _chk(rays_o, torch.float32, "rays_o"); _chk(rays_d, torch.float32, "rays_d")
     _chk(aabbs, torch.float32, "aabbs"); _chk(frame_times, torch.float32, "frame_times")
+    _chk(pixel_index, torch.int64, "pixel_index", allow_none=True)
+    assert pixel_index is None or (exchange is None and pixel_index.shape == (rays_o.shape[0],))
     _chk(bkgd, torch.float32, "render_bkgd", allow_none=True)
     assert rays_o.ndim == 2 and rays_o.shape[1] == 3 and rays_o.shape == rays_d.shape
     assert binaries.is_cuda and binaries.is_contiguous() and binaries.ndim == 4
@@ -928,7 +930,9 @@
             _p(rgb), _p(opacity), _p(depth), _p(ws[0]), ws[0].numel(), C.c_void_p(ws[1].data_ptr()),
             totals, C.byref(tracer.struct) if tracer is not None else None,
             C.c_void_p(field_stream.cuda_stream) if field_stream is not None else None, _stream())
-    if exchange is None:
+    if pixel_index is not None:
+        rc = L.ced_render_frames_test_raster(*args, _p(pixel_index))
+    elif exchange is None:
         rc = L.ced_render_frames_test(*args)
     else:
         assert exchange.n_frames == n_frames and exchange.counts.device == dev
diff --git a/ced_nerf_amd/utils.py b/ced_nerf_amd/utils.py
--- a/ced_nerf_amd/utils.py
+++ b/ced_nerf_amd/utils.py
@@ -215,6 +215,7 @@
     field_stream=None,
     field_max_workgroups: int = 0,
     exchange=None,
+    pixel_index: Optional[torch.Tensor] = None,
 ):
     if timestamps is None:
         raise NotImplementedError("DNGPradianceField needs timestamps (dnerf path of cednerf/utils.py:186-194)")
@@ -232,7 +233,7 @@
         radiance_field._descriptor(), n_frames, rays_o, rays_d, estimator.binaries, estimator.aabbs.contiguous(),
         near_plane, far_plane, render_step_size, cone_angle, early_stop_eps, max_samples, ts, bk,
         tracer=tracer, field_stream=field_stream, accel=estimator.occupancy_accel(), max_workgroups=field_max_workgroups,
-        exchange=exchange)
+        exchange=exchange, pixel_index=pixel_index)
     return rgb.view((*shape[:-1], 3)), opacity.view((*shape[:-1], 1)), depth.view((*shape[:-1], 1)), totals
 
 
diff --git a/include/cednerf_hip.h b/include/cednerf_hip.h
--- a/include/cednerf_hip.h
+++ b/include/cednerf_hip.h
@@ -275,6 +275,15 @@
                            const float *frame_times, const float *bkgd, float *rgb, float *opacity, float *depth,
                            void *workspace, int64_t workspace_bytes, int64_t *host_stats,
                            int64_t *total_samples_out, ced_frame_trace *trace, void *field_stream, void *stream);
+int ced_render_frames_test_raster(const ced_field_desc *field, int32_t n_frames, int64_t rays_per_frame,
+                                  const float *rays_o, const float *rays_d, const uint8_t *binaries, int32_t n_grids,
+                                  int32_t res, const float *aabbs, const void *accel, float near_plane, float far_plane,
+                                  float render_step_size, float cone_angle, float early_stop_eps, int32_t max_samples,
+                                  const float *frame_times, const float *bkgd, float *rgb, float *opacity, float *depth,
+                                  void *workspace, int64_t workspace_bytes, int64_t *host_stats,
+                                  int64_t *total_samples_out, ced_frame_trace *trace, void *field_stream, void *stream,
+                                  const int64_t *pixel_index);
+int ced_host_frames_of_rays(int64_t n, const int64_t *rays, int64_t rays_per_frame, int64_t *frames);
 
 typedef int (*ced_exchange_fn)(void *user, int64_t *counts, int32_t n_counts, int32_t iteration, void *stream);
 typedef struct ced_shard_exchange {
```
